# nv-tlabs/ChronoEdit

Hardware: AMD Instinct MI355X
Metric: denoising-steps/sec (higher is better)
Workload: dtype bf16

## Files before the change

### chronoedit_amd/csrc/ce_attn.hip

```cpp
#include <cstdlib>

#include "ce_common.h"

namespace {

constexpr int HD = 128;
constexpr int QW = 32;
constexpr int KVB = 64;
constexpr int K_TILE_BYTES = KVB * HD * 2;
constexpr int VT_TILE_BYTES = HD * KVB * 2;
constexpr int BUF_BYTES = K_TILE_BYTES + VT_TILE_BYTES;
constexpr int OST_ROW = HD * 2 + 16;
constexpr int smem_bytes(int nwave, bool two_seg) {
  const int stage = nwave * QW * OST_ROW;
  return two_seg ? 2 * BUF_BYTES + stage : (stage > 2 * BUF_BYTES ? stage : 2 * BUF_BYTES);
}
constexpr float NEG_BIG = -1.0e30f;

__device__ __forceinline__ int vt_swz(int dv) {
  return ((((dv >> 2) & 7) << 1) | (((dv >> 1) ^ (dv >> 5)) & 1)) ^ (((dv >> 6) & 1) << 1);
}

struct KVSeg {
  const bf16* k;
  const bf16* v;
  int len;
  int ldk;
  int ldv;
};
struct BlkRows {
  int rows;
  int stride;
  uint32_t magic;
  int vt_cols;
  unsigned char* q8;
  unsigned char* s8;
  int ld8;
};

template <bool TWO_SEG, int NWAVE>
__global__ __launch_bounds__(NWAVE * 64, NWAVE == 8 ? 2 : 2) void attn_fwd_kernel(const bf16* __restrict__ Q, bf16* __restrict__ O, KVSeg seg0,
                                                       KVSeg seg1, int Nq, int H, int ldq, int ldo, int nqb,
                                                       float scale_log2e) {
  extern __shared__ __attribute__((aligned(16))) unsigned char smem[];
  {
    const size_t bz = blockIdx.y;
    Q += bz * Nq * ldq;
    O += bz * Nq * ldo;
    seg0.k += bz * seg0.len * seg0.ldk;
    seg0.v += bz * seg0.len * seg0.ldv;
    if (TWO_SEG) {
      seg1.k += bz * seg1.len * seg1.ldk;
      seg1.v += bz * seg1.len * seg1.ldv;
    }
  }
  const int tid = threadIdx.x, lane = tid & 63, wave = tid >> 6;
  const int l31 = lane & 31, hh = lane >> 5;

  int head, qb;
  if ((H & 7) == 0) {
    const int xcd = blockIdx.x & 7, local = blockIdx.x >> 3;
    head = xcd + 8 * (local / nqb);
    qb = local % nqb;
  } else {
    head = blockIdx.x / nqb;
    qb = blockIdx.x % nqb;
  }
  constexpr int QB = QW * NWAVE;
  constexpr int NT = NWAVE * 64;
  const int q0 = qb * QB + wave * QW;
  const int hoff = head * HD;

  bf16x8 qf[8];
  {
    const bf16* qrow = Q + (size_t)min(q0 + l31, Nq - 1) * ldq + hoff + 8 * hh;
#pragma unroll
    for (int ks = 0; ks < 8; ++ks) qf[ks] = *reinterpret_cast<const bf16x8*>(qrow + 16 * ks);
  }

  constexpr int KREP = 1024 / NT, KROWS = NT / 16;
  const int k_ck = tid & 15, k_row0 = tid >> 4;
  constexpr int VREP = 512 / NT, VKQ = NT / 32;
  const int v_dvq = tid & 31, v_kvq = tid >> 5;

  unsigned char* ost = smem + (TWO_SEG ? 2 * BUF_BYTES : 0) + (size_t)(wave * QW + l31) * OST_ROW;

#pragma unroll
  for (int sidx = 0; sidx < (TWO_SEG ? 2 : 1); ++sidx) {
    const KVSeg sg = sidx == 0 ? seg0 : seg1;
    const int ntiles = (sg.len + KVB - 1) / KVB;

    f32x16 oacc[4];
#pragma unroll
    for (int m = 0; m < 4; ++m)
#pragma unroll
      for (int r = 0; r < 16; ++r) oacc[m][r] = 0.f;
    float m_run = NEG_BIG, l_run = 0.f;

    u32x4 kreg[KREP];
    u32x2 vreg[VREP][4];
    auto load_tile = [&](int t) {
      const int kv0 = t * KVB;
#pragma unroll
      for (int i = 0; i < KREP; ++i) {
        const int r = min(kv0 + k_row0 + KROWS * i, sg.len - 1);
        kreg[i] = *reinterpret_cast<const u32x4*>(sg.k + (size_t)r * sg.ldk + hoff + k_ck * 8);
      }
#pragma unroll
      for (int p = 0; p < VREP; ++p)
#pragma unroll
        for (int i = 0; i < 4; ++i) {
          const int r = min(kv0 + 4 * (v_kvq + VKQ * p) + i, sg.len - 1);
          vreg[p][i] = *reinterpret_cast<const u32x2*>(sg.v + (size_t)r * sg.ldv + hoff + v_dvq * 4);
        }
    };
    auto store_tile = [&](int buf) {
      unsigned char* sK = smem + buf * BUF_BYTES;
      unsigned char* sV = sK + K_TILE_BYTES;
#pragma unroll
      for (int i = 0; i < KREP; ++i) {
        const int r = k_row0 + KROWS * i;
        *reinterpret_cast<u32x4*>(sK + r * (HD * 2) + ((k_ck ^ (r & 15)) << 4)) = kreg[i];
      }
#pragma unroll
      for (int p = 0; p < VREP; ++p)
#pragma unroll
        for (int j = 0; j < 4; ++j) {
          const int w = j >> 1;
          uint32_t lo, hi;
          if ((j & 1) == 0) {
            lo = (vreg[p][0][w] & 0xffffu) | (vreg[p][1][w] << 16);
            hi = (vreg[p][2][w] & 0xffffu) | (vreg[p][3][w] << 16);
          } else {
            lo = (vreg[p][0][w] >> 16) | (vreg[p][1][w] & 0xffff0000u);
            hi = (vreg[p][2][w] >> 16) | (vreg[p][3][w] & 0xffff0000u);
          }
          const int dv = 4 * v_dvq + j;
          u32x2 val = {lo, hi};
          *reinterpret_cast<u32x2*>(sV + dv * (KVB * 2) + (((v_kvq + VKQ * p) ^ vt_swz(dv)) << 3)) = val;
        }
    };

    load_tile(0);
    __syncthreads();
    store_tile(0);
    __syncthreads();

    for (int t = 0; t < ntiles; ++t) {
      const int cur = t & 1;
      if (t + 1 < ntiles) load_tile(t + 1);
      const unsigned char* sK = smem + cur * BUF_BYTES;
      const unsigned char* sV = sK + K_TILE_BYTES;

      f32x16 st[2];
#pragma unroll
      for (int f = 0; f < 2; ++f) {
#pragma unroll
        for (int r = 0; r < 16; ++r) st[f][r] = 0.f;
        const int r = 32 * f + l31;
        const unsigned char* krow = sK + r * (HD * 2);
#pragma unroll
        for (int ks = 0; ks < 8; ++ks) {
          const bf16x8 kf = *reinterpret_cast<const bf16x8*>(krow + (((2 * ks + hh) ^ (r & 15)) << 4));
          st[f] = __builtin_amdgcn_mfma_f32_32x32x16_bf16(kf, qf[ks], st[f], 0, 0, 0);
        }
      }
      if ((t + 1) * KVB > sg.len) {
        const int base = t * KVB + 4 * hh;
#pragma unroll
        for (int f = 0; f < 2; ++f)
#pragma unroll
          for (int r = 0; r < 16; ++r) {
            const int kv = base + 32 * f + (r & 3) + 8 * (r >> 2);
            if (kv >= sg.len) st[f][r] = NEG_BIG;
          }
      }
      float mx = st[0][0];
#pragma unroll
      for (int f = 0; f < 2; ++f)
#pragma unroll
        for (int r = 0; r < 16; ++r) mx = fmaxf(mx, st[f][r]);
      mx = fmaxf(mx, __shfl_xor(mx, 32, 64));
      const float m_new = fmaxf(m_run, mx);
      const float alpha = __builtin_amdgcn_exp2f((m_run - m_new) * scale_log2e);
      const float mc = m_new * scale_log2e;
      m_run = m_new;
      float psum = 0.f;
#pragma unroll
      for (int f = 0; f < 2; ++f)
#pragma unroll
        for (int r = 0; r < 16; ++r) {
          const float p = __builtin_amdgcn_exp2f(fmaf(st[f][r], scale_log2e, -mc));
          st[f][r] = p;
          psum += p;
        }
      l_run = l_run * alpha + psum;
      if (__any(alpha != 1.0f)) {
#pragma unroll
        for (int m = 0; m < 4; ++m)
#pragma unroll
          for (int r = 0; r < 16; ++r) oacc[m][r] *= alpha;
      }

#pragma unroll
      for (int s = 0; s < 4; ++s) {
        const int f = s >> 1, rb = 8 * (s & 1);
        f32x2 t0 = {st[f][rb + 0], st[f][rb + 1]}, t1 = {st[f][rb + 2], st[f][rb + 3]};
        f32x2 t2 = {st[f][rb + 4], st[f][rb + 5]}, t3 = {st[f][rb + 6], st[f][rb + 7]};
        const bf16x2 p0 = __builtin_convertvector(t0, bf16x2), p1 = __builtin_convertvector(t1, bf16x2);
        const bf16x2 p2 = __builtin_convertvector(t2, bf16x2), p3 = __builtin_convertvector(t3, bf16x2);
        const bf16x8 pf = {p0[0], p0[1], p1[0], p1[1], p2[0], p2[1], p3[0], p3[1]};
        const int c0 = 4 * s + hh;
#pragma unroll
        for (int m = 0; m < 4; ++m) {
          const int dv = 32 * m + l31;
          const unsigned char* vrow = sV + dv * (KVB * 2);
          const int sw = vt_swz(dv);
          const bf16x4 va = *reinterpret_cast<const bf16x4*>(vrow + ((c0 ^ sw) << 3));
          const bf16x4 vb = *reinterpret_cast<const bf16x4*>(vrow + (((c0 + 2) ^ sw) << 3));
          const bf16x8 vf = {va[0], va[1], va[2], va[3], vb[0], vb[1], vb[2], vb[3]};
          oacc[m] = __builtin_amdgcn_mfma_f32_32x32x16_bf16(vf, pf, oacc[m], 0, 0, 0);
        }
      }
      if (t + 1 < ntiles) store_tile(cur ^ 1);
      __syncthreads();
    }

    const float l_tot = l_run + __shfl_xor(l_run, 32, 64);
    const float inv = 1.0f / l_tot;
#pragma unroll
    for (int m = 0; m < 4; ++m)
#pragma unroll
      for (int a = 0; a < 4; ++a) {
        uint32_t w0 = pack_bf16(oacc[m][4 * a + 0] * inv, oacc[m][4 * a + 1] * inv);
        uint32_t w1 = pack_bf16(oacc[m][4 * a + 2] * inv, oacc[m][4 * a + 3] * inv);
        u32x2* slot = reinterpret_cast<u32x2*>(ost + (32 * m + 8 * a + 4 * hh) * 2);
        if (TWO_SEG && sidx == 1) {
          const u32x2 pv = *slot;
          w0 = pack_bf16(bf16lo(pv[0]) + bf16lo(w0), bf16hi(pv[0]) + bf16hi(w0));
          w1 = pack_bf16(bf16lo(pv[1]) + bf16lo(w1), bf16hi(pv[1]) + bf16hi(w1));
        }
        u32x2 val = {w0, w1};
        *slot = val;
      }
  }

  __syncthreads();
#pragma unroll
  for (int i = 0; i < 8; ++i) {
    const int c = lane + 64 * i;
    const int rl = c >> 4, cc = c & 15;
    const int q = q0 + rl;
    if (q < Nq) {
      const u32x4 v = *reinterpret_cast<const u32x4*>(smem + (TWO_SEG ? 2 * BUF_BYTES : 0) + (size_t)(wave * QW + rl) * OST_ROW + cc * 16);
      *reinterpret_cast<u32x4*>(O + (size_t)q * ldo + hoff + cc * 8) = v;
    }
  }
}


#define CE_EPOCH_BARRIER()                          \
  asm volatile("s_waitcnt lgkmcnt(0)" ::: "memory"); \
  __builtin_amdgcn_s_barrier()
constexpr int PK_ROW = HD * 2 + 16;
constexpr int PV_ROW = KVB * 2 + 16;
constexpr int PK_TILE = KVB * PK_ROW;
constexpr int PV_TILE = HD * PV_ROW;
typedef __attribute__((ext_vector_type(4))) unsigned pp_u4;
typedef __attribute__((ext_vector_type(2))) unsigned pp_u2;

constexpr int K_GRP = 1088;
typedef __attribute__((address_space(3))) void lds_void;
#ifdef CE_DIAGNOSTICS
__device__ unsigned long long g_sp_exact_hits = 0ull;
#endif
constexpr float SP_SPEC_THR = 1024.0f;
constexpr int SP_V0 = 2 * PK_TILE;
constexpr int SP_TILE_BYTES = 2 * PK_TILE + 3 * PV_TILE;
constexpr int sp_smem_bytes(bool two_seg) { return two_seg ? SP_TILE_BYTES + 8 * QW * OST_ROW : SP_TILE_BYTES; }

template <bool TWO_SEG, bool VT = false, bool QOUT = false>
__global__ __launch_bounds__(512, 2) void attn_fwd_sp_kernel(const bf16* __restrict__ Q_, bf16* __restrict__ O_, KVSeg seg0_,
                                                              KVSeg seg1_, int Nq, int H, int ldq, int ldo, int nqb,
                                                              float scale_log2e, int batch, BlkRows blk) {
  extern __shared__ __attribute__((aligned(16))) unsigned char smem[];
  constexpr int NWAVE = 8, QB = QW * NWAVE;
  const int tid = threadIdx.x, lane = tid & 63;
  const int wave = __builtin_amdgcn_readfirstlane(tid >> 6);
  const int l31 = lane & 31, hh = lane >> 5;
  for (int item = blockIdx.x; item < nqb * H * batch; item += gridDim.x) {
  const bf16* Q = Q_;
  bf16* O = O_;
  KVSeg seg0 = seg0_, seg1 = seg1_;

  int head, qb, bz;
  {
    const int nqb_full = Nq / QB;
    if ((H & 7) == 0) {
      const int xcd = item & 7, local = item >> 3, hx_n = H >> 3;
      const int full = batch * hx_n * nqb_full;
      if (local < full) {
        bz = local / (hx_n * nqb_full);
        const int r = local % (hx_n * nqb_full);
        head = xcd + 8 * (r / nqb_full);
        qb = r % nqb_full;
      } else {
        const int l2 = local - full;
        bz = l2 / hx_n;
        head = xcd + 8 * (l2 % hx_n);
        qb = nqb_full;
      }
    } else {
      bz = item / (nqb * H);
      const int r = item % (nqb * H);
      head = r / nqb;
      qb = r % nqb;
    }
  }
  {
    if (VT && blk.rows > 0) {
      Q += (size_t)bz * blk.rows * ldq;
      O += (size_t)bz * blk.rows * ldo;
      seg0.k += (size_t)bz * blk.rows * seg0.ldk;
      seg0.v += (size_t)bz * blk.vt_cols;
    } else {
      Q += (size_t)bz * Nq * ldq;
      O += (size_t)bz * Nq * ldo;
      seg0.k += (size_t)bz * seg0.len * seg0.ldk;
      seg0.v += VT ? (size_t)bz * (TWO_SEG ? blk.vt_cols : seg0.len) : (size_t)bz * seg0.len * seg0.ldv;
    }
    if (TWO_SEG) {
      seg1.k += (size_t)bz * seg1.len * seg1.ldk;
      seg1.v += VT ? (size_t)bz * blk.stride : (size_t)bz * seg1.len * seg1.ldv;
    }
  }
  const int q0 = qb * QB + wave * QW;
  const int hoff = head * HD;
  const bool active = q0 < Nq;
  const int q0row = (VT && blk.rows > 0) ? (q0 / blk.rows) * blk.stride + q0 % blk.rows : q0;

  bf16x8 qf[8];
  {
    const bf16* qrow = Q + (size_t)(q0 + l31 < Nq ? q0row + l31 : 0) * ldq + hoff + 8 * hh;
#pragma unroll
    for (int ks = 0; ks < 8; ++ks) qf[ks] = *reinterpret_cast<const bf16x8*>(qrow + 16 * ks);
  }
  auto scale_q = [&]() __attribute__((always_inline)) {
#pragma unroll
  for (int ks = 0; ks < 8; ++ks) {
    const u32x4 w = __builtin_bit_cast(u32x4, qf[ks]);
    u32x4 o;
#pragma unroll
    for (int i = 0; i < 4; ++i) o[i] = pack_bf16(bf16lo(w[i]) * scale_log2e, bf16hi(w[i]) * scale_log2e);
    qf[ks] = __builtin_bit_cast(bf16x8, o);
  }
#pragma unroll
  for (int ks = 0; ks < 8; ++ks) asm volatile("" : "+v"(qf[ks]));

  };
  const int v_dvq = (tid & 1) | (((tid >> 4) & 15) << 1), v_kvq = ((tid >> 1) & 7) | (((tid >> 8) & 1) << 3);
  const int v_chunk = (v_kvq & ~3) | ((v_kvq & 1) << 1) | ((v_kvq >> 1) & 1);
  unsigned char* ost = smem + (TWO_SEG ? SP_TILE_BYTES : 0) + (size_t)(wave * QW + l31) * OST_ROW;
  const int k_w = l31 & 3;
  const unsigned char* k_rd = smem + (l31 >> 2) * K_GRP + k_w * 256 + ((hh ^ (k_w & 1)) << 4);
  const int k_eo[2] = {(k_w >> 1) << 5, ((k_w >> 1) ^ 1) << 5};
  const unsigned char* v_rd = smem + SP_V0 + l31 * PV_ROW + hh * 16;
  int vt_off[4];
#pragma unroll
  for (int s4 = 0; s4 < 4; ++s4) {
    const int x = (l31 >> 1) & 7;
    vt_off[s4] = l31 * 128 + ((2 * (s4 ^ (x >> 1)) + (hh ^ (x & 1))) << 4);
  }
  unsigned char* v_wr = smem + SP_V0 + (4 * v_dvq) * PV_ROW + v_chunk * 8;

#pragma unroll
  for (int sidx = 0; sidx < (TWO_SEG ? 2 : 1); ++sidx) {
    const KVSeg sg = sidx == 0 ? seg0 : seg1;
    const int ntiles = (sg.len + KVB - 1) / KVB;
    const int k_rows_span = (VT && blk.rows > 0) ? ((sg.len - 1) / blk.rows) * blk.stride + blk.rows : sg.len;
    const auto k_rsrc = __builtin_amdgcn_make_buffer_rsrc((void*)(sg.k + hoff), 0, (k_rows_span - 1) * sg.ldk * 2 + HD * 2, 0x00020000);
    const auto v_rsrc = VT ? __builtin_amdgcn_make_buffer_rsrc((void*)(sg.v + (size_t)hoff * sg.ldv), 0, ((HD - 1) * sg.ldv + ntiles * KVB) * 2, 0x00020000)
                           : __builtin_amdgcn_make_buffer_rsrc((void*)(sg.v + hoff), 0, (sg.len - 1) * sg.ldv * 2 + HD * 2, 0x00020000);
    int v_voff[4];
#pragma unroll
    for (int i = 0; i < 4; ++i) v_voff[i] = (4 * v_kvq + i) * sg.ldv * 2 + v_dvq * 8;
    const int k_tile_bytes = KVB * sg.ldk * 2, v_tile_bytes = KVB * sg.ldv * 2;

    f32x16 oacc[4];
#pragma unroll
    for (int m = 0; m < 4; ++m)
#pragma unroll
      for (int r = 0; r < 16; ++r) oacc[m][r] = 0.f;
    float l_run = 0.f, alpha_prev = 1.0f, mc = 0.f;
    f32x16 cinit;
#pragma unroll
    for (int r = 0; r < 16; ++r) cinit[r] = 0.f;
    u32x4 ppk[4];
#pragma unroll
    for (int s4 = 0; s4 < 4; ++s4) ppk[s4] = u32x4{0u, 0u, 0u, 0u};

    pp_u2 vreg[4];
    const int kd_row = VT ? (lane >> 4) + 4 * ((wave >> 1) & 1) + 8 * (wave & 1) + 16 * (wave >> 2) : 4 * wave + (lane >> 4);
    const int kd_voff0 = kd_row * sg.ldk * 2 + (((lane & 15) ^ (lane >> 4)) << 4), kd_voff1 = kd_voff0 + 32 * sg.ldk * 2;
    const int vd_row = 8 * wave + (lane >> 3);
    const int vd_voff0 = vd_row * sg.ldv * 2 + (((lane & 7) ^ ((vd_row >> 1) & 7)) << 4), vd_voff1 = vd_voff0 + 64 * sg.ldv * 2;
    auto dma_v = [&](int t, int buf, int j) {
      __builtin_amdgcn_raw_ptr_buffer_load_lds(v_rsrc, (lds_void*)(smem + SP_V0 + buf * PV_TILE + (wave + 8 * j) * 1024), 16,
                                               j ? vd_voff1 : vd_voff0, t * (KVB * 2), 0, 0);
    };
    auto dma_k = [&](int t, int buf, int j) {
      int soff = t * k_tile_bytes;
      if (VT && blk.rows > 0) {
        const int b_ = blk.magic ? (int)__umulhi((uint32_t)t, blk.magic) : t;
        soff = (b_ * blk.stride + (t - b_ * (blk.rows >> 6)) * KVB) * sg.ldk * 2;
      }
      __builtin_amdgcn_raw_ptr_buffer_load_lds(k_rsrc, (lds_void*)(smem + buf * PK_TILE + (wave + 8 * j) * K_GRP), 16,
                                               j ? kd_voff1 : kd_voff0, soff, 0, 0);
    };
    auto load_v = [&](int t) {
      const int so = t * v_tile_bytes;
#pragma unroll
      for (int i = 0; i < 4; ++i) vreg[i] = __builtin_amdgcn_raw_buffer_load_b64(v_rsrc, v_voff[i], so, 0);
    };
    auto store_v_part = [&](int buf, int j) {
      const int w = j >> 1;
      uint32_t lo, hi;
      if ((j & 1) == 0) {
        lo = (vreg[0][w] & 0xffffu) | (vreg[1][w] << 16);
        hi = (vreg[2][w] & 0xffffu) | (vreg[3][w] << 16);
      } else {
        lo = (vreg[0][w] >> 16) | (vreg[1][w] & 0xffff0000u);
        hi = (vreg[2][w] >> 16) | (vreg[3][w] & 0xffff0000u);
      }
      pp_u2 val = {lo, hi};
      *reinterpret_cast<pp_u2*>(v_wr + buf * PV_TILE + j * PV_ROW) = val;
    };
    auto store_v = [&](int buf) {
#pragma unroll
      for (int j = 0; j < 4; ++j) {
        const int w = j >> 1;
        uint32_t lo, hi;
        if ((j & 1) == 0) {
          lo = (vreg[0][w] & 0xffffu) | (vreg[1][w] << 16);
          hi = (vreg[2][w] & 0xffffu) | (vreg[3][w] << 16);
        } else {
          lo = (vreg[0][w] >> 16) | (vreg[1][w] & 0xffff0000u);
          hi = (vreg[2][w] >> 16) | (vreg[3][w] & 0xffff0000u);
        }
        pp_u2 val = {lo, hi};
        *reinterpret_cast<pp_u2*>(v_wr + buf * PV_TILE + j * PV_ROW) = val;
      }
    };

    if (TWO_SEG && sidx == 1) { CE_EPOCH_BARRIER(); }
    dma_k(0, 0, 0);
    dma_k(0, 0, 1);
    __builtin_amdgcn_sched_barrier(0);
    if (VT) {
      dma_v(0, 0, 0);
      dma_v(0, 0, 1);
    } else {
      load_v(0);
    }
    {
      const pp_u4 z = {0u, 0u, 0u, 0u};
      for (int i = tid; i < PV_TILE / 16; i += NWAVE * 64) *reinterpret_cast<pp_u4*>(smem + SP_V0 + 2 * PV_TILE + i * 16) = z;
    }
    if (!VT) {
      store_v(0);
      asm volatile("s_waitcnt vmcnt(0)" ::: "memory");
      load_v(1);
    }
    if (sidx == 0) scale_q();

#define CE_SP_KWAIT()                                          \
  do {                                                         \
    if (VT) asm volatile("s_waitcnt vmcnt(2)" ::: "memory");   \
    else asm volatile("s_waitcnt vmcnt(4)" ::: "memory");      \
  } while (0)
    int vb_prev = 2, vb_cur = 0;

    for (int t = 0; !active && t < ntiles; ++t) {
      CE_SP_KWAIT();
      CE_EPOCH_BARRIER();
      const int vb_next = 3 - vb_prev - vb_cur;
      dma_k(t + 1, (t + 1) & 1, 0);
      dma_k(t + 1, (t + 1) & 1, 1);
      __builtin_amdgcn_sched_barrier(0);
      if (VT) {
        dma_v(t + 1, vb_next, 0);
        dma_v(t + 1, vb_next, 1);
      } else {
        store_v(vb_next);
        load_v(t + 2);
      }
      vb_prev = vb_cur;
      vb_cur = vb_next;
    }
    for (int t = 0; active && t < ntiles; ++t) {
      CE_SP_KWAIT();
// ... 622 lines not shown
#pragma unroll
          for (int m = 0; m < 4; ++m)
#pragma unroll
            for (int r = 0; r < 16; ++r) oacc[sb][m][r] *= alpha_prev[sb];
          W4A_SETTLE_O(sb);
        }
#pragma unroll
      for (int u = 0; u < 16; ++u) {
        const bf16x8 vfd = CE_LDV(vtb, u);
#pragma unroll
        for (int sb = 0; sb < NSB; ++sb) W4A_PV(oacc[sb][u & 3], vfd, ppk[sb][u >> 2]);
      }
    }
#undef CE_LDK
#undef CE_LDV
#pragma unroll
    for (int sb = 0; sb < NSB; ++sb) W4A_SETTLE_O(sb);
    CE_EPOCH_BARRIER();
#pragma unroll
    for (int sb = 0; sb < NSB; ++sb) {
      unsigned char* ost = smem + (size_t)(wave * QWW + 32 * sb + l31) * OST_ROW;
      const float l_tot = l_run[sb] + __shfl_xor(l_run[sb], 32, 64);
      const float inv = 1.0f / l_tot;
#pragma unroll
      for (int m = 0; m < 4; ++m)
#pragma unroll
        for (int a = 0; a < 4; ++a) {
          const uint32_t w0 = pack_bf16(oacc[sb][m][4 * a + 0] * inv, oacc[sb][m][4 * a + 1] * inv);
          const uint32_t w1 = pack_bf16(oacc[sb][m][4 * a + 2] * inv, oacc[sb][m][4 * a + 3] * inv);
          *reinterpret_cast<u32x2*>(ost + (32 * m + 8 * a + 4 * hh) * 2) = u32x2{w0, w1};
        }
    }
  };
  if (active) {
    if (two_sub) run(w4_int<2>{});
    else run(w4_int<1>{});
  }
  __syncthreads();
#pragma unroll
  for (int i = 0; i < 16; ++i) {
    const int c = lane + 64 * i;
    const int rl = c >> 4, cc = c & 15;
    if (q0 + rl < Nq) {
      const u32x4 v = *reinterpret_cast<const u32x4*>(smem + (size_t)(wave * QWW + rl) * OST_ROW + cc * 16);
      *reinterpret_cast<u32x4*>(O + (size_t)(q0row + rl) * ldo + hoff + cc * 8) = v;
    }
  }
  __syncthreads();
  }
}
#undef W4A_S_FIRST
#undef W4A_S
#undef W4A_PV
#undef W4A_ADD
#undef W4A_CVT
#undef W4A_EXP
#undef W4A_SETTLE_S
#undef W4A_SETTLE_O

__global__ __launch_bounds__(256) void v_transpose_kernel(const bf16* __restrict__ V, int ldv, bf16* __restrict__ VT, int ldvt, int n_keys,
                                                          int blk_rows, int blk_stride, int vt_cols) {
  __shared__ __attribute__((aligned(16))) unsigned char tile[HD * (KVB * 2 + 16)];
  constexpr int TROW = KVB * 2 + 16;
  const int tid = threadIdx.x, head = blockIdx.y, key0 = blockIdx.x * KVB;
  if (blk_rows > 0) {
    V += ((size_t)(key0 / blk_rows) * blk_stride + (size_t)blockIdx.z * blk_rows + key0 % blk_rows - key0) * ldv;
    VT += (size_t)blockIdx.z * vt_cols;
  }
  const int col_end = blk_rows > 0 ? vt_cols : ldvt;
  const int kq = tid & 15, dq = tid >> 4;
#pragma unroll
  for (int pass = 0; pass < 2; ++pass) {
    const int d0 = 4 * (dq + 16 * pass);
    pp_u2 r[4];
#pragma unroll
    for (int i = 0; i < 4; ++i) {
      const int key = key0 + 4 * kq + i;
      r[i] = key < n_keys ? *reinterpret_cast<const pp_u2*>(V + (size_t)key * ldv + head * HD + d0) : pp_u2{0u, 0u};
    }
#pragma unroll
    for (int j = 0; j < 4; ++j) {
      const int w = j >> 1;
      uint32_t lo, hi;
      if ((j & 1) == 0) {
        lo = (r[0][w] & 0xffffu) | (r[1][w] << 16);
        hi = (r[2][w] & 0xffffu) | (r[3][w] << 16);
      } else {
        lo = (r[0][w] >> 16) | (r[1][w] & 0xffff0000u);
        hi = (r[2][w] >> 16) | (r[3][w] & 0xffff0000u);
      }
      *reinterpret_cast<pp_u2*>(tile + (d0 + j) * TROW + kq * 8) = pp_u2{lo, hi};
    }
  }
  __syncthreads();
#pragma unroll
  for (int i = 0; i < 4; ++i) {
    const int c = tid + 256 * i;
    const int d = c >> 3, ch = c & 7;
    const pp_u4 v = *reinterpret_cast<const pp_u4*>(tile + d * TROW + ch * 16);
    const int col = key0 + 8 * ch;
    if (col < col_end) *reinterpret_cast<pp_u4*>(VT + (size_t)(head * HD + d) * ldvt + col) = v;
  }
}

}

#ifdef CE_DIAGNOSTICS
extern "C" int ce_diag_mx_exact_hits(unsigned long long* out, int reset);
CE_API int ce_diag_attention_exact_route_hits(unsigned long long* hits, int reset) {
  if (!hits) return CE_ERR_ARG;
  unsigned long long v = 0ull, z = 0ull;
  if (hipDeviceSynchronize() != hipSuccess) return CE_ERR_ARG;
  if (hipMemcpyFromSymbol(&v, HIP_SYMBOL(g_sp_exact_hits), sizeof(v)) != hipSuccess) return CE_ERR_ARG;
  if (reset && hipMemcpyToSymbol(HIP_SYMBOL(g_sp_exact_hits), &z, sizeof(z)) != hipSuccess) return CE_ERR_ARG;
  hits[0] = v;
  return ce_diag_mx_exact_hits(hits + 1, reset);
}
#endif
CE_KNOB g_attn_nwave = 0;
#ifdef CE_DIAGNOSTICS
CE_API int ce_set_attention_waves(int nwave) {
  const int old = g_attn_nwave;
  if (nwave == 0 || nwave == 4 || nwave == 8 || nwave == 16 || nwave == 64 || nwave == 128 || nwave == 129) g_attn_nwave = nwave;
  return old;
}
#endif

CE_API int ce_attention_batched_bf16(const void* Q, const void* K1, const void* V1, int len1, int ldk1, int ldv1,
                                         const void* K2, const void* V2, int len2, int ldk2, int ldv2, void* O, int Nq, int H,
                                         int head_dim, int ldq, int ldo, float softmax_scale, int batch, hipStream_t stream) {
  if (!Q || !K1 || !V1 || !O) return CE_ERR_ARG;
  if (head_dim != HD || Nq <= 0 || H <= 0 || len1 <= 0 || batch <= 0 || batch > 65535) return CE_ERR_SHAPE;
  if ((ldq & 7) || (ldo & 7) || (ldk1 & 7) || (ldv1 & 3)) return CE_ERR_ALIGN;
  const bool two = (K2 != nullptr && V2 != nullptr && len2 > 0);
  if (two && ((ldk2 & 7) || (ldv2 & 3))) return CE_ERR_ALIGN;
  KVSeg s0{(const bf16*)K1, (const bf16*)V1, len1, ldk1, ldv1};
  KVSeg s1{(const bf16*)K2, (const bf16*)V2, two ? len2 : 0, ldk2, ldv2};
  const float sl2 = softmax_scale * 1.4426950408889634f;
  const bool sp = g_attn_nwave == 64 || g_attn_nwave == 0 || g_attn_nwave >= 128;
  const int nwave = sp ? 8 : g_attn_nwave;
  const int nqb = (Nq + nwave * QW - 1) / (nwave * QW);
  dim3 grid(nqb * H, batch), block(nwave * 64);
  if (sp) {
#define CE_ATTN_SP(TWO)                                                                                              \
  do {                                                                                                               \
    static bool done_[CE_MAX_DEVICES] = {};                                                                          \
    bool& done = done_[ce_device_slot()];                                                                            \
    if (!done) {                                                                                                     \
      (void)hipFuncSetAttribute((const void*)attn_fwd_sp_kernel<TWO>, hipFuncAttributeMaxDynamicSharedMemorySize,    \
                                sp_smem_bytes(TWO));                                                                 \
      done = true;                                                                                                   \
    }                                                                                                                \
    hipLaunchKernelGGL((attn_fwd_sp_kernel<TWO>), dim3(nqb * H * batch), block, sp_smem_bytes(TWO), stream, (const bf16*)Q, \
                       (bf16*)O, s0, s1, Nq, H, ldq, ldo, nqb, sl2, batch, BlkRows{0, 0, 0u, 0});                    \
  } while (0)
    if (two) CE_ATTN_SP(true); else CE_ATTN_SP(false);
#undef CE_ATTN_SP
    return (int)hipGetLastError();
  }
#define CE_ATTN_LAUNCH(TWO, NW)                                                                                     \
  do {                                                                                                              \
    static bool done_[CE_MAX_DEVICES] = {};                                                                         \
    bool& done = done_[ce_device_slot()];                                                                           \
    if (!done) {                                                                                                    \
      (void)hipFuncSetAttribute((const void*)attn_fwd_kernel<TWO, NW>, hipFuncAttributeMaxDynamicSharedMemorySize,  \
                                smem_bytes(NW, TWO));                                                               \
      done = true;                                                                                                  \
    }                                                                                                               \
    hipLaunchKernelGGL((attn_fwd_kernel<TWO, NW>), grid, block, smem_bytes(NW, TWO), stream, (const bf16*)Q, (bf16*)O, \
                       s0, s1, Nq, H, ldq, ldo, nqb, sl2);                                                          \
  } while (0)
  if (two) {
    if (nwave == 8) CE_ATTN_LAUNCH(true, 8); else CE_ATTN_LAUNCH(true, 4);
  } else {
    if (nwave == 8) CE_ATTN_LAUNCH(false, 8); else CE_ATTN_LAUNCH(false, 4);
  }
#undef CE_ATTN_LAUNCH
  return (int)hipGetLastError();
}

CE_API int ce_attention_bf16(const void* Q, const void* K1, const void* V1, int len1, int ldk1, int ldv1, const void* K2,
                                 const void* V2, int len2, int ldk2, int ldv2, void* O, int Nq, int H, int head_dim, int ldq,
                                 int ldo, float softmax_scale, hipStream_t stream) {
  return ce_attention_batched_bf16(Q, K1, V1, len1, ldk1, ldv1, K2, V2, len2, ldk2, ldv2, O, Nq, H, head_dim, ldq, ldo,
                                   softmax_scale, 1, stream);
}

CE_API int ce_v_transpose_bf16(const void* v, int ldv, void* vt, int ldvt, int n_keys, int H, hipStream_t stream) {
  if (!v || !vt) return CE_ERR_ARG;
  if (n_keys <= 0 || H <= 0 || ldvt < n_keys) return CE_ERR_SHAPE;
  if ((ldv & 3) || (ldvt & 7)) return CE_ERR_ALIGN;
  hipLaunchKernelGGL(v_transpose_kernel, dim3((ldvt + KVB - 1) / KVB, H), dim3(256), 0, stream, (const bf16*)v, ldv, (bf16*)vt, ldvt, n_keys, 0, 0, 0);
  return (int)hipGetLastError();
}

CE_API int ce_v_transpose_blocked_bf16(const void* v, int ldv, void* vt, int ldvt, int n_keys, int H, int batch, int blk_rows, int blk_stride,
                                           int vt_sample_cols, hipStream_t stream) {
  if (!v || !vt) return CE_ERR_ARG;
  if (n_keys <= 0 || H <= 0 || batch <= 0 || blk_rows <= 0 || (blk_rows & 63) || blk_stride < batch * blk_rows || (vt_sample_cols & 63) ||
      vt_sample_cols < (n_keys + KVB - 1) / KVB * KVB || ldvt < batch * vt_sample_cols)
    return CE_ERR_SHAPE;
  if ((ldv & 3) || (ldvt & 7)) return CE_ERR_ALIGN;
  hipLaunchKernelGGL(v_transpose_kernel, dim3(vt_sample_cols / KVB, H, batch), dim3(256), 0, stream, (const bf16*)v, ldv, (bf16*)vt, ldvt, n_keys,
                     blk_rows, blk_stride, vt_sample_cols);
  return (int)hipGetLastError();
}

#ifdef CE_DIAGNOSTICS
extern "C" int ce_attn16_launch(const void* Q, const void* K, const void* Vt, int len, int ldk, int ldvt, void* O, int Nq, int H, int ldq, int ldo,
                                float sl2, int batch, int cus, hipStream_t stream);
#endif

static int attention_vt_launch(const void* Q, const void* K, const void* Vt, int len, int ldk, int ldvt, void* O, int Nq, int H, int head_dim,
                               int ldq, int ldo, float softmax_scale, int batch, int blk_rows, int blk_stride, int vt_sample_cols,
                               hipStream_t stream) {
  if (!Q || !K || !Vt || !O) return CE_ERR_ARG;
  if (head_dim != HD || Nq <= 0 || H <= 0 || len <= 0 || batch <= 0 || batch > 65535) return CE_ERR_SHAPE;
  const int ntiles_cols = (len + KVB - 1) / KVB * KVB;
  if (blk_rows == 0) {
    vt_sample_cols = len;
    if (ldvt < (batch - 1) * len + ntiles_cols) return CE_ERR_SHAPE;
  } else {
    if ((blk_rows & 63) || blk_stride < batch * blk_rows || (Nq % blk_rows) || vt_sample_cols < ntiles_cols ||
        ldvt < (batch - 1) * vt_sample_cols + ntiles_cols)
      return CE_ERR_SHAPE;
  }
  if ((ldq & 7) || (ldo & 7) || (ldk & 7) || (ldvt & 7) || (batch > 1 && (vt_sample_cols & 1))) return CE_ERR_ALIGN;
  KVSeg s0{(const bf16*)K, (const bf16*)Vt, len, ldk, ldvt};
  KVSeg s1{nullptr, nullptr, 0, 0, 0};
  BlkRows blk{blk_rows, blk_stride, 0u, vt_sample_cols};
  if (blk_rows > 0) {
    const uint32_t tps = (uint32_t)(blk_rows >> 6);
    blk.magic = tps == 1 ? 0u : (uint32_t)(((1ull << 32) + tps - 1) / tps);
  }
  const float sl2 = softmax_scale * 1.4426950408889634f;
  const int nqb = (Nq + 8 * QW - 1) / (8 * QW);
  static bool done_[CE_MAX_DEVICES] = {};
  bool& done = done_[ce_device_slot()];
  if (!done) {
    (void)hipFuncSetAttribute((const void*)attn_fwd_sp_kernel<false, true>, hipFuncAttributeMaxDynamicSharedMemorySize, sp_smem_bytes(false));
    done = true;
  }
  const int cus = ce_device_cus();
  const int items = nqb * H * batch;
#ifdef CE_DIAGNOSTICS
  if (g_attn_nwave == 16 && blk_rows == 0) {
    const int rc = ce_attn16_launch(Q, K, Vt, len, ldk, ldvt, O, Nq, H, ldq, ldo, sl2, batch, cus, stream);
    if (rc != CE_ERR_ALIGN) return rc;
  }
#endif
  if (g_attn_nwave == 128 || g_attn_nwave == 129) {
    static bool done4_[CE_MAX_DEVICES] = {};
    bool& done4 = done4_[ce_device_slot()];
    if (!done4) {
      (void)hipFuncSetAttribute((const void*)attn_fwd_w4_kernel, hipFuncAttributeMaxDynamicSharedMemorySize, W4_SMEM);
      done4 = true;
    }
    const int grid4 = (g_attn_nwave == 129 && items > cus) ? (cus & ~7) : items;
    hipLaunchKernelGGL(attn_fwd_w4_kernel, dim3(grid4), dim3(256), W4_SMEM, stream, (const bf16*)Q, (bf16*)O, s0, Nq, H, ldq, ldo, nqb,
                       sl2, batch, blk);
    return (int)hipGetLastError();
  }
  const int grid_vt = items <= 2 * cus ? items : ((2 * cus) & ~7);
  hipLaunchKernelGGL((attn_fwd_sp_kernel<false, true>), dim3(grid_vt), dim3(512), sp_smem_bytes(false), stream, (const bf16*)Q, (bf16*)O,
                     s0, s1, Nq, H, ldq, ldo, nqb, sl2, batch, blk);
  return (int)hipGetLastError();
}

CE_API int ce_attention_vt_bf16(const void* Q, const void* K, const void* Vt, int len, int ldk, int ldvt, void* O, int Nq, int H,
                                    int head_dim, int ldq, int ldo, float softmax_scale, int batch, hipStream_t stream) {
  return attention_vt_launch(Q, K, Vt, len, ldk, ldvt, O, Nq, H, head_dim, ldq, ldo, softmax_scale, batch, 0, 0, 0, stream);
}

CE_API int ce_attention_vt_blocked_bf16(const void* Q, const void* K, const void* Vt, int len, int ldk, int ldvt, void* O, int Nq, int H,
                                            int head_dim, int ldq, int ldo, float softmax_scale, int batch, int blk_rows, int blk_stride,
                                            int vt_sample_cols, hipStream_t stream) {
  if (blk_rows <= 0) return CE_ERR_SHAPE;
  return attention_vt_launch(Q, K, Vt, len, ldk, ldvt, O, Nq, H, head_dim, ldq, ldo, softmax_scale, batch, blk_rows, blk_stride, vt_sample_cols,
                             stream);
}


static int attention_2seg_vt_launch(const void* Q, const void* K1, const void* V1t, int len1, int ldk1, int ldv1t, int vt_cols1,
                                    const void* K2, const void* V2t, int len2, int ldk2, int ldv2t, int vt_cols2, void* O, int Nq,
                                    int H, int head_dim, int ldq, int ldo, float softmax_scale, int batch, void* O8, void* S8, int ldo8,
                                    hipStream_t stream) {
  if (!Q || !K1 || !V1t || !K2 || !V2t || (!O && !O8)) return CE_ERR_ARG;
  if (head_dim != HD || Nq <= 0 || H <= 0 || len1 <= 0 || len2 <= 0 || batch <= 0 || batch > 65535) return CE_ERR_SHAPE;
  const int c1 = (len1 + KVB - 1) / KVB * KVB, c2 = (len2 + KVB - 1) / KVB * KVB;
  if (vt_cols1 < len1 || vt_cols2 < len2 || ldv1t < (batch - 1) * vt_cols1 + c1 || ldv2t < (batch - 1) * vt_cols2 + c2) return CE_ERR_SHAPE;
  if ((ldq & 7) || (ldo & 7) || (ldk1 & 7) || (ldk2 & 7) || (ldv1t & 7) || (ldv2t & 7) || (vt_cols1 & 1) || (vt_cols2 & 1)) return CE_ERR_ALIGN;
  KVSeg s0{(const bf16*)K1, (const bf16*)V1t, len1, ldk1, ldv1t};
  KVSeg s1{(const bf16*)K2, (const bf16*)V2t, len2, ldk2, ldv2t};
  const float sl2 = softmax_scale * 1.4426950408889634f;
  const int nqb = (Nq + 8 * QW - 1) / (8 * QW);
  static bool done_[CE_MAX_DEVICES] = {};
  bool& done = done_[ce_device_slot()];
  if (!done) {
    (void)hipFuncSetAttribute((const void*)attn_fwd_sp_kernel<true, true>, hipFuncAttributeMaxDynamicSharedMemorySize, sp_smem_bytes(true));
    (void)hipFuncSetAttribute((const void*)attn_fwd_sp_kernel<true, true, true>, hipFuncAttributeMaxDynamicSharedMemorySize, sp_smem_bytes(true));
    done = true;
  }
  const BlkRows blk{0, vt_cols2, 0u, vt_cols1, (unsigned char*)O8, (unsigned char*)S8, ldo8};
  const int cus = ce_device_cus();
  const int items = nqb * H * batch;
  const int grid = items <= 2 * cus ? items : ((2 * cus) & ~7);
  if (O8)
    hipLaunchKernelGGL((attn_fwd_sp_kernel<true, true, true>), dim3(grid), dim3(512), sp_smem_bytes(true), stream, (const bf16*)Q,
                       (bf16*)O, s0, s1, Nq, H, ldq, ldo, nqb, sl2, batch, blk);
  else
    hipLaunchKernelGGL((attn_fwd_sp_kernel<true, true>), dim3(grid), dim3(512), sp_smem_bytes(true), stream, (const bf16*)Q, (bf16*)O,
                       s0, s1, Nq, H, ldq, ldo, nqb, sl2, batch, blk);
  return (int)hipGetLastError();
}

CE_API int ce_attention_2seg_vt_bf16(const void* Q, const void* K1, const void* V1t, int len1, int ldk1, int ldv1t, int vt_cols1,
                                         const void* K2, const void* V2t, int len2, int ldk2, int ldv2t, int vt_cols2, void* O, int Nq,
                                         int H, int head_dim, int ldq, int ldo, float softmax_scale, int batch, hipStream_t stream) {
  if (!O) return CE_ERR_ARG;
  return attention_2seg_vt_launch(Q, K1, V1t, len1, ldk1, ldv1t, vt_cols1, K2, V2t, len2, ldk2, ldv2t, vt_cols2, O, Nq, H, head_dim, ldq, ldo,
                                  softmax_scale, batch, nullptr, nullptr, 0, stream);
}

CE_API int ce_attention_2seg_vt_quant_bf16(const void* Q, const void* K1, const void* V1t, int len1, int ldk1, int ldv1t, int vt_cols1,
                                               const void* K2, const void* V2t, int len2, int ldk2, int ldv2t, int vt_cols2, void* o8,
                                               void* scale8, int Nq, int H, int head_dim, int ldq, int ldo8, float softmax_scale, int batch,
                                               hipStream_t stream) {
  if (!o8 || !scale8 || (ldo8 & 15) || ((H * head_dim) & 127)) return CE_ERR_ARG;
  return attention_2seg_vt_launch(Q, K1, V1t, len1, ldk1, ldv1t, vt_cols1, K2, V2t, len2, ldk2, ldv2t, vt_cols2, nullptr, Nq, H, head_dim, ldq,
                                  8, softmax_scale, batch, o8, scale8, ldo8, stream);
}
```

### chronoedit_amd/csrc/ce_rowops.hip

```cpp
#include "ce_common.h"

#define ROW_MAXC 10
#ifndef CE_LN_ROWS
#define CE_LN_ROWS 2
#endif

template <int FP8, bool FULL, int R>
__global__ __launch_bounds__(256) void ln_affine_kernel(const bf16* __restrict__ x, bf16* __restrict__ y,
                                                        const float* __restrict__ a, const float* __restrict__ b,
                                                        int M, int D, int ldx, int ldy, float eps, int ab_rows, int ab_stride,
                                                        unsigned char* __restrict__ q8, float* __restrict__ qscale, int ldq) {
  const int lane = threadIdx.x & 63;
  const int row0 = (blockIdx.x * 4 + (threadIdx.x >> 6)) * R;
  if (row0 >= M) return;
  if (ab_rows > 0) {
    a += (size_t)(row0 / ab_rows) * ab_stride;
    b += (size_t)(row0 / ab_rows) * ab_stride;
  }
  const int nch = D >> 3;
  u32x4 raw[R][ROW_MAXC];
  float mean[R], rstd[R];
#pragma unroll
  for (int k = 0; k < R; ++k) {
    const bf16* xr = x + (size_t)min(row0 + k, M - 1) * ldx;
#pragma unroll
    for (int i = 0; i < ROW_MAXC; ++i) {
      const int c = lane + 64 * i;
      if (FULL || c < nch) raw[k][i] = *reinterpret_cast<const u32x4*>(xr + c * 8);
    }
  }
#pragma unroll
  for (int k = 0; k < R; ++k) {
    float s = 0.f;
#pragma unroll
    for (int i = 0; i < ROW_MAXC; ++i) {
      const int c = lane + 64 * i;
      if (FULL || c < nch) {
#pragma unroll
        for (int j = 0; j < 4; ++j) s += bf16lo(raw[k][i][j]) + bf16hi(raw[k][i][j]);
      }
    }
    mean[k] = wave_sum(s) / (float)D;
    float v = 0.f;
#pragma unroll
    for (int i = 0; i < ROW_MAXC; ++i) {
      const int c = lane + 64 * i;
      if (FULL || c < nch) {
#pragma unroll
        for (int j = 0; j < 4; ++j) {
          const float d0 = bf16lo(raw[k][i][j]) - mean[k], d1 = bf16hi(raw[k][i][j]) - mean[k];
          v += d0 * d0 + d1 * d1;
        }
      }
    }
    rstd[k] = 1.0f / sqrtf(wave_sum(v) / (float)D + eps);
  }
  float amax[R];
#pragma unroll
  for (int k = 0; k < R; ++k) amax[k] = 0.f;
#pragma unroll
  for (int i = 0; i < ROW_MAXC; ++i) {
    const int c = lane + 64 * i;
    if (FULL || c < nch) {
      const f32x4 a0 = *reinterpret_cast<const f32x4*>(a + c * 8), a1 = *reinterpret_cast<const f32x4*>(a + c * 8 + 4);
      const f32x4 b0 = *reinterpret_cast<const f32x4*>(b + c * 8), b1 = *reinterpret_cast<const f32x4*>(b + c * 8 + 4);
#pragma unroll
      for (int k = 0; k < R; ++k) {
        u32x4 o;
#pragma unroll
        for (int j = 0; j < 4; ++j) {
          const float aa0 = j < 2 ? a0[2 * j] : a1[2 * j - 4], aa1 = j < 2 ? a0[2 * j + 1] : a1[2 * j - 3];
          const float bb0 = j < 2 ? b0[2 * j] : b1[2 * j - 4], bb1 = j < 2 ? b0[2 * j + 1] : b1[2 * j - 3];
          const float n0 = (bf16lo(raw[k][i][j]) - mean[k]) * rstd[k], n1 = (bf16hi(raw[k][i][j]) - mean[k]) * rstd[k];
          o[j] = pack_bf16(n0 * aa0 + bb0, n1 * aa1 + bb1);
          if (FP8 == 1) amax[k] = fmaxf(amax[k], fmaxf(fabsf(bf16lo(o[j])), fabsf(bf16hi(o[j]))));
        }
        if (FP8 == 1) raw[k][i] = o;
        else if (FP8 == 0 && row0 + k < M) *reinterpret_cast<u32x4*>(y + (size_t)(row0 + k) * ldy + c * 8) = o;
        if (FP8 == 2) raw[k][i] = o;
      }
    }
    if (FP8 == 2) {
#pragma unroll
      for (int k = 0; k < R; ++k) {
        const bool on = (FULL || c < nch) && row0 + k < M;
        const u32x4 v = raw[k][i];
        float am = 0.f;
        if (FULL || c < nch) {
#pragma unroll
          for (int j = 0; j < 4; ++j) am = fmaxf(am, fmaxf(fabsf(bf16lo(v[j])), fabsf(bf16hi(v[j]))));
        }
        am = fmaxf(am, __shfl_xor(am, 1, 64));
        am = fmaxf(am, __shfl_xor(am, 2, 64));
        if (on) {
          const int byte = mx_scale_byte_nosat(am);
          const float inv = mx_inv_scale(byte);
          int w0 = 0, w1 = 0;
          w0 = __builtin_amdgcn_cvt_pk_fp8_f32(clamp448(bf16lo(v[0]) * inv), clamp448(bf16hi(v[0]) * inv), w0, false);
          w0 = __builtin_amdgcn_cvt_pk_fp8_f32(clamp448(bf16lo(v[1]) * inv), clamp448(bf16hi(v[1]) * inv), w0, true);
          w1 = __builtin_amdgcn_cvt_pk_fp8_f32(clamp448(bf16lo(v[2]) * inv), clamp448(bf16hi(v[2]) * inv), w1, false);
          w1 = __builtin_amdgcn_cvt_pk_fp8_f32(clamp448(bf16lo(v[3]) * inv), clamp448(bf16hi(v[3]) * inv), w1, true);
          const u32x2 ov = {(uint32_t)w0, (uint32_t)w1};
          *reinterpret_cast<u32x2*>(q8 + (size_t)(row0 + k) * ldq + c * 8) = ov;
          if ((lane & 3) == 0) reinterpret_cast<unsigned char*>(qscale)[mx_gemm_scale_offset(row0 + k, c >> 2, D >> 7)] = (unsigned char)byte;
        }
      }
    }
  }
  if (FP8 == 1) {
#pragma unroll
    for (int k = 0; k < R; ++k) {
      const float am = wave_max(amax[k]);
      const float sc = am > 0.f ? am * (1.0f / 448.0f) : 1.0f;
      const float inv = 1.0f / sc;
      if (row0 + k >= M) continue;
      if (lane == 0) qscale[row0 + k] = sc;
      unsigned char* qr = q8 + (size_t)(row0 + k) * ldq;
#pragma unroll
      for (int i = 0; i < ROW_MAXC; ++i) {
        const int c = lane + 64 * i;
        if (FULL || c < nch) {
          const u32x4 v = raw[k][i];
          int w0 = 0, w1 = 0;
          w0 = __builtin_amdgcn_cvt_pk_fp8_f32(bf16lo(v[0]) * inv, bf16hi(v[0]) * inv, w0, false);
          w0 = __builtin_amdgcn_cvt_pk_fp8_f32(bf16lo(v[1]) * inv, bf16hi(v[1]) * inv, w0, true);
          w1 = __builtin_amdgcn_cvt_pk_fp8_f32(bf16lo(v[2]) * inv, bf16hi(v[2]) * inv, w1, false);
          w1 = __builtin_amdgcn_cvt_pk_fp8_f32(bf16lo(v[3]) * inv, bf16hi(v[3]) * inv, w1, true);
          u32x2 o = {(uint32_t)w0, (uint32_t)w1};
          *reinterpret_cast<u32x2*>(qr + c * 8) = o;
        }
      }
    }
  }
}

template <bool FULL>
__global__ __launch_bounds__(256) void rmsnorm_rope_kernel(bf16* __restrict__ x0, const float* __restrict__ w0,
                                                           bf16* __restrict__ x1, const float* __restrict__ w1,
                                                           const float* __restrict__ cs, int M, int D, int ld,
                                                           int head_dim, float eps, int rope_rows) {
  const int lane = threadIdx.x & 63;
  const int row = blockIdx.x * 4 + (threadIdx.x >> 6);
  if (row >= M) return;
  bf16* __restrict__ x = blockIdx.y ? x1 : x0;
  const float* __restrict__ w = blockIdx.y ? w1 : w0;
  const int cs_row = rope_rows > 0 ? row % rope_rows : row;
  const int nch = D >> 3;
  bf16* xr = x + (size_t)row * ld;
  u32x4 raw[ROW_MAXC];
  float s = 0.f;
#pragma unroll
  for (int i = 0; i < ROW_MAXC; ++i) {
    const int c = lane + 64 * i;
    if (FULL || c < nch) {
      raw[i] = *reinterpret_cast<const u32x4*>(xr + c * 8);
#pragma unroll
      for (int j = 0; j < 4; ++j) {
        const float v0 = bf16lo(raw[i][j]), v1 = bf16hi(raw[i][j]);
        s += v0 * v0 + v1 * v1;
      }
    }
  }
  const float rstd = 1.0f / sqrtf(wave_sum(s) / (float)D + eps);
  const int half = head_dim >> 1;
  const bool cs_once = cs != nullptr && (512 % head_dim) == 0;
  f32x4 csa = {0.f, 0.f, 0.f, 0.f}, csb = {0.f, 0.f, 0.f, 0.f};
  if (cs_once) {
    const float* p = cs + ((size_t)cs_row * half + (((lane * 8) % head_dim) >> 1)) * 2;
    csa = *reinterpret_cast<const f32x4*>(p);
    csb = *reinterpret_cast<const f32x4*>(p + 4);
  }
#pragma unroll
  for (int i = 0; i < ROW_MAXC; ++i) {
    const int c = lane + 64 * i;
    if (FULL || c < nch) {
      const f32x4 w0 = *reinterpret_cast<const f32x4*>(w + c * 8), w1 = *reinterpret_cast<const f32x4*>(w + c * 8 + 4);
      u32x4 o;
      f32x4 cs0 = csa, cs1 = csb;
      if (cs != nullptr && !cs_once) {
        const int pair0 = ((c * 8) % head_dim) >> 1;
        const float* p = cs + ((size_t)cs_row * half + pair0) * 2;
        cs0 = *reinterpret_cast<const f32x4*>(p);
        cs1 = *reinterpret_cast<const f32x4*>(p + 4);
      }
#pragma unroll
      for (int j = 0; j < 4; ++j) {
        const float ww0 = j < 2 ? w0[2 * j] : w1[2 * j - 4], ww1 = j < 2 ? w0[2 * j + 1] : w1[2 * j - 3];
        float v0 = round_bf16(round_bf16(bf16lo(raw[i][j]) * rstd) * ww0);
        float v1 = round_bf16(round_bf16(bf16hi(raw[i][j]) * rstd) * ww1);
        if (cs != nullptr) {
          const float co = j < 2 ? cs0[2 * j] : cs1[2 * j - 4], si = j < 2 ? cs0[2 * j + 1] : cs1[2 * j - 3];
          const float r0 = v0 * co - v1 * si, r1 = v0 * si + v1 * co;
          v0 = r0;
          v1 = r1;
        }
        o[j] = pack_bf16(v0, v1);
      }
      *reinterpret_cast<u32x4*>(xr + c * 8) = o;
    }
  }
}

template <bool FULL>
__global__ __launch_bounds__(256) void rope_scatter_kernel(const bf16* __restrict__ x, int ldx, bf16* __restrict__ send,
                                                           int M, int D, int W, int nt, int col0, const float* __restrict__ w0,
                                                           int col1, const float* __restrict__ w1, int col2,
                                                           const float* __restrict__ w2, const float* __restrict__ cs,
                                                           int head_dim, float eps, int rope_rows) {
  const int lane = threadIdx.x & 63;
  const int row = blockIdx.x * 4 + (threadIdx.x >> 6);
  if (row >= M) return;
  const int ti = blockIdx.y;
  const int col = ti == 0 ? col0 : ti == 1 ? col1 : col2;
  const float* __restrict__ w = ti == 0 ? w0 : ti == 1 ? w1 : w2;
  const int cs_row = rope_rows > 0 ? row % rope_rows : row;
  const int nch = D >> 3;
  const int Dl = D / W;
  const bf16* xr = x + (size_t)row * ldx + col;
  u32x4 raw[ROW_MAXC];
  float s = 0.f;
#pragma unroll
  for (int i = 0; i < ROW_MAXC; ++i) {
    const int c = lane + 64 * i;
    if (FULL || c < nch) {
      raw[i] = *reinterpret_cast<const u32x4*>(xr + c * 8);
#pragma unroll
      for (int j = 0; j < 4; ++j) {
        const float v0 = bf16lo(raw[i][j]), v1 = bf16hi(raw[i][j]);
        s += v0 * v0 + v1 * v1;
      }
    }
  }
  const float rstd = 1.0f / sqrtf(wave_sum(s) / (float)D + eps);
  const int half = head_dim >> 1;
#pragma unroll
  for (int i = 0; i < ROW_MAXC; ++i) {
    const int c = lane + 64 * i;
    if (FULL || c < nch) {
      u32x4 o = raw[i];
      if (w != nullptr) {
        const f32x4 wa = *reinterpret_cast<const f32x4*>(w + c * 8), wb = *reinterpret_cast<const f32x4*>(w + c * 8 + 4);
        f32x4 cs0, cs1;
        if (cs != nullptr) {
          const int pair0 = ((c * 8) % head_dim) >> 1;
          const float* p = cs + ((size_t)cs_row * half + pair0) * 2;
          cs0 = *reinterpret_cast<const f32x4*>(p);
          cs1 = *reinterpret_cast<const f32x4*>(p + 4);
        }
#pragma unroll
        for (int j = 0; j < 4; ++j) {
          const float ww0 = j < 2 ? wa[2 * j] : wb[2 * j - 4], ww1 = j < 2 ? wa[2 * j + 1] : wb[2 * j - 3];
          float v0 = round_bf16(round_bf16(bf16lo(raw[i][j]) * rstd) * ww0);
          float v1 = round_bf16(round_bf16(bf16hi(raw[i][j]) * rstd) * ww1);
          if (cs != nullptr) {
            const float co = j < 2 ? cs0[2 * j] : cs1[2 * j - 4], si = j < 2 ? cs0[2 * j + 1] : cs1[2 * j - 3];
            const float r0 = v0 * co - v1 * si, r1 = v0 * si + v1 * co;
            v0 = r0;
            v1 = r1;
          }
          o[j] = pack_bf16(v0, v1);
        }
      }
      const int n = c * 8, r = n / Dl, cc = n - r * Dl;
      *reinterpret_cast<u32x4*>(send + (((size_t)r * M + row) * nt + ti) * Dl + cc) = o;
    }
  }
}

template <typename TT>
__global__ void timestep_sinusoid_kernel(const TT* __restrict__ t, float* __restrict__ out, int dim) {
  const int i = blockIdx.x * blockDim.x + threadIdx.x;
  const int half = dim >> 1;
  if (i >= dim) return;
  const int k = i < half ? i : i - half;
  const float freq = expf(-9.210340371976184f * (float)k / (float)half);
  const float arg = (float)t[0] * freq;
  out[i] = i < half ? cosf(arg) : sinf(arg);
}

constexpr int GEMV_ROWS = 16;
template <typename WT>
__global__ __launch_bounds__(256) void gemv_kernel(const WT* __restrict__ W, const float* __restrict__ x,
                                                   const float* __restrict__ bias, float* __restrict__ y, int N, int K,
                                                   int flags) {
  extern __shared__ __attribute__((aligned(16))) float xs[];
  for (int k = threadIdx.x; k < K; k += 256) {
    float xv = x[k];
    if (flags & 1) xv = round_bf16(silu(xv));
    xs[k] = xv;
  }
  __syncthreads();
  const int lane = threadIdx.x & 63, wave = threadIdx.x >> 6;
  constexpr int VEC = 16 / sizeof(WT);
  const bool vec = (K % (64 * VEC)) == 0 && ((size_t)W & 15) == 0;
  for (int r = 0; r < GEMV_ROWS / 4; ++r) {
    const int n = blockIdx.x * GEMV_ROWS + r * 4 + wave;
    if (n >= N) break;
    const WT* wr = W + (size_t)n * K;
    float acc = 0.f;
    if (vec) {
      for (int k = lane * VEC; k < K; k += 64 * VEC) {
        const u32x4 wv = *reinterpret_cast<const u32x4*>(wr + k);
        const f32x4 x0 = *reinterpret_cast<const f32x4*>(xs + k);
        if (sizeof(WT) == 2) {
          const f32x4 x1 = *reinterpret_cast<const f32x4*>(xs + k + 4);
#pragma unroll
          for (int j = 0; j < 4; ++j) {
            acc += bf16lo(wv[j]) * (j < 2 ? x0[2 * j] : x1[2 * j - 4]);
            acc += bf16hi(wv[j]) * (j < 2 ? x0[2 * j + 1] : x1[2 * j - 3]);
          }
        } else {
#pragma unroll
          for (int j = 0; j < 4; ++j) acc += __uint_as_float(wv[j]) * x0[j];
        }
      }
    } else {
      for (int k = lane; k < K; k += 64) acc += (float)wr[k] * xs[k];
    }
    acc = wave_sum(acc);
    if (lane == 0) {
      float rr = acc + (bias ? bias[n] : 0.f);
      if (flags & 4) rr = round_bf16(rr);
      if (flags & 2) rr = silu(rr);
      y[n] = rr;
    }
  }
}

__global__ void modulation_kernel(const float* __restrict__ table, const float* __restrict__ v, float* __restrict__ mod,
                                  int L, int J, int D, int v_rows, int one_mask) {
  const size_t idx = (size_t)blockIdx.x * blockDim.x + threadIdx.x;
  const size_t total = (size_t)L * J * D;
  if (idx >= total) return;
  const int d = idx % D;
  const int j = (idx / D) % J;
  const float add = v[(size_t)(v_rows == 1 ? 0 : j) * D + d];
  float r = table[idx] + add;
  if ((one_mask >> j) & 1) r = 1.0f + r;
  mod[idx] = r;
}

__global__ void patchify_kernel(const bf16* __restrict__ x, bf16* __restrict__ cols, int C, int T, int H, int W, int Kpad,
                                int row0, int nrows) {
  const size_t idx = (size_t)blockIdx.x * blockDim.x + threadIdx.x;
  const int h2 = H >> 1, w2 = W >> 1;
  const size_t ntok = (size_t)T * h2 * w2;
  const size_t total = (size_t)nrows * Kpad;
  if (idx >= total) return;
  const int k = idx % Kpad;
  const size_t tok = idx / Kpad + row0;
  bf16 v = (bf16)0.f;
  if (k < C * 4 && tok < ntok) {
    const int c = k >> 2, dh = (k >> 1) & 1, dw = k & 1;
    const int wq = tok % w2, hq = (tok / w2) % h2, t = tok / ((size_t)w2 * h2);
    v = x[(((size_t)c * T + t) * H + (hq * 2 + dh)) * W + wq * 2 + dw];
  }
  cols[idx] = v;
}

__global__ void unpatchify_kernel(const bf16* __restrict__ y, bf16* __restrict__ out, int Cout, int T, int H, int W, int ldy) {
  const size_t idx = (size_t)blockIdx.x * blockDim.x + threadIdx.x;
  const size_t total = (size_t)Cout * T * H * W;
  if (idx >= total) return;
  const int w = idx % W, h = (idx / W) % H, t = (idx / ((size_t)W * H)) % T, c = idx / ((size_t)W * H * T);
  const int h2 = H >> 1, w2 = W >> 1;
  const size_t tok = ((size_t)t * h2 + (h >> 1)) * w2 + (w >> 1);
  out[idx] = y[tok * ldy + ((h & 1) * 2 + (w & 1)) * Cout + c];
}

CE_API int ce_ln_affine_bf16(const void* x, void* y, const float* a, const float* b, int M, int D, int ldx, int ldy,
                                 float eps, int ab_rows, int ab_stride, hipStream_t stream) {
  if (!x || !y || !a || !b) return CE_ERR_ARG;
  if (M <= 0 || D <= 0 || (D & 7) || D > 64 * 8 * ROW_MAXC || (ldx & 7) || (ldy & 7) || (ab_rows > 0 && (ab_stride & 3))) return CE_ERR_SHAPE;
  const bool multi = D == 64 * 8 * ROW_MAXC && (ab_rows <= 0 || ab_rows % CE_LN_ROWS == 0);
  if (multi)
    hipLaunchKernelGGL((ln_affine_kernel<0, true, CE_LN_ROWS>), dim3((M + 4 * CE_LN_ROWS - 1) / (4 * CE_LN_ROWS)), dim3(256), 0, stream,
                       (const bf16*)x, (bf16*)y, a, b, M, D, ldx, ldy, eps, ab_rows, ab_stride, nullptr, nullptr, 0);
  else if (D == 64 * 8 * ROW_MAXC)
    hipLaunchKernelGGL((ln_affine_kernel<0, true, 1>), dim3((M + 3) / 4), dim3(256), 0, stream, (const bf16*)x, (bf16*)y, a, b, M,
                       D, ldx, ldy, eps, ab_rows, ab_stride, nullptr, nullptr, 0);
  else
    hipLaunchKernelGGL((ln_affine_kernel<0, false, 1>), dim3((M + 3) / 4), dim3(256), 0, stream, (const bf16*)x, (bf16*)y, a, b, M,
                       D, ldx, ldy, eps, ab_rows, ab_stride, nullptr, nullptr, 0);
  return (int)hipGetLastError();
}

CE_API int ce_ln_affine_fp8(const void* x, void* q, float* scale, const float* a, const float* b, int M, int D, int ldx, int ldq,
                                float eps, int ab_rows, int ab_stride, hipStream_t stream) {
  if (!x || !q || !scale || !a || !b) return CE_ERR_ARG;
  if (M <= 0 || D <= 0 || (D & 7) || D > 64 * 8 * ROW_MAXC || (ldx & 7) || (ldq & 7) || (ab_rows > 0 && (ab_stride & 3))) return CE_ERR_SHAPE;
  if (D == 64 * 8 * ROW_MAXC)
    hipLaunchKernelGGL((ln_affine_kernel<1, true, 1>), dim3((M + 3) / 4), dim3(256), 0, stream, (const bf16*)x, nullptr, a, b, M, D,
                       ldx, 0, eps, ab_rows, ab_stride, (unsigned char*)q, scale, ldq);
  else
    hipLaunchKernelGGL((ln_affine_kernel<1, false, 1>), dim3((M + 3) / 4), dim3(256), 0, stream, (const bf16*)x, nullptr, a, b, M, D,
                       ldx, 0, eps, ab_rows, ab_stride, (unsigned char*)q, scale, ldq);
  return (int)hipGetLastError();
}

CE_API int ce_ln_affine_mxfp8(const void* x, void* q, void* scale8, const float* a, const float* b, int M, int D, int ldx, int ldq, float eps,
                                  int ab_rows, int ab_stride, hipStream_t stream) {
  if (!x || !q || !scale8 || !a || !b) return CE_ERR_ARG;
  if (M <= 0 || D <= 0 || (D & 127) || D > 64 * 8 * ROW_MAXC || (ldx & 7) || (ldq & 7) || (ab_rows > 0 && (ab_stride & 3))) return CE_ERR_SHAPE;
  if (D == 64 * 8 * ROW_MAXC)
    hipLaunchKernelGGL((ln_affine_kernel<2, true, 1>), dim3((M + 3) / 4), dim3(256), 0, stream, (const bf16*)x, nullptr, a, b, M, D, ldx, 0, eps,
                       ab_rows, ab_stride, (unsigned char*)q, (float*)scale8, ldq);
  else
    hipLaunchKernelGGL((ln_affine_kernel<2, false, 1>), dim3((M + 3) / 4), dim3(256), 0, stream, (const bf16*)x, nullptr, a, b, M, D, ldx, 0, eps,
                       ab_rows, ab_stride, (unsigned char*)q, (float*)scale8, ldq);
  return (int)hipGetLastError();
}

CE_API int ce_rmsnorm_rope_bf16(void* x, const float* w, void* x2, const float* w2, const float* cos_sin, int M, int D, int ld,
                                    int head_dim, float eps, int rope_rows, hipStream_t stream) {
  if (!x || !w || (x2 && !w2)) return CE_ERR_ARG;
  if (M <= 0 || D <= 0 || (D & 7) || D > 64 * 8 * ROW_MAXC || (ld & 7) || (head_dim & 7) || D % head_dim) return CE_ERR_SHAPE;
  if (D == 64 * 8 * ROW_MAXC)
    hipLaunchKernelGGL(rmsnorm_rope_kernel<true>, dim3((M + 3) / 4, x2 ? 2 : 1), dim3(256), 0, stream, (bf16*)x, w, (bf16*)x2, w2,
                       cos_sin, M, D, ld, head_dim, eps, rope_rows);
  else
    hipLaunchKernelGGL(rmsnorm_rope_kernel<false>, dim3((M + 3) / 4, x2 ? 2 : 1), dim3(256), 0, stream, (bf16*)x, w, (bf16*)x2, w2,
                       cos_sin, M, D, ld, head_dim, eps, rope_rows);
  return (int)hipGetLastError();
}

CE_API int ce_timestep_sinusoid(const int64_t* t, float* out, int dim, hipStream_t stream) {
  if (!t || !out || dim <= 0 || (dim & 1)) return CE_ERR_ARG;
  hipLaunchKernelGGL(timestep_sinusoid_kernel<int64_t>, dim3((dim + 255) / 256), dim3(256), 0, stream, t, out, dim);
  return (int)hipGetLastError();
}

CE_API int ce_timestep_sinusoid_f32(const float* t, float* out, int dim, hipStream_t stream) {
  if (!t || !out || dim <= 0 || (dim & 1)) return CE_ERR_ARG;
  hipLaunchKernelGGL(timestep_sinusoid_kernel<float>, dim3((dim + 255) / 256), dim3(256), 0, stream, t, out, dim);
  return (int)hipGetLastError();
}

CE_API int ce_gemv(const void* W, int w_is_bf16, const float* x, const float* bias, float* y, int N, int K, int flags,
                       hipStream_t stream) {
  if (!W || !x || !y || N <= 0 || K <= 0) return CE_ERR_ARG;
  if (K > 16384) return CE_ERR_SHAPE;
  if (w_is_bf16)
    hipLaunchKernelGGL(gemv_kernel<bf16>, dim3((N + GEMV_ROWS - 1) / GEMV_ROWS), dim3(256), (size_t)K * 4, stream, (const bf16*)W, x, bias, y,
                       N, K, flags);
  else
    hipLaunchKernelGGL(gemv_kernel<float>, dim3((N + GEMV_ROWS - 1) / GEMV_ROWS), dim3(256), (size_t)K * 4, stream, (const float*)W, x, bias,
                       y, N, K, flags);
  return (int)hipGetLastError();
}

CE_API int ce_modulation(const float* table, const float* v, float* mod, int L, int J, int D, int v_rows, int one_mask,
                             hipStream_t stream) {
  if (!table || !v || !mod || L <= 0 || J <= 0 || D <= 0 || (v_rows != 1 && v_rows != J)) return CE_ERR_ARG;
  const size_t total = (size_t)L * J * D;
  hipLaunchKernelGGL(modulation_kernel, dim3((unsigned)((total + 255) / 256)), dim3(256), 0, stream, table, v, mod, L, J, D,
                     v_rows, one_mask);
  return (int)hipGetLastError();
}

CE_API int ce_patchify_rows_bf16(const void* x, void* cols, int C, int T, int H, int W, int Kpad, int row0, int nrows,
                                     hipStream_t stream) {
  if (!x || !cols || (H & 1) || (W & 1) || Kpad < C * 4 || row0 < 0 || nrows <= 0) return CE_ERR_ARG;
  const size_t total = (size_t)nrows * Kpad;
  hipLaunchKernelGGL(patchify_kernel, dim3((unsigned)((total + 255) / 256)), dim3(256), 0, stream, (const bf16*)x, (bf16*)cols,
                     C, T, H, W, Kpad, row0, nrows);
  return (int)hipGetLastError();
}

CE_API int ce_patchify_bf16(const void* x, void* cols, int C, int T, int H, int W, int Kpad, hipStream_t stream) {
  if ((H & 1) || (W & 1)) return CE_ERR_ARG;
  return ce_patchify_rows_bf16(x, cols, C, T, H, W, Kpad, 0, T * (H / 2) * (W / 2), stream);
}

CE_API int ce_rope_scatter_bf16(const void* x, int ldx, void* send, int M, int D, int W, int nt, int col0, const float* w0,
                                    int col1, const float* w1, int col2, const float* w2, const float* cos_sin, int head_dim,
                                    float eps, int rope_rows, hipStream_t stream) {
  if (!x || !send || nt < 1 || nt > 3 || W < 1) return CE_ERR_ARG;
  if (M <= 0 || D <= 0 || (D & 7) || D > 64 * 8 * ROW_MAXC || (ldx & 7) || (head_dim & 7) || D % head_dim || D % W ||
      ((D / W) & 7) || (col0 & 7) || (col1 & 7) || (col2 & 7))
    return CE_ERR_SHAPE;
  if (D == 64 * 8 * ROW_MAXC)
    hipLaunchKernelGGL(rope_scatter_kernel<true>, dim3((M + 3) / 4, nt), dim3(256), 0, stream, (const bf16*)x, ldx, (bf16*)send, M,
                       D, W, nt, col0, w0, col1, w1, col2, w2, cos_sin, head_dim, eps, rope_rows);
  else
    hipLaunchKernelGGL(rope_scatter_kernel<false>, dim3((M + 3) / 4, nt), dim3(256), 0, stream, (const bf16*)x, ldx, (bf16*)send, M,
                       D, W, nt, col0, w0, col1, w1, col2, w2, cos_sin, head_dim, eps, rope_rows);
  return (int)hipGetLastError();
}

CE_API int ce_unpatchify_bf16(const void* y, void* out, int Cout, int T, int H, int W, int ldy, hipStream_t stream) {
  if (!y || !out || (H & 1) || (W & 1) || ldy < 4 * Cout) return CE_ERR_ARG;
  const size_t total = (size_t)Cout * T * H * W;
  hipLaunchKernelGGL(unpatchify_kernel, dim3((unsigned)((total + 255) / 256)), dim3(256), 0, stream, (const bf16*)y, (bf16*)out,
                     Cout, T, H, W, ldy);
  return (int)hipGetLastError();
}
```

### chronoedit_amd/hiplib.py

```python
from __future__ import annotations

import ctypes
import os
import re
import subprocess
from typing import Dict, List

PKG_DIR = os.path.dirname(os.path.abspath(__file__))
ROOT = os.path.dirname(PKG_DIR)
CSRC = os.path.join(PKG_DIR, "csrc")
LIB_DIR = os.path.join(PKG_DIR, "lib")
LIB_PATH = os.path.join(LIB_DIR, "libchronoedit_hip.so")
DIAG_LIB_PATH = os.path.join(LIB_DIR, "libchronoedit_hip_diag.so")
OBJ_DIR = os.path.join(LIB_DIR, "obj")
HEADER = os.path.join(ROOT, "include", "chronoedit_hip.h")
DIAG_HEADER = os.path.join(ROOT, "include", "chronoedit_hip_diag.h")

DIAG_SOURCES = ["ce_gemm.hip", "ce_gemm256.hip", "ce_attn.hip", "ce_attn_fp8.hip", "ce_gemm_fp8.hip", "ce_gemm_fp8w4.hip"]
DIAG_ONLY_SOURCES = ["ce_attn16.hip"]
SOURCES = ["ce_rowops.hip", "ce_gemm.hip", "ce_gemm256.hip", "ce_gemm256w4.hip", "ce_gemm384.hip", "ce_attn.hip", "ce_attn16.hip", "ce_attn_fp8.hip", "ce_sched.hip", "ce_conv.hip", "ce_enc.hip", "ce_gemm_fp8.hip", "ce_gemm_fp8w4.hip", "ce_comm.hip", "ce_lora.hip"]

_c = ctypes
_P, _I, _F = _c.c_void_p, _c.c_int, _c.c_float

SIGNATURES: Dict[str, List] = {
    "ce_ln_affine_bf16": [_P, _P, _P, _P, _I, _I, _I, _I, _F, _I, _I, _P],
    "ce_rmsnorm_rope_bf16": [_P, _P, _P, _P, _P, _I, _I, _I, _I, _F, _I, _P],
    "ce_gemm_bf16": [_P, _P, _P, _P, _I, _P, _P, _I, _I, _I, _I, _I, _I, _I, _I, _I, _c.c_longlong, _I, _c.c_longlong, _P, _c.c_size_t, _P],
    "ce_rmsnorm_rope_mxfp8": [_P, _P, _P, _P, _P, _I, _I, _I, _I, _I, _F, _I, _F, _P],
    "ce_v_mxfp8_transpose": [_P, _I, _P, _P, _I, _I, _I, _I, _P],
    "ce_attention_mxfp8": [_P, _P, _P, _P, _P, _P, _P, _I, _I, _I, _I, _I, _I, _I, _I, _I, _P],
    "ce_attention_mxfp8_quant": [_P, _P, _P, _P, _P, _P, _P, _P, _I, _I, _I, _I, _I, _I, _I, _I, _I, _P],
    "ce_attention_mxfp8_add": [_P, _P, _P, _P, _P, _P, _P, _I, _P, _I, _P, _P, _I, _I, _I, _I, _I, _I, _I, _I, _I, _P],
    "ce_rope_scatter_bf16": [_P, _I, _P, _I, _I, _I, _I, _I, _P, _I, _P, _I, _P, _P, _I, _F, _I, _P],
    "ce_patchify_rows_bf16": [_P, _P, _I, _I, _I, _I, _I, _I, _I, _P],
    "ce_comm_load": [ctypes.c_char_p],
    "ce_comm_unique_id": [_P],
    "ce_comm_init": [ctypes.POINTER(ctypes.c_void_p), _P, _I, _I],
    "ce_comm_destroy": [_P],
    "ce_comm_all_to_all": [_P, _P, _P, ctypes.c_size_t, _P],
    "ce_comm_all_gather": [_P, _P, _P, ctypes.c_size_t, _P],
    "ce_ln_affine_fp8": [_P, _P, _P, _P, _P, _I, _I, _I, _I, _F, _I, _I, _P],
    "ce_quant_rows_fp8": [_P, _P, _P, _I, _I, _I, _I, _P],
    "ce_gemm_fp8": [_P, _P, _P, _P, _P, _P, _I, _P, _P, _I, _I, _I, _I, _I, _I, _I, _I, _P, _c.c_size_t, _P],
    "ce_quant_rows_mxfp8": [_P, _P, _P, _I, _I, _I, _I, _P],
    "ce_quant_rows_mxfp8_w": [_P, _P, _P, _I, _I, _I, _I, _P],
    "ce_ln_affine_mxfp8": [_P, _P, _P, _P, _P, _I, _I, _I, _I, _F, _I, _I, _P],
    "ce_gemm_mxfp8": [_P, _P, _P, _P, _P, _P, _I, _P, _P, _I, _I, _I, _I, _I, _I, _I, _I, _P, _c.c_size_t, _P],
    "ce_gemm_mxfp8_gelu_quant": [_P, _P, _P, _P, _P, _P, _P, _I, _I, _I, _I, _I, _I, _P, _c.c_size_t, _P],
    "ce_gemm_batched_bf16": [_P, _P, _P, _P, _I, _I, _I, _I, _I, _I, _I, _I, _I] + [ctypes.c_longlong] * 6 + [_P],
    "ce_im2col_patch2d_bf16": [_P, _P, _I, _I, _I, _I, _I, _I, _P],
    "ce_gather_rows_bf16": [_P, _P, _P, _I, _I, _I, _I, _I, _P],
    "ce_rmsnorm_bf16": [_P, _P, _P, _I, _I, _I, _I, _F, _P],
    "ce_softmax_t5_bf16": [_P, _P, _I, _I, _I, _I, _I, _I, _P, _P, _P, _P],
    "ce_attention_bf16": [_P, _P, _P, _I, _I, _I, _P, _P, _I, _I, _I, _P, _I, _I, _I, _I, _I, _F, _P],
    "ce_attention_batched_bf16": [_P, _P, _P, _I, _I, _I, _P, _P, _I, _I, _I, _P, _I, _I, _I, _I, _I, _F, _I, _P],
    "ce_attention_vt_bf16": [_P, _P, _P, _I, _I, _I, _P, _I, _I, _I, _I, _I, _F, _I, _P],
    "ce_attention_2seg_vt_bf16": [_P, _P, _P, _I, _I, _I, _I, _P, _P, _I, _I, _I, _I, _P, _I, _I, _I, _I, _I, _F, _I, _P],
    "ce_attention_2seg_vt_quant_bf16": [_P, _P, _P, _I, _I, _I, _I, _P, _P, _I, _I, _I, _I, _P, _P, _I, _I, _I, _I, _I, _F, _I, _P],
    "ce_v_transpose_bf16": [_P, _I, _P, _I, _I, _I, _P],
    "ce_attention_vt_blocked_bf16": [_P, _P, _P, _I, _I, _I, _P, _I, _I, _I, _I, _I, _F, _I, _I, _I, _I, _P],
    "ce_v_transpose_blocked_bf16": [_P, _I, _P, _I, _I, _I, _I, _I, _I, _I, _P],
    "ce_timestep_sinusoid": [_P, _P, _I, _P],
    "ce_timestep_sinusoid_f32": [_P, _P, _I, _P],
    "ce_gemv": [_P, _I, _P, _P, _P, _I, _I, _I, _P],
    "ce_modulation": [_P, _P, _P, _I, _I, _I, _I, _I, _P],
    "ce_patchify_bf16": [_P, _P, _I, _I, _I, _I, _I, _P],
    "ce_unpatchify_bf16": [_P, _P, _I, _I, _I, _I, _I, _P],
    "ce_conv_igemm_bf16": [_P, _I, _P, _P, _P, _I, _P] + [_I] * 16 + [_P],
    "ce_conv3d_head_bf16": [_P, _I, _P, _P, _P, _I] + [_I] * 10 + [_P],
    "ce_gemm_bf16_tile_rows": [_I, _I, _I, _I, _c.c_longlong],
    "ce_zero_border_bf16": [_P, _I, _I, _I, _I, _I, _P],
    "ce_conv3d_gemm_bf16": [_P, _P, _I, _P, _P, _P, _I, _I, _I, _I, _I, _I, _I, _I, _P],
    "ce_conv3d_gemm_rms_silu_bf16": [_P, _P, _I, _P, _P, _P, _P, _I, _I, _I, _I, _I, _I, _I, _P, _I, _P],
    "ce_rms_silu_bf16": [_P, _P, _P, _c.c_longlong, _I, _I, _I, _I, _I, _I, _P],
    "ce_upsample2x_bf16": [_P, _P, _I, _I, _I, _I, _P],
    "ce_softmax_rows_f32_bf16": [_P, _P, _I, _I, _I, _I, _I, _F, _P],
    "ce_attention_1head_bf16": [_P, _P, _P, _P, _I, _I, _I, _I, _I, _I, _I, _F, _P, _c.c_longlong, _P],
    "ce_cfg_unipc_step": [_P, _P, _P, _P, _P, _P, _P, _P, _P, _c.c_longlong, _I, _P],
    "ce_lora_merge_bf16": [_P, _I, _P, _I, _I, _I, _I, _P, _P, _P, _P, _P],
    "ce_build_info": [],
}
DIAG_SIGNATURES: Dict[str, List] = {
    "ce_set_gemm_variant": [_I],
    "ce_set_attention_waves": [_I],
    "ce_set_gemm_fp8_variant": [_I],
    "ce_set_attention_mxfp8_variant": [_I],
    "ce_set_attention_mxfp8_persistent": [_I],
    "ce_diag_attention_exact_route_hits": [_P, _I],
}


def header_symbols(diag: bool = False) -> List[str]:
    txt = open(DIAG_HEADER if diag else HEADER).read()
    return re.findall(r"^int (ce_\w+)\(", txt, flags=re.M)


def exported_symbols(path: str) -> List[str]:
    nm = "/opt/rocm/lib/llvm/bin/llvm-nm" if os.path.exists("/opt/rocm/lib/llvm/bin/llvm-nm") else "nm"
    out = subprocess.run([nm, "-D", "--defined-only", path], check=True, capture_output=True, text=True).stdout
    return sorted(l.split()[-1] for l in out.splitlines() if l.split() and l.split()[-2] in ("T", "t", "W", "D", "B"))


HIPCC_FLAGS = ["--offload-arch=gfx950", "-O3", "-std=c++17", "-fPIC", "-fvisibility=hidden"]


def build(force: bool = False, verbose: bool = False, jobs: int = 0) -> str:
    import glob
    from concurrent.futures import ThreadPoolExecutor
    srcs = [s for s in SOURCES if os.path.exists(os.path.join(CSRC, s))]
    hdrs = sorted(glob.glob(os.path.join(CSRC, "*.h"))) + [HEADER, DIAG_HEADER]
    hdr_m = max(os.path.getmtime(d) for d in hdrs)
    os.makedirs(OBJ_DIR, exist_ok=True)
    hipcc = os.environ.get("HIPCC", "/opt/rocm/bin/hipcc")
    todo, objs, diag_objs = [], [], []
    for s_ in srcs:
        src, stem = os.path.join(CSRC, s_), s_[:-4]
        variants = [("", [])] + ([(".diag", ["-DCE_DIAGNOSTICS"])] if s_ in DIAG_SOURCES else [])
        for tag, defs in variants:
            obj = os.path.join(OBJ_DIR, stem + tag + ".o")
            if force or not os.path.exists(obj) or os.path.getmtime(obj) < max(os.path.getmtime(src), hdr_m):
                todo.append([hipcc, *HIPCC_FLAGS, *defs, "-I", CSRC, "-c", src, "-o", obj])
            if tag or s_ in DIAG_ONLY_SOURCES:
                diag_objs.append(obj)
            else:
                objs.append(obj)
        if s_ not in DIAG_SOURCES and s_ not in DIAG_ONLY_SOURCES:
            diag_objs.append(os.path.join(OBJ_DIR, stem + ".o"))

    def run(cmd):
        if verbose:
            print(" ".join(cmd), flush=True)
        subprocess.run(cmd, check=True)

    if todo:
        with ThreadPoolExecutor(max_workers=jobs or min(8, os.cpu_count() or 4)) as ex:
            list(ex.map(run, todo))
    for path, group, diag in ((LIB_PATH, objs, False), (DIAG_LIB_PATH, diag_objs, True)):
        if force or todo or not os.path.exists(path) or os.path.getmtime(path) < max([hdr_m] + [os.path.getmtime(o) for o in group]):
            vs = os.path.join(OBJ_DIR, "exports_diag.map" if diag else "exports.map")
            names = header_symbols() + (header_symbols(diag=True) if diag else [])
            with open(vs, "w") as f:
                f.write("{\n  global:\n" + "".join(f"    {n};\n" for n in names) + "  local: *;\n};\n")
            run([hipcc, "--offload-arch=gfx950", "-shared", "-fPIC", *group, "-ldl", f"-Wl,--version-script={vs}", "-o", path])
    return LIB_PATH


_LIB = None
_DIAG = None


def _open(path: str, diag: bool) -> ctypes.CDLL:
    if not os.path.exists(path):
        raise RuntimeError(
            f"{path} is missing: the HIP extension is the only compute path of chronoedit_amd "
            "(no CPU/eager fallback). Build it with `python -c 'import __graft_entry__ as g; g.build()'`."
        )
    import torch
    declared, selectors = set(header_symbols()), set(header_symbols(diag=True))
    if diag:
        declared |= selectors
    exported = {s for s in exported_symbols(path) if s.startswith("ce_")}
    missing, unknown = declared - exported, exported - declared - selectors
    if missing or unknown:
        raise RuntimeError(f"{path} does not match include/chronoedit_hip{'_diag' if diag else ''}.h: missing {sorted(missing)}, "
                           f"not declared {sorted(unknown)}")
    lib = ctypes.CDLL(path)
    for name, argtypes in dict(SIGNATURES, **(DIAG_SIGNATURES if diag else {})).items():
        fn = getattr(lib, name)
        fn.argtypes = argtypes
        fn.restype = _c.c_int
    return lib


def load() -> ctypes.CDLL:
    global _LIB
    if _LIB is not None:
        return _LIB
    path = LIB_PATH
    override = os.environ.get("CE_HIPLIB_PATH")
    if override:
        import warnings
        warnings.warn(f"CE_HIPLIB_PATH is set: loading {override} instead of the in-tree build {LIB_PATH}", RuntimeWarning, stacklevel=2)
        path = override
    lib = _open(path, diag=False)
    info = lib.ce_build_info()
    if (info & 1 or (info >> 8) & 255) and os.environ.get("CE_HIPLIB_ALLOW_DIAGNOSTIC_BUILD") != "1":
        raise RuntimeError(f"{path}: ce_build_info() = {info:#x} - " + ("a timing-only F8_ABLATE build whose results are garbage" if (info >> 8) & 255
                           else "the diagnostic build") + "; refusing to use it as the product library (CE_HIPLIB_ALLOW_DIAGNOSTIC_BUILD=1 overrides)")
    _LIB = lib
    return lib


def load_diagnostics() -> ctypes.CDLL:
    global _DIAG
    if _DIAG is None:
        _DIAG = _open(DIAG_LIB_PATH, diag=True)
        if not _DIAG.ce_build_info() & 1:
            raise RuntimeError(f"{DIAG_LIB_PATH} was not compiled with -DCE_DIAGNOSTICS")
    return _DIAG
```

### chronoedit_amd/ops.py

```python
from __future__ import annotations

import ctypes
from typing import Optional

import torch

from . import hiplib

EPI_BIAS, EPI_BIAS_GELU, EPI_GATE_RES, EPI_BIAS_GELU_ERF = 0, 1, 2, 3
EPI_F32, EPI_MUL, EPI_BIAS_ROW, EPI_BIAS_T = 4, 5, 6, 7

_lib = None
_product = None

_KNOB_DEFAULTS = {"ce_set_gemm_variant": -1, "ce_set_attention_waves": 0, "ce_set_gemm_fp8_variant": 1,
                  "ce_set_attention_mxfp8_variant": 1, "ce_set_attention_mxfp8_persistent": 512}
_knobs = dict(_KNOB_DEFAULTS)


def lib():
    global _lib, _product
    if _lib is None:
        _lib = _product = hiplib.load()
        import os
        v8 = os.environ.get("CE_GEMM_FP8_VARIANT")
        if v8 is not None:
            _set_knob("ce_set_gemm_fp8_variant", int(v8))
        v = os.environ.get("CE_GEMM_VARIANT")
        if v is not None:
            _set_knob("ce_set_gemm_variant", int(v))
    return _lib


_force_diag = False


def force_diagnostics(on: bool = True) -> None:
    global _lib, _force_diag
    lib()
    _force_diag = bool(on)
    want = hiplib.load_diagnostics() if (_force_diag or any(_knobs[k] != _KNOB_DEFAULTS[k] for k in _knobs)) else _product
    if want is not _lib:
        _lib = want


def attention_exact_route_hits(reset: bool = True):
    buf = (ctypes.c_ulonglong * 2)()
    _check(hiplib.load_diagnostics().ce_diag_attention_exact_route_hits(buf, 1 if reset else 0), "ce_diag_attention_exact_route_hits")
    return int(buf[0]), int(buf[1])


def _set_knob(symbol: str, v: int) -> int:
    global _lib
    lib()
    diag = hiplib.load_diagnostics()
    prev = getattr(diag, symbol)(int(v))
    _knobs[symbol] = getattr(diag, symbol)(int(v))
    want = diag if (_force_diag or any(_knobs[k] != _KNOB_DEFAULTS[k] for k in _knobs)) else _product
    if want is not _lib:
        _lib = want
    return prev


class HipKernelError(RuntimeError):
    pass


_PROF = None


class profile:

    def __enter__(self):
        global _PROF
        _PROF = []
        return self

    def __exit__(self, *exc):
        global _PROF
        self.records, _PROF = _PROF, None
        return False

    def summary(self):
        torch.cuda.synchronize()
        out = {}
        for key, work, st, en in self.records:
            d = out.setdefault(key, {"n": 0, "total_ms": 0.0, "work": work})
            d["n"] += 1
            d["total_ms"] += st.elapsed_time(en)
        for d in out.values():
            d["avg_ms"] = d["total_ms"] / d["n"]
        return out


def _prof_begin():
    if _PROF is None:
        return None
    st = torch.cuda.Event(enable_timing=True)
    st.record()
    return st


def _prof_end(st, key, work):
    if st is not None:
        en = torch.cuda.Event(enable_timing=True)
        en.record()
        _PROF.append((key, work, st, en))


def _check(rc: int, name: str):
    if rc != 0:
        kind = {-1: "bad argument", -2: "unsupported shape", -3: "misaligned stride"}.get(rc, f"hipError {rc}")
        raise HipKernelError(f"{name} failed: {kind}")


def _stream() -> ctypes.c_void_p:
    return ctypes.c_void_p(torch.cuda.current_stream().cuda_stream)


def _ptr(t: Optional[torch.Tensor]) -> ctypes.c_void_p:
    return ctypes.c_void_p(0 if t is None else t.data_ptr())


def _dev(t: torch.Tensor, dtype, name: str):
    if not t.is_cuda:
        raise HipKernelError(f"{name}: tensor must live on the GPU (the HIP path has no CPU fallback)")
    if t.dtype != dtype:
        raise TypeError(f"{name}: expected {dtype}, got {t.dtype}")


def _rows(t: torch.Tensor, name: str):
    if t.dim() != 2 or t.stride(1) != 1:
        raise ValueError(f"{name}: need a 2-D tensor with contiguous rows, got shape {tuple(t.shape)} stride {t.stride()}")
    return t.shape[0], t.shape[1], t.stride(0)


def ln_affine(x: torch.Tensor, a: torch.Tensor, b: torch.Tensor, eps: float, out: Optional[torch.Tensor] = None,
              ab_rows: int = 0, ab_stride: int = 0):
    _dev(x, torch.bfloat16, "x"), _dev(a, torch.float32, "a"), _dev(b, torch.float32, "b")
    M, D, ldx = _rows(x, "x")
    if out is None:
        out = torch.empty((M, D), dtype=torch.bfloat16, device=x.device)
    _, _, ldy = _rows(out, "out")
    st = _prof_begin()
    _check(lib().ce_ln_affine_bf16(_ptr(x), _ptr(out), _ptr(a), _ptr(b), M, D, ldx, ldy, float(eps), int(ab_rows), int(ab_stride),
                                   _stream()), "ce_ln_affine_bf16")
    _prof_end(st, f"ln_affine_{M}x{D}", 4.0 * M * D)
    return out


def rmsnorm_rope_(x: torch.Tensor, w: torch.Tensor, cos_sin: Optional[torch.Tensor], head_dim: int, eps: float,
                  x2: Optional[torch.Tensor] = None, w2: Optional[torch.Tensor] = None):
    _dev(x, torch.bfloat16, "x"), _dev(w, torch.float32, "w")
    M, D, ld = _rows(x, "x")
    rope_rows = 0
    if cos_sin is not None:
        _dev(cos_sin, torch.float32, "cos_sin")
        assert cos_sin.is_contiguous() and cos_sin.shape[1:] == (head_dim // 2, 2) and M % cos_sin.shape[0] == 0, (cos_sin.shape, M)
        rope_rows = cos_sin.shape[0]
    if x2 is not None:
        _dev(x2, torch.bfloat16, "x2"), _dev(w2, torch.float32, "w2")
        assert _rows(x2, "x2") == (M, D, ld)
    st = _prof_begin()
    _check(lib().ce_rmsnorm_rope_bf16(_ptr(x), _ptr(w), _ptr(x2), _ptr(w2), _ptr(cos_sin), M, D, ld, head_dim, float(eps), rope_rows,
                                      _stream()), "ce_rmsnorm_rope_bf16")
    _prof_end(st, f"rmsnorm_rope_{M}x{D}" + ("x2" if x2 is not None else ""), (8.0 if x2 is not None else 4.0) * M * D)
    return x


def gemm(a: torch.Tensor, w: torch.Tensor, bias: Optional[torch.Tensor], out: Optional[torch.Tensor] = None,
         epilogue: int = EPI_BIAS, gate: Optional[torch.Tensor] = None, res: Optional[torch.Tensor] = None, gate_rows: int = 0):
    _dev(a, torch.bfloat16, "a"), _dev(w, torch.bfloat16, "w")
    a_seg_k, a_seg_stride = 0, 0
    if a.dim() == 3:
        S, M, Ks = a.shape
        if a.stride(2) != 1 or a.stride(1) < Ks:
            raise ValueError(f"gemm: segmented a needs unit inner stride, got {a.stride()}")
        K, lda, a_seg_k, a_seg_stride = S * Ks, a.stride(1), Ks, a.stride(0)
    else:
        M, K, lda = _rows(a, "a")
    N, K2, ldw = _rows(w, "w")
    if K != K2:
        raise ValueError(f"gemm: K mismatch {K} vs {K2}")
    if bias is not None:
        _dev(bias, torch.float32, "bias")
        assert bias.numel() == (M if epilogue == EPI_BIAS_ROW else N) and bias.is_contiguous()
    oshape = (N, M) if epilogue == EPI_BIAS_T else (M, N)
    if out is None:
        out = torch.empty(oshape, dtype=torch.bfloat16, device=a.device)
    _dev(out, torch.bfloat16, "out")
    Mo, No, ldc = _rows(out, "out")
    assert (Mo, No) == oshape, ((Mo, No), oshape)
    ldres = 0
    if epilogue in (EPI_GATE_RES, EPI_MUL):
        if res is None:
            raise ValueError("EPI_GATE_RES / EPI_MUL need res")
        _dev(res, torch.bfloat16, "res")
        _, _, ldres = _rows(res, "res")
        if gate is not None:
            _dev(gate, torch.float32, "gate")
            assert gate.is_contiguous() and gate.numel() == (N if gate_rows <= 0 else (M + gate_rows - 1) // gate_rows * N)
    ws, ws_bytes = _gemm_scratch(a.device)
    st = _prof_begin()
    _check(lib().ce_gemm_bf16(_ptr(a), _ptr(w), _ptr(out), _ptr(bias), epilogue, _ptr(gate), _ptr(res), M, N, K, lda, ldw, ldc, ldres,
                              int(gate_rows), int(a_seg_k), int(a_seg_stride), 0, 0, ws, ws_bytes, _stream()), "ce_gemm_bf16")
    _prof_end(st, f"gemm_{M}x{N}x{K}_epi{epilogue}", 2.0 * M * N * K)
    return out


def rope_scatter(x: torch.Tensor, cols, weights, D: int, world: int, cos_sin: Optional[torch.Tensor], head_dim: int, eps: float,
                 out: Optional[torch.Tensor] = None):
    _dev(x, torch.bfloat16, "x")
    M, _, ldx = _rows(x, "x")
    nt = len(cols)
    assert 1 <= nt <= 3 and len(weights) == nt
    for w in weights:
        if w is not None:
            _dev(w, torch.float32, "w")
            assert w.is_contiguous() and w.numel() == D
    rope_rows = 0
    if cos_sin is not None:
        _dev(cos_sin, torch.float32, "cos_sin")
        assert cos_sin.is_contiguous() and cos_sin.shape[1:] == (head_dim // 2, 2) and M % cos_sin.shape[0] == 0
        rope_rows = cos_sin.shape[0]
    if out is None:
        out = torch.empty((world, M, nt, D // world), dtype=torch.bfloat16, device=x.device)
    _dev(out, torch.bfloat16, "out")
    assert out.is_contiguous() and out.numel() == M * nt * D
    c = list(cols) + [0] * (3 - nt)
    w = list(weights) + [None] * (3 - nt)
    st = _prof_begin()
    _check(lib().ce_rope_scatter_bf16(_ptr(x), ldx, _ptr(out), M, D, world, nt, c[0], _ptr(w[0]), c[1], _ptr(w[1]), c[2], _ptr(w[2]),
                                      _ptr(cos_sin), head_dim, float(eps), rope_rows, _stream()), "ce_rope_scatter_bf16")
    _prof_end(st, f"rope_scatter_{M}x{D}x{nt}", 4.0 * M * D * nt)
    return out


_gemm_split = True
GEMM_WS_BYTES = 256 * 384 * 256 * 4


GEMM_WS_STREAMS = 8
_gemm_default = {}
_gemm_own = {}


def _gemm_scratch(device: torch.device):
    if not _gemm_split:
        return None, 0
    dev = device.index if device.index is not None else torch.cuda.current_device()
    stream = torch.cuda.current_stream(dev).cuda_stream
    first = _gemm_default.get(dev)
    if first is not None and first[0] == stream:
        buf = first[1]
    elif (dev, stream) in _gemm_own:
        buf = _gemm_own[(dev, stream)] = _gemm_own.pop((dev, stream))
    else:
        with torch.cuda.device(dev):
            capturing = torch.cuda.is_current_stream_capturing()
        if capturing:
            if first is None:
                return None, 0
            buf = first[1]
        elif first is None:
            buf = torch.empty(GEMM_WS_BYTES, dtype=torch.uint8, device=dev)
            _gemm_default[dev] = (stream, buf)
        else:
            mine = [k for k in _gemm_own if k[0] == dev]
            if len(mine) >= GEMM_WS_STREAMS:
                del _gemm_own[mine[0]]
            buf = _gemm_own[(dev, stream)] = torch.empty(GEMM_WS_BYTES, dtype=torch.uint8, device=dev)
    return buf.data_ptr(), buf.numel()


def set_gemm_split(on: bool) -> bool:
    global _gemm_split
    prev, _gemm_split = _gemm_split, bool(on)
    return prev


def set_gemm_variant(v: int) -> int:
    return _set_knob("ce_set_gemm_variant", v)


def set_attention_waves(n: int) -> int:
    return _set_knob("ce_set_attention_waves", n)


def attention(q: torch.Tensor, k: torch.Tensor, v: torch.Tensor, heads: int, out: Optional[torch.Tensor] = None,
              k2: Optional[torch.Tensor] = None, v2: Optional[torch.Tensor] = None, scale: Optional[float] = None,
              batch: int = 1):
    for n, t in (("q", q), ("k", k), ("v", v)):
        _dev(t, torch.bfloat16, n)
    Nq, Dq, ldq = _rows(q, "q")
    head_dim = Dq // heads
    L1, _, ldk = _rows(k, "k")
    L1v, _, ldv = _rows(v, "v")
    assert L1 == L1v
    if batch < 1 or Nq % batch or L1 % batch or (k2 is not None and k2.shape[0] % batch):
        raise ValueError(f"attention: row counts must be multiples of batch={batch}")
    if out is None:
        out = torch.empty((Nq, Dq), dtype=torch.bfloat16, device=q.device)
    _, _, ldo = _rows(out, "out")
    L2 = ldk2 = ldv2 = 0
    if k2 is not None:
        _dev(k2, torch.bfloat16, "k2"), _dev(v2, torch.bfloat16, "v2")
        L2, _, ldk2 = _rows(k2, "k2")
        _, _, ldv2 = _rows(v2, "v2")
    if scale is None:
        scale = head_dim ** -0.5
    st = _prof_begin()
    nq, l1, l2 = Nq // batch, L1 // batch, L2 // batch
    _check(lib().ce_attention_batched_bf16(_ptr(q), _ptr(k), _ptr(v), l1, ldk, ldv, _ptr(k2), _ptr(v2), l2, ldk2, ldv2, _ptr(out),
                                           nq, heads, head_dim, ldq, ldo, float(scale), batch, _stream()), "ce_attention_bf16")
    _prof_end(st, f"attention_{nq}x{l1}+{l2}_h{heads}" + (f"_b{batch}" if batch > 1 else ""),
              4.0 * nq * (l1 + l2) * head_dim * heads * batch)
    return out


def vt_columns(n_keys_total: int) -> int:
    return (n_keys_total + 63) // 64 * 64 + 64


def v_transpose(v: torch.Tensor, heads: int, out: Optional[torch.Tensor] = None):
    _dev(v, torch.bfloat16, "v")
    n, D, ldv = _rows(v, "v")
    assert D == heads * 128
    if out is None:
        out = torch.empty((D, vt_columns(n)), dtype=torch.bfloat16, device=v.device)
    _dev(out, torch.bfloat16, "vt")
    assert out.shape[0] == D and out.is_contiguous() and out.shape[1] >= n
    st = _prof_begin()
    _check(lib().ce_v_transpose_bf16(_ptr(v), ldv, _ptr(out), out.shape[1], n, heads, _stream()), "ce_v_transpose_bf16")
    _prof_end(st, f"v_transpose_{n}x{D}", 4.0 * n * D)
    return out


def attention_vt(q: torch.Tensor, k: torch.Tensor, vt: torch.Tensor, heads: int, out: Optional[torch.Tensor] = None,
                 scale: Optional[float] = None, batch: int = 1):
    for n, t in (("q", q), ("k", k), ("vt", vt)):
        _dev(t, torch.bfloat16, n)
    Nq, Dq, ldq = _rows(q, "q")
    L1, _, ldk = _rows(k, "k")
    assert Dq == heads * 128 and vt.shape[0] == Dq and vt.stride(1) == 1
    if batch < 1 or Nq % batch or L1 % batch:
        raise ValueError(f"attention_vt: row counts must be multiples of batch={batch}")
    if out is None:
        out = torch.empty((Nq, Dq), dtype=torch.bfloat16, device=q.device)
    _, _, ldo = _rows(out, "out")
    if scale is None:
        scale = 128 ** -0.5
    st = _prof_begin()
    nq, l1 = Nq // batch, L1 // batch
    _check(lib().ce_attention_vt_bf16(_ptr(q), _ptr(k), _ptr(vt), l1, ldk, vt.stride(0), _ptr(out), nq, heads, 128, ldq, ldo, float(scale),
                                      batch, _stream()), "ce_attention_vt_bf16")
    _prof_end(st, f"attention_{nq}x{l1}+0_h{heads}" + (f"_b{batch}" if batch > 1 else ""), 4.0 * nq * l1 * 128 * heads * batch)
    return out


def attention_2seg_vt(q: torch.Tensor, k1: torch.Tensor, v1t: torch.Tensor, len1: int, k2: torch.Tensor, v2t: torch.Tensor, len2: int,
                      heads: int, out: Optional[torch.Tensor] = None, scale: Optional[float] = None, batch: int = 1,
                      cols1: Optional[int] = None, cols2: Optional[int] = None, out8: Optional[torch.Tensor] = None,
                      scale8: Optional[torch.Tensor] = None):
    for n, t in (("q", q), ("k1", k1), ("v1t", v1t), ("k2", k2), ("v2t", v2t)):
        _dev(t, torch.bfloat16, n)
    Nq, Dq, ldq = _rows(q, "q")
    _, _, ldk1 = _rows(k1, "k1")
    _, _, ldk2 = _rows(k2, "k2")
    assert Dq == heads * 128 and v1t.shape[0] == Dq and v2t.shape[0] == Dq and v1t.stride(1) == 1 and v2t.stride(1) == 1
    assert Nq % batch == 0 and k1.shape[0] == batch * len1 and k2.shape[0] == batch * len2
    if cols1 is None:
        assert v1t.shape[1] % batch == 0
        cols1 = v1t.shape[1] // batch
    if cols2 is None:
        assert v2t.shape[1] % batch == 0
        cols2 = v2t.shape[1] // batch
    if scale is None:
        scale = 128 ** -0.5
    nq = Nq // batch
    if out8 is not None:
        _dev(out8, torch.uint8, "out8"), _dev(scale8, torch.uint8, "scale8")
        _, D8, ld8 = _rows(out8, "out8")
        assert out8.shape[0] == Nq and D8 == Dq and scale8.is_contiguous() and scale8.numel() >= mx_scale_bytes(Nq, Dq)
        st = _prof_begin()
        _check(lib().ce_attention_2seg_vt_quant_bf16(_ptr(q), _ptr(k1), _ptr(v1t), len1, ldk1, v1t.stride(0), int(cols1), _ptr(k2), _ptr(v2t),
                                                     len2, ldk2, v2t.stride(0), int(cols2), _ptr(out8), _ptr(scale8), nq, heads, 128, ldq, ld8,
                                                     float(scale), batch, _stream()), "ce_attention_2seg_vt_quant_bf16")
        _prof_end(st, f"attention_{nq}x{len1}+{len2}_h{heads}" + (f"_b{batch}" if batch > 1 else "") + "_mxq",
                  4.0 * nq * (len1 + len2) * 128 * heads * batch)
        return out8
    if out is None:
        out = torch.empty((Nq, Dq), dtype=torch.bfloat16, device=q.device)
    _, _, ldo = _rows(out, "out")
    st = _prof_begin()
    _check(lib().ce_attention_2seg_vt_bf16(_ptr(q), _ptr(k1), _ptr(v1t), len1, ldk1, v1t.stride(0), int(cols1), _ptr(k2), _ptr(v2t),
                                           len2, ldk2, v2t.stride(0), int(cols2), _ptr(out), nq, heads, 128, ldq, ldo,
                                           float(scale), batch, _stream()), "ce_attention_2seg_vt_bf16")
    _prof_end(st, f"attention_{nq}x{len1}+{len2}_h{heads}" + (f"_b{batch}" if batch > 1 else ""), 4.0 * nq * (len1 + len2) * 128 * heads * batch)
    return out


def v_transpose_blocked(v: torch.Tensor, heads: int, batch: int, blk_rows: int, n_keys: int, out: Optional[torch.Tensor] = None):
    _dev(v, torch.bfloat16, "v")
    rows, D, ldv = _rows(v, "v")
    assert D == heads * 128 and blk_rows % 64 == 0 and rows % (batch * blk_rows) == 0
    cols = (n_keys + 63) // 64 * 64 + 64
    if out is None:
        out = torch.empty((D, batch * cols), dtype=torch.bfloat16, device=v.device)
    assert out.shape == (D, batch * cols) and out.is_contiguous()
    st = _prof_begin()
    _check(lib().ce_v_transpose_blocked_bf16(_ptr(v), ldv, _ptr(out), out.shape[1], n_keys, heads, batch, blk_rows, batch * blk_rows, cols,
                                             _stream()), "ce_v_transpose_blocked_bf16")
    _prof_end(st, f"v_transpose_{batch * n_keys}x{D}", 4.0 * batch * n_keys * D)
    return out


def attention_vt_blocked(q: torch.Tensor, k: torch.Tensor, vt: torch.Tensor, heads: int, batch: int, blk_rows: int, n_keys: int,
                         out: Optional[torch.Tensor] = None, scale: Optional[float] = None):
    for n, t in (("q", q), ("k", k), ("vt", vt)):
        _dev(t, torch.bfloat16, n)
    rows, Dq, ldq = _rows(q, "q")
    rk, _, ldk = _rows(k, "k")
    assert Dq == heads * 128 and vt.shape[0] == Dq and vt.stride(1) == 1 and rows == rk and rows % (batch * blk_rows) == 0
    nq = rows // batch
    cols = vt.shape[1] // batch
    if out is None:
        out = torch.empty((rows, Dq), dtype=torch.bfloat16, device=q.device)
    _, _, ldo = _rows(out, "out")
    if scale is None:
        scale = 128 ** -0.5
    st = _prof_begin()
    _check(lib().ce_attention_vt_blocked_bf16(_ptr(q), _ptr(k), _ptr(vt), n_keys, ldk, vt.stride(0), _ptr(out), nq, heads, 128, ldq, ldo,
                                              float(scale), batch, blk_rows, batch * blk_rows, cols, _stream()), "ce_attention_vt_blocked_bf16")
    _prof_end(st, f"attention_{nq}x{n_keys}+0_h{heads}" + (f"_b{batch}" if batch > 1 else ""), 4.0 * nq * n_keys * 128 * heads * batch)
    return out


def timestep_sinusoid(t: torch.Tensor, dim: int, out: Optional[torch.Tensor] = None):
    if t.dtype == torch.float32:
        _dev(t, torch.float32, "timestep")
    else:
        _dev(t, torch.int64, "timestep")
    if out is None:
        out = torch.empty((dim,), dtype=torch.float32, device=t.device)
    if t.dtype == torch.float32:
        _check(lib().ce_timestep_sinusoid_f32(_ptr(t), _ptr(out), dim, _stream()), "ce_timestep_sinusoid_f32")
    else:
        _check(lib().ce_timestep_sinusoid(_ptr(t), _ptr(out), dim, _stream()), "ce_timestep_sinusoid")
    return out


def gemv(w: torch.Tensor, x: torch.Tensor, bias: Optional[torch.Tensor], flags: int = 0, out: Optional[torch.Tensor] = None):
    _dev(x, torch.float32, "x")
    assert w.is_cuda and w.dtype in (torch.float32, torch.bfloat16) and w.is_contiguous()
    N, K = w.shape
    assert x.numel() == K
    if bias is not None:
        _dev(bias, torch.float32, "bias")
    if out is None:
        out = torch.empty((N,), dtype=torch.float32, device=x.device)
    _check(lib().ce_gemv(_ptr(w), int(w.dtype == torch.bfloat16), _ptr(x), _ptr(bias), _ptr(out), N, K, flags, _stream()), "ce_gemv")
    return out


def modulation(table: torch.Tensor, v: torch.Tensor, one_mask: int, out: Optional[torch.Tensor] = None):
    _dev(table, torch.float32, "table"), _dev(v, torch.float32, "v")
    L, J, D = table.shape
    v_rows = v.numel() // D
    assert table.is_contiguous() and v.is_contiguous() and v_rows in (1, J)
    if out is None:
        out = torch.empty_like(table)
    _check(lib().ce_modulation(_ptr(table), _ptr(v), _ptr(out), L, J, D, v_rows, one_mask, _stream()), "ce_modulation")
    return out


def patchify(x: torch.Tensor, kpad: int, out: Optional[torch.Tensor] = None, row0: int = 0, nrows: Optional[int] = None):
    _dev(x, torch.bfloat16, "x")
    assert x.is_contiguous() and x.dim() == 4
    C, T, H, W = x.shape
    n = T * (H // 2) * (W // 2) if nrows is None else int(nrows)
    if out is None:
        out = torch.empty((n, kpad), dtype=torch.bfloat16, device=x.device)
    assert out.is_contiguous() and out.shape == (n, kpad)
    _check(lib().ce_patchify_rows_bf16(_ptr(x), _ptr(out), C, T, H, W, kpad, int(row0), n, _stream()), "ce_patchify_rows_bf16")
    return out


def unpatchify(y: torch.Tensor, cout: int, T: int, H: int, W: int, out: Optional[torch.Tensor] = None):
    _dev(y, torch.bfloat16, "y")
    _, _, ldy = _rows(y, "y")
    if out is None:
        out = torch.empty((cout, T, H, W), dtype=torch.bfloat16, device=y.device)
    _check(lib().ce_unpatchify_bf16(_ptr(y), _ptr(out), cout, T, H, W, ldy, _stream()), "ce_unpatchify_bf16")
    return out


def cfg_unipc_step(v_cond: torch.Tensor, v_uncond: Optional[torch.Tensor], x: torch.Tensor, x_last: torch.Tensor, m0: torch.Tensor,
                   m1: torch.Tensor, coef: torch.Tensor, x0_out: Optional[torch.Tensor] = None, round_sigma_v: bool = True,
                   bf16_state: bool = False):
    _dev(v_cond, torch.bfloat16, "v_cond")
    for n, t in (("x", x), ("x_last", x_last), ("m0", m0), ("m1", m1), ("coef", coef)):
        _dev(t, torch.float32, n)
        assert t.is_contiguous()
    if v_uncond is not None:
        _dev(v_uncond, torch.bfloat16, "v_uncond")
        assert v_uncond.is_contiguous()
    assert v_cond.is_contiguous() and coef.numel() >= 10
    n = x.numel()
    assert v_cond.numel() == n == x_last.numel() == m0.numel() == m1.numel()
    _check(lib().ce_cfg_unipc_step(_ptr(v_cond), _ptr(v_uncond), _ptr(x), _ptr(x_last), _ptr(m0), _ptr(m1), _ptr(x0_out), _ptr(coef),
                                   _ptr(None), n, int(round_sigma_v) | (2 if bf16_state else 0), _stream()), "ce_cfg_unipc_step")
    return x


def conv3d_gemm(in_stack: torch.Tensor, weight: torch.Tensor, bias: Optional[torch.Tensor], out_stack: torch.Tensor,
                res_stack: Optional[torch.Tensor], *, T_out: int, H: int, W: int, Cin: int, Cout: int, KT: int, n_tile: int = 0):
    _dev(in_stack, torch.bfloat16, "in_stack")
    _dev(out_stack, torch.bfloat16, "out_stack")
    _dev(weight, torch.bfloat16, "weight")
    assert in_stack.is_contiguous() and out_stack.is_contiguous() and weight.is_contiguous() and weight.dim() == 2
    assert in_stack.shape[0] >= T_out + KT and tuple(in_stack.shape[1:]) == (H + 2, W + 2, Cin), in_stack.shape
    assert out_stack.shape[0] >= T_out and tuple(out_stack.shape[1:3]) == (H + 2, W + 2), out_stack.shape
    if res_stack is not None:
        _dev(res_stack, torch.bfloat16, "res_stack")
        assert res_stack.is_contiguous() and res_stack.shape[1:] == out_stack.shape[1:] and res_stack.shape[0] >= T_out
    st_ev = _prof_begin()
    _check(lib().ce_conv3d_gemm_bf16(_ptr(in_stack), _ptr(weight), weight.shape[1], _ptr(bias), _ptr(out_stack), _ptr(res_stack), T_out, H, W,
                                     Cin, Cout, KT, out_stack.shape[3], n_tile, _stream()), "ce_conv3d_gemm_bf16")
    _prof_end(st_ev, f"conv_{KT}x3x3_{Cin}->{Cout}_{T_out}x{H}x{W}", 2.0 * T_out * H * W * Cout * Cin * KT * 9)


def conv3d_gemm_rms_silu(in_stack: torch.Tensor, weight: torch.Tensor, bias: Optional[torch.Tensor], normed_stack: torch.Tensor, gamma: torch.Tensor, *,
                         T_out: int, H: int, W: int, Cin: int, Cout: int, KT: int, silu: bool = True, out_stack: Optional[torch.Tensor] = None,
                         res_stack: Optional[torch.Tensor] = None):
    _dev(in_stack, torch.bfloat16, "in_stack")
    _dev(normed_stack, torch.bfloat16, "normed_stack")
    _dev(weight, torch.bfloat16, "weight")
    _dev(gamma, torch.float32, "gamma")
    assert in_stack.is_contiguous() and normed_stack.is_contiguous() and weight.is_contiguous() and weight.dim() == 2 and gamma.numel() == Cout
    assert in_stack.shape[0] >= T_out + KT and tuple(in_stack.shape[1:]) == (H + 2, W + 2, Cin), in_stack.shape
    assert normed_stack.shape[0] >= T_out and tuple(normed_stack.shape[1:3]) == (H + 2, W + 2), normed_stack.shape
    for t, nm in ((out_stack, "out_stack"), (res_stack, "res_stack")):
        if t is not None:
            _dev(t, torch.bfloat16, nm)
            assert t.is_contiguous() and t.shape[1:] == normed_stack.shape[1:] and t.shape[0] >= T_out, (nm, t.shape)
    assert res_stack is None or out_stack is not None
# ... 498 lines not shown
```

### chronoedit_amd/transformer.py

```python
from __future__ import annotations

import inspect
import math
import re
from dataclasses import dataclass
from types import SimpleNamespace
from typing import Any, Dict, Optional, Tuple, Union

import torch
import torch.nn as nn

from . import ops, weights
from .weights import LoraMixin


_VT_GEMM_SWAPPED = __import__("os").environ.get("CE_VT_GEMM") == "row"


@dataclass
class Transformer2DModelOutput:
    sample: torch.Tensor


class _Config(SimpleNamespace):
    def __getitem__(self, k):
        return getattr(self, k)

    def get(self, k, d=None):
        return getattr(self, k, d)


class RMSNormParams(nn.Module):

    def __init__(self, dim: int, eps: float, device=None, dtype=None):
        super().__init__()
        self.eps = eps
        self.weight = nn.Parameter(torch.ones(dim, device=device, dtype=dtype))


class AttentionParams(nn.Module):

    def __init__(self, dim: int, heads: int, eps: float, added_kv_proj_dim: Optional[int], device=None, dtype=None):
        super().__init__()
        kw = dict(device=device, dtype=dtype)
        self.heads = heads
        self.to_q = nn.Linear(dim, dim, **kw)
        self.to_k = nn.Linear(dim, dim, **kw)
        self.to_v = nn.Linear(dim, dim, **kw)
        self.to_out = nn.ModuleList([nn.Linear(dim, dim, **kw), nn.Dropout(0.0)])
        self.norm_q = RMSNormParams(dim, eps, **kw)
        self.norm_k = RMSNormParams(dim, eps, **kw)
        self.add_k_proj = self.add_v_proj = self.norm_added_k = None
        if added_kv_proj_dim is not None:
            self.add_k_proj = nn.Linear(added_kv_proj_dim, dim, **kw)
            self.add_v_proj = nn.Linear(added_kv_proj_dim, dim, **kw)
            self.norm_added_k = RMSNormParams(dim, eps, **kw)


class _GELUProj(nn.Module):
    def __init__(self, din, dout, device=None, dtype=None):
        super().__init__()
        self.proj = nn.Linear(din, dout, device=device, dtype=dtype)


class FeedForwardParams(nn.Module):

    def __init__(self, dim, inner, dim_out=None, device=None, dtype=None):
        super().__init__()
        self.net = nn.ModuleList([
            _GELUProj(dim, inner, device=device, dtype=dtype),
            nn.Dropout(0.0),
            nn.Linear(inner, dim_out if dim_out is not None else dim, device=device, dtype=dtype),
        ])


class BlockParams(nn.Module):

    def __init__(self, dim, ffn_dim, heads, cross_attn_norm, eps, added_kv_proj_dim, device=None, dtype=None):
        super().__init__()
        self.attn1 = AttentionParams(dim, heads, eps, None, device=device, dtype=dtype)
        self.attn2 = AttentionParams(dim, heads, eps, added_kv_proj_dim, device=device, dtype=dtype)
        self.norm2 = nn.LayerNorm(dim, eps, elementwise_affine=True, device=device, dtype=torch.float32) if cross_attn_norm else nn.Identity()
        self.ffn = FeedForwardParams(dim, ffn_dim, device=device, dtype=dtype)
        self.scale_shift_table = nn.Parameter(torch.randn(1, 6, dim, device=device, dtype=torch.float32) / dim**0.5)


class _TimestepEmbedding(nn.Module):
    def __init__(self, din, dim, device=None):
        super().__init__()
        self.linear_1 = nn.Linear(din, dim, device=device, dtype=torch.float32)
        self.linear_2 = nn.Linear(dim, dim, device=device, dtype=torch.float32)


class _TextProjection(nn.Module):
    def __init__(self, din, dim, device=None, dtype=None):
        super().__init__()
        self.linear_1 = nn.Linear(din, dim, device=device, dtype=dtype)
        self.linear_2 = nn.Linear(dim, dim, device=device, dtype=dtype)


class _ImageEmbedding(nn.Module):
    def __init__(self, din, dout, device=None, dtype=None):
        super().__init__()
        self.norm1 = nn.LayerNorm(din, device=device, dtype=torch.float32)
        self.ff = FeedForwardParams(din, din, dout, device=device, dtype=dtype)
        self.norm2 = nn.LayerNorm(dout, device=device, dtype=torch.float32)


class ConditionEmbedderParams(nn.Module):

    def __init__(self, dim, time_freq_dim, time_proj_dim, text_embed_dim, image_embed_dim, device=None, dtype=None):
        super().__init__()
        self.time_embedder = _TimestepEmbedding(time_freq_dim, dim, device=device)
        self.time_proj = nn.Linear(dim, time_proj_dim, device=device, dtype=dtype)
        self.text_embedder = _TextProjection(text_embed_dim, dim, device=device, dtype=dtype)
        self.image_embedder = None
        if image_embed_dim is not None:
            self.image_embedder = _ImageEmbedding(image_embed_dim, dim, device=device, dtype=dtype)


import itertools

_GENERATION = itertools.count(1)


class ChronoEditTransformer3DModel(LoraMixin, nn.Module):

    _supports_gradient_checkpointing = False
    _no_split_modules = ["BlockParams"]
    _keep_in_fp32_modules = ["time_embedder", "scale_shift_table", "norm1", "norm2", "norm3"]
    _keys_to_ignore_on_load_unexpected = ["norm_added_q"]

    def __init__(
        self,
        patch_size: Tuple[int, int, int] = (1, 2, 2),
        num_attention_heads: int = 40,
        attention_head_dim: int = 128,
        in_channels: int = 16,
        out_channels: int = 16,
        text_dim: int = 4096,
        freq_dim: int = 256,
        ffn_dim: int = 13824,
        num_layers: int = 40,
        cross_attn_norm: bool = True,
        qk_norm: Optional[str] = "rms_norm_across_heads",
        eps: float = 1e-6,
        image_dim: Optional[int] = None,
        added_kv_proj_dim: Optional[int] = None,
        rope_max_seq_len: int = 1024,
        rope_temporal_skip_len: int = 8,
        device=None,
        dtype: torch.dtype = torch.bfloat16,
    ) -> None:
        super().__init__()
        if qk_norm != "rms_norm_across_heads":
            raise NotImplementedError("only qk_norm='rms_norm_across_heads' (the ChronoEdit/Wan setting) is supported")
        if tuple(patch_size) != (1, 2, 2):
            raise NotImplementedError("patch_size must be (1, 2, 2)")
        if attention_head_dim != 128:
            raise NotImplementedError("the gfx950 attention kernel is specialised for head_dim 128")
        self.config = _Config(
            patch_size=tuple(patch_size), num_attention_heads=num_attention_heads, attention_head_dim=attention_head_dim,
            in_channels=in_channels, out_channels=out_channels or in_channels, text_dim=text_dim, freq_dim=freq_dim,
            ffn_dim=ffn_dim, num_layers=num_layers, cross_attn_norm=cross_attn_norm, qk_norm=qk_norm, eps=eps,
            image_dim=image_dim, added_kv_proj_dim=added_kv_proj_dim, rope_max_seq_len=rope_max_seq_len,
            rope_temporal_skip_len=rope_temporal_skip_len,
        )
        inner = num_attention_heads * attention_head_dim
        kw = dict(device=device, dtype=dtype)
        self.patch_embedding = nn.Conv3d(in_channels, inner, kernel_size=patch_size, stride=patch_size, **kw)
        self.condition_embedder = ConditionEmbedderParams(inner, freq_dim, inner * 6, text_dim, image_dim, **kw)
        self.blocks = nn.ModuleList(
            [BlockParams(inner, ffn_dim, num_attention_heads, cross_attn_norm, eps, added_kv_proj_dim, **kw) for _ in range(num_layers)]
        )
        self.proj_out = nn.Linear(inner, self.config.out_channels * math.prod(patch_size), **kw)
        self.scale_shift_table = nn.Parameter(torch.randn(1, 2, inner, device=device, dtype=torch.float32) / inner**0.5)
        self._engine: Optional["DiTEngine"] = None
        self._gen = next(_GENERATION)
        self.cache_context = False
        self.gemm_dtype = "bf16"
        self.fp8_linears = self.FP8_LINEARS
        self.attn_dtype = "bf16"
        self.v_transposed = True
        self.sp_batch_cfg = True
        self.fp8_fuse_quant = True
        self.fp8_fuse_attn_quant = True
        self.cross_vt = True
        self._sp = None
        self._cfgp = None

    @property
    def dtype(self) -> torch.dtype:
        return self.proj_out.weight.dtype

    @property
    def device(self) -> torch.device:
        return self.proj_out.weight.device

    @classmethod
    def from_pretrained(cls, path: str, subfolder: Optional[str] = None, torch_dtype: torch.dtype = torch.bfloat16,
                        device=None, **unused) -> "ChronoEditTransformer3DModel":
        cfg = weights.read_config(path, subfolder)
        known = set(inspect.signature(cls.__init__).parameters) - {"self", "device", "dtype"}
        model = cls(**{k: v for k, v in cfg.items() if k in known}, device=device, dtype=torch_dtype)
        sd = weights.load_state_dict_files(weights.shard_files(path, subfolder))
        weights.assign_state_dict(model, sd, ignore_unexpected=cls._keys_to_ignore_on_load_unexpected)
        model.invalidate()
        return model

    def load_wan_native_state_dict(self, sd: Dict[str, torch.Tensor]):
        renamed = weights.wan_native_to_diffusers(sd, [k for k, _ in self.named_parameters()])
        weights.assign_state_dict(self, renamed, ignore_unexpected=self._keys_to_ignore_on_load_unexpected)
        self.invalidate()
        return self

    def wan_native_state_dict(self) -> Dict[str, torch.Tensor]:
        return {weights.diffusers_to_wan_native_key(k): p.detach() for k, p in self.named_parameters()}

    def save_pretrained(self, path: str, max_shard_bytes: int = 5 << 30):
        return weights.save_pretrained(self, path, dict(vars(self.config)), max_shard_bytes, "ChronoEditTransformer3DModel")

    def load_synthetic_(self, params: Dict[str, torch.Tensor]):
        own = dict(self.named_parameters())
        missing = set(own) - set(params)
        extra = set(params) - set(own)
        if missing or extra:
            raise KeyError(f"state mismatch: missing {sorted(missing)[:4]} unexpected {sorted(extra)[:4]}")
        with torch.no_grad():
            for k, p in own.items():
                p.copy_(params[k].to(p.dtype))
        self.invalidate()
        return self

    def enable_sequence_parallel(self, group=None, force: bool = False, owned_comm: bool = False):
        from .parallel import Ulysses
        self._sp = Ulysses(group, force=force, owned_comm=owned_comm)
        if self.config.num_attention_heads % self._sp.world:
            raise ValueError(f"{self.config.num_attention_heads} heads do not divide over {self._sp.world} ranks")
        if self._engine is not None:
            self._engine._ws = {}
            self._engine.ws_generation += 1
        return self

    def enable_cfg_parallel(self):
        from .parallel import CFGParallel, Ulysses
        self._cfgp = CFGParallel()
        self._sp = Ulysses(self._cfgp.sp_group)
        if self.config.num_attention_heads % self._sp.world:
            raise ValueError(f"{self.config.num_attention_heads} heads do not divide over {self._sp.world} ranks")
        if self._engine is not None:
            self._engine._ws = {}
            self._engine.ws_generation += 1
        return self

    def clear_context_cache(self):
        if self._engine is not None:
            self._engine.clear_context_cache()

    @torch.no_grad()
    def prime_context(self, encoder_hidden_states: torch.Tensor, encoder_hidden_states_image: Optional[torch.Tensor]):
        if self.cache_context:
            self.engine()._context(encoder_hidden_states, encoder_hidden_states_image)

    def invalidate(self):
        self._engine = None

    FP8_LINEARS = ("qkv", "o1", "q2", "o2", "f1", "f2")
    FP8_POLICIES = {"fast": ("qkv", "o1", "q2", "o2", "f1", "f2"), "accurate": ("qkv", "o1", "q2", "f1", "f2")}

    def enable_fp8_gemms(self, on: bool = True, mx: bool = True, linears=None, policy: Optional[str] = None):
        if policy is not None:
            if linears is not None:
                raise ValueError("enable_fp8_gemms: give `linears` or `policy`, not both")
            if policy not in self.FP8_POLICIES:
                raise ValueError(f"enable_fp8_gemms: unknown policy {policy!r} (one of {sorted(self.FP8_POLICIES)})")
            linears = self.FP8_POLICIES[policy]
        linears = tuple(self.FP8_LINEARS if linears is None else linears)
        bad = [n for n in linears if n not in self.FP8_LINEARS]
        if bad:
            raise ValueError(f"enable_fp8_gemms: unknown Linear name(s) {bad} (of {self.FP8_LINEARS})")
        self.fp8_linears = tuple(n for n in self.FP8_LINEARS if n in linears)
        self.gemm_dtype = ("mxfp8" if mx else "fp8") if (on and self.fp8_linears) else "bf16"
        self._engine = None
        return self

    def enable_transposed_v(self, on: bool = True):
        self.v_transposed = bool(on)
        if self._engine is not None:
            self._engine.v_transposed = self.v_transposed
            self._engine._ws = {}
            self._engine.ws_generation += 1
        return self

    def enable_cross_vt(self, on: bool = True):
        self.cross_vt = bool(on)
        self._engine = None
        return self

    def enable_fp8_attention(self, on: bool = True, cross: bool = False):
        self.attn_dtype = "mxfp8" if on else "bf16"
        self.fp8_cross = bool(on and cross)
        self._engine = None
        return self

    def attention_path(self) -> str:
        sharded = self._sp is not None and self._sp.sharded
        return "mxfp8" if (self.attn_dtype == "mxfp8" and not sharded) else "bf16"

    def _apply(self, fn, *a, **kw):
        self._engine = None
        out = super()._apply(fn, *a, **kw)
        self._lora_moved(fn)
        return out

    def load_state_dict(self, *a, **kw):
        self._engine = None
        return super().load_state_dict(*a, **kw)

    _LORA_SLOTS = {"attn1.to_q": "qkv", "attn1.to_k": "qkv", "attn1.to_v": "qkv", "attn1.to_out.0": "o1", "attn2.to_q": "q2", "attn2.to_out.0": "o2",
                   "ffn.net.0.proj": "f1", "ffn.net.2": "f2", "attn2.to_k": "k_t", "attn2.to_v": "v_t", "attn2.add_k_proj": "k_i", "attn2.add_v_proj": "v_i"}
    _LORA_CONTEXT_SLOTS = ("k_t", "v_t", "k_i", "v_i")

    def _lora_weights_changed(self, modules):
        eng = self._engine
        if eng is None:
            return
        own = dict(self.named_modules())
        requant, context = set(), False
        for m in modules:
            mt = re.match(r"^blocks\.(\d+)\.(.+)$", m)
            slot = self._LORA_SLOTS.get(mt.group(2)) if mt else None
            if slot is None:
                return self.invalidate()
            li = int(mt.group(1))
            op = getattr(eng, f"w_{slot}_all", None) if slot in self._LORA_CONTEXT_SLOTS else getattr(eng.blk[li], "w_" + slot, None)
            if op is None or op.untyped_storage().data_ptr() != own[m].weight.untyped_storage().data_ptr():
                return self.invalidate()
            context |= slot in self._LORA_CONTEXT_SLOTS
            if slot in eng.fp8_set:
                requant.add((li, slot))
        for li, slot in sorted(requant):
            p = eng.blk[li]
            q, s = getattr(p, "q_" + slot)
            (ops.quant_rows_mxfp8(getattr(p, "w_" + slot), out=q, scale=s, w_order=True) if eng.mx else
             ops.quant_rows_fp8(getattr(p, "w_" + slot), out=q, scale=s))
        if context:
            eng.clear_context_cache()

    def engine(self) -> "DiTEngine":
        rt = getattr(self, "_lora_rt", None)
        if rt is not None and rt.dirty:
            self._lora_apply()
        if self._engine is None:
            self._engine = DiTEngine(self)
            self._gen = next(_GENERATION)
        return self._engine

    def engine_generation(self):
        eng = self._engine
        sp = self._sp
        return (self._gen, None if eng is None else eng.ws_generation, self.gemm_dtype, self.fp8_linears, self.attn_dtype, self.v_transposed, self.cross_vt,
                self.sp_batch_cfg, bool(getattr(self, "rope_plain_temporal", False)), self.cache_context,
                None if sp is None else (sp.world, sp.rank), self._cfgp is not None)

    @torch.no_grad()
    def forward(
        self,
        hidden_states: torch.Tensor,
        timestep: torch.LongTensor,
        encoder_hidden_states: torch.Tensor,
        encoder_hidden_states_image: Optional[torch.Tensor] = None,
        return_dict: bool = True,
        attention_kwargs: Optional[Dict[str, Any]] = None,
    ) -> Union[Transformer2DModelOutput, Tuple[torch.Tensor]]:
        if not hidden_states.is_cuda:
            raise ops.HipKernelError("ChronoEditTransformer3DModel (chronoedit_amd) runs only on an MI355X device: "
                                     "there is no CPU fallback (use oracle/ for CPU reference numbers)")
        B = hidden_states.shape[0]
        ts = timestep.reshape(-1)
        if ts.numel() == 1 and B > 1:
            ts = ts.expand(B)
        output = self.engine().forward(hidden_states, ts, encoder_hidden_states, encoder_hidden_states_image).to(hidden_states.dtype)
        if not return_dict:
            return (output,)
        return Transformer2DModelOutput(sample=output)


def rope_cos_sin(head_dim: int, max_len: int, skip_len: int, T: int, Hp: int, Wp: int, theta: float = 10000.0,
                 plain_temporal: bool = False) -> torch.Tensor:
    assert plain_temporal or T == 2 or T == skip_len, f"num_frames must be 2 or {skip_len}, but got {T}"
    h_dim = w_dim = 2 * (head_dim // 6)
    t_dim = head_dim - h_dim - w_dim

    def ang(dim, idx):
        f = 1.0 / (theta ** (torch.arange(0, dim, 2, dtype=torch.float64)[: dim // 2] / dim))
        return torch.outer(idx.to(torch.float64), f)

    t_idx = torch.tensor([0, skip_len - 1]) if (T == 2 and not plain_temporal) else torch.arange(T)
    assert max(T, Hp, Wp, skip_len) <= max_len
    a_t = ang(t_dim, t_idx).view(T, 1, 1, -1).expand(T, Hp, Wp, -1)
    a_h = ang(h_dim, torch.arange(Hp)).view(1, Hp, 1, -1).expand(T, Hp, Wp, -1)
    a_w = ang(w_dim, torch.arange(Wp)).view(1, 1, Wp, -1).expand(T, Hp, Wp, -1)
    a = torch.cat([a_t, a_h, a_w], dim=-1).reshape(T * Hp * Wp, head_dim // 2)
    return torch.stack([torch.cos(a), torch.sin(a)], dim=-1).to(torch.float32).contiguous()


def _pad_k(w: torch.Tensor, mult: int = 64) -> torch.Tensor:
    K = w.shape[1]
    Kp = (K + mult - 1) // mult * mult
    if Kp == K:
        return w.contiguous()
    out = torch.zeros((w.shape[0], Kp), dtype=w.dtype, device=w.device)
    out[:, :K] = w
    return out


def _pad_n(w: torch.Tensor, b: Optional[torch.Tensor], mult: int = 8):
    N = w.shape[0]
    Np = (N + mult - 1) // mult * mult
    if Np == N:
        return w, b
    w2 = torch.zeros((Np, w.shape[1]), dtype=w.dtype, device=w.device)
    w2[:N] = w
    b2 = None
    if b is not None:
        b2 = torch.zeros((Np,), dtype=b.dtype, device=b.device)
        b2[:N] = b
    return w2, b2


class DiTEngine:

    def __init__(self, model: ChronoEditTransformer3DModel):
        cfg = model.config
        self.cfg = cfg
        self.model = model
        dev = model.device
        if dev.type != "cuda":
            raise ops.HipKernelError("DiTEngine needs the model on the GPU")
        if model.dtype != torch.bfloat16:
            raise TypeError("the HIP path computes in bf16 (run_inference_diffusers.py hard-codes bf16, :344-362); "
                            f"got model dtype {model.dtype}")
        self.dev = dev
        self.D = cfg.num_attention_heads * cfg.attention_head_dim
        self.H = cfg.num_attention_heads
        self.F = cfg.ffn_dim
        self.L = cfg.num_layers
        f32 = lambda t: t.detach().to(torch.float32).contiguous()
        ce = model.condition_embedder

        self.kpatch = (cfg.in_channels * 4 + 63) // 64 * 64
        self.w_patch = _pad_k(model.patch_embedding.weight.detach().reshape(self.D, -1))
        self.b_patch = f32(model.patch_embedding.bias)

        self.te_w1, self.te_b1 = ce.time_embedder.linear_1.weight.detach().contiguous(), f32(ce.time_embedder.linear_1.bias)
        self.te_w2, self.te_b2 = ce.time_embedder.linear_2.weight.detach().contiguous(), f32(ce.time_embedder.linear_2.bias)
        self.tp_w, self.tp_b = ce.time_proj.weight.detach().contiguous(), f32(ce.time_proj.bias)

        self.tx_w1, self.tx_b1 = _pad_k(ce.text_embedder.linear_1.weight.detach()), f32(ce.text_embedder.linear_1.bias)
        self.tx_w2, self.tx_b2 = ce.text_embedder.linear_2.weight.detach().contiguous(), f32(ce.text_embedder.linear_2.bias)
        self.has_image = ce.image_embedder is not None
        if self.has_image:
            ie = ce.image_embedder
            self.im_n1 = (f32(ie.norm1.weight), f32(ie.norm1.bias), ie.norm1.eps)
            self.im_w1, self.im_b1 = _pad_k(ie.ff.net[0].proj.weight.detach()), f32(ie.ff.net[0].proj.bias)
            self.im_w2, self.im_b2 = _pad_k(ie.ff.net[2].weight.detach()), f32(ie.ff.net[2].bias)
            self.im_n2 = (f32(ie.norm2.weight), f32(ie.norm2.bias), ie.norm2.eps)

        self.blk = []
        tables = []
        for blk in model.blocks:
            p = SimpleNamespace()
            a1, a2 = blk.attn1, blk.attn2
            p.w_qkv = self._fuse([a1.to_q, a1.to_k, a1.to_v])
            p.b_qkv = torch.cat([f32(a1.to_q.bias), f32(a1.to_k.bias), f32(a1.to_v.bias)])
            p.nq1, p.nk1 = f32(a1.norm_q.weight), f32(a1.norm_k.weight)
            p.w_o1, p.b_o1 = a1.to_out[0].weight.detach().contiguous(), f32(a1.to_out[0].bias)
            p.w_q2, p.b_q2 = a2.to_q.weight.detach().contiguous(), f32(a2.to_q.bias)
            p.nq2, p.nk2 = f32(a2.norm_q.weight), f32(a2.norm_k.weight)
            p.has_img = a2.add_k_proj is not None
            if p.has_img:
                p.nk_i = f32(a2.norm_added_k.weight)
            p.w_o2, p.b_o2 = a2.to_out[0].weight.detach().contiguous(), f32(a2.to_out[0].bias)
            if cfg.cross_attn_norm:
                p.n2w, p.n2b = f32(blk.norm2.weight), f32(blk.norm2.bias)
            else:
                p.n2w = p.n2b = None
            p.w_f1, p.b_f1 = blk.ffn.net[0].proj.weight.detach().contiguous(), f32(blk.ffn.net[0].proj.bias)
            p.w_f2, p.b_f2 = blk.ffn.net[2].weight.detach().contiguous(), f32(blk.ffn.net[2].bias)
            tables.append(f32(blk.scale_shift_table).reshape(6, self.D))
            self.blk.append(p)
        self.fp8_attn = model.attn_dtype == "mxfp8"
        self.fp8_cross = self.fp8_attn and bool(getattr(model, "fp8_cross", False))
        self.fp8 = model.gemm_dtype in ("fp8", "mxfp8")
        self.mx = model.gemm_dtype == "mxfp8"
        self.fp8_set = frozenset(getattr(model, "fp8_linears", model.FP8_LINEARS)) if self.fp8 else frozenset()
        self.fuse_quant = bool(getattr(model, "fp8_fuse_quant", True)) and self.F % 128 == 0
        self.fuse_attn_quant = self.fuse_quant and bool(getattr(model, "fp8_fuse_attn_quant", True))
        self.v_transposed = bool(getattr(model, "v_transposed", True))
        if self.fp8:
            if self.D % 256 or self.F % 256:
                raise NotImplementedError("fp8 GEMMs need inner and ffn dims that are multiples of 256")
            for p in self.blk:
                for name in sorted(self.fp8_set):
                    w = getattr(p, "w_" + name)
                    setattr(p, "q_" + name, ops.quant_rows_mxfp8(w, w_order=True) if self.mx else ops.quant_rows_fp8(w))
        self.w_k_t_all = self._fuse([blk.attn2.to_k for blk in model.blocks])
        self.b_k_t_all = torch.cat([f32(blk.attn2.to_k.bias) for blk in model.blocks])
        self.w_v_t_all = self._fuse([blk.attn2.to_v for blk in model.blocks])
        self.b_v_t_all = torch.cat([f32(blk.attn2.to_v.bias) for blk in model.blocks])
        self.all_img = all(p.has_img for p in self.blk)
        if self.all_img:
            self.w_k_i_all = self._fuse([blk.attn2.add_k_proj for blk in model.blocks])
            self.b_k_i_all = torch.cat([f32(blk.attn2.add_k_proj.bias) for blk in model.blocks])
            self.w_v_i_all = self._fuse([blk.attn2.add_v_proj for blk in model.blocks])
            self.b_v_i_all = torch.cat([f32(blk.attn2.add_v_proj.bias) for blk in model.blocks])
        self.cross_vt = bool(getattr(model, "cross_vt", True))
        self._ctx_bufs = {}
        self.tables = torch.stack(tables, 0).contiguous()
        self.table_out = f32(model.scale_shift_table).reshape(1, 2, self.D)
        self.w_out, self.b_out = _pad_n(model.proj_out.weight.detach().contiguous(), f32(model.proj_out.bias))
        self.ones = torch.ones(self.D, dtype=torch.float32, device=dev)
        self.zeros = torch.zeros(self.D, dtype=torch.float32, device=dev)
        self._rope = {}
        self._ws = {}
        self.ws_generation = 0
        self._ctx_key = None
        self._ctx = None
        self._ctx_refs = None

    def _fuse(self, linears) -> torch.Tensor:
        w = torch.cat([l.weight.detach() for l in linears], dim=0).contiguous()
        o = 0
        for l in linears:
            n = l.weight.shape[0]
            l.weight.data = w[o : o + n]
            o += n
        return w

    def _ln_linear(self, ws, x: torch.Tensor, a_row, b_row, p, name: str, out: torch.Tensor, ab_rows: int = 0, ab_stride: int = 0, **kw):
        eps = self.cfg.eps
        if name not in self.fp8_set:
            ops.ln_affine(x, a_row, b_row, eps, out=ws.h, ab_rows=ab_rows, ab_stride=ab_stride)
            return ops.gemm(ws.h, getattr(p, "w_" + name), getattr(p, "b_" + name), out=out, **kw)
        aq = ws.a8[:, : x.shape[1]]
        wq, sw = getattr(p, "q_" + name)
        if self.mx:
            ops.ln_affine_mxfp8(x, a_row, b_row, eps, out=aq, scale=ws.s8, ab_rows=ab_rows, ab_stride=ab_stride)
            return ops.gemm_mxfp8(aq, ws.s8, wq, sw, getattr(p, "b_" + name), out=out, **kw)
        ops.ln_affine_fp8(x, a_row, b_row, eps, out=aq, scale=ws.s8, ab_rows=ab_rows, ab_stride=ab_stride)
        return ops.gemm_fp8(aq, ws.s8, wq, sw, getattr(p, "b_" + name), out=out, **kw)

    def _linear(self, ws, a: torch.Tensor, p, name: str, out: torch.Tensor, quantised: bool = False, **kw):
        w, b = getattr(p, "w_" + name), getattr(p, "b_" + name)
        if name not in self.fp8_set:
            assert not quantised, name
            return ops.gemm(a, w, b, out=out, **kw)
        K = a.shape[1]
        aq = ws.a8[:, :K]
        wq, sw = getattr(p, "q_" + name)
        if self.mx:
            if not quantised:
                ops.quant_rows_mxfp8(a, out=aq, scale=ws.s8)
            return ops.gemm_mxfp8(aq, ws.s8, wq, sw, b, out=out, **kw)
        ops.quant_rows_fp8(a, out=aq, scale=ws.s8)
        return ops.gemm_fp8(aq, ws.s8, wq, sw, b, out=out, **kw)

    def _self_attention_ulysses(self, ws, sp, x, a_row, b_row, p, cs, N: int, Nl: int, B: int = 1):
        D, H, hd, eps, W = self.D, self.H, self.cfg.attention_head_dim, self.cfg.eps, sp.world
        Dl = D // W
        if "qkv" not in self.fp8_set:
            ops.ln_affine(x, a_row, b_row, eps, out=ws.h, ab_rows=Nl, ab_stride=6 * D)
            lin = lambda lo, hi, out: ops.gemm(ws.h, p.w_qkv[lo:hi], p.b_qkv[lo:hi], out=out)
        else:
            aq = ws.a8[:, :D]
            wq, sw = p.q_qkv
            if self.mx:
                ops.ln_affine_mxfp8(x, a_row, b_row, eps, out=aq, scale=ws.s8, ab_rows=Nl, ab_stride=6 * D)
                sblk = (D // 128) * 512
                lin = lambda lo, hi, out: ops.gemm_mxfp8(aq, ws.s8, wq[lo:hi], sw[lo // 128 * sblk: hi // 128 * sblk], p.b_qkv[lo:hi], out=out)
            else:
                ops.ln_affine_fp8(x, a_row, b_row, eps, out=aq, scale=ws.s8, ab_rows=Nl, ab_stride=6 * D)
                lin = lambda lo, hi, out: ops.gemm_fp8(aq, ws.s8, wq[lo:hi], sw[lo:hi], p.b_qkv[lo:hi], out=out)
        lin(D, 3 * D, ws.qkv[:, D:])
        ops.rope_scatter(ws.qkv, (D, 2 * D), (p.nk1, None), D, W, cs, hd, eps, out=ws.send_kv)
        _, wait_kv = sp.all_to_all(ws.send_kv, ws.recv_kv, async_op=True)
        lin(0, D, ws.qkv[:, :D])
        ops.rope_scatter(ws.qkv, (0,), (p.nq1,), D, W, cs, hd, eps, out=ws.send_q)
        _, wait_q = sp.all_to_all(ws.send_q, ws.recv_q, async_op=True)
        wait_kv.wait()
        wait_q.wait()
        kv = sp.gathered_view(ws.recv_kv)
        if B > 1:
            vt_shape = (Dl, B * ops.vt_columns(N))
            ws.vt_sp = ops.v_transpose_blocked(kv[:, Dl:], H // W, B, Nl, N, out=ws.vt_sp if getattr(ws, "vt_sp", torch.empty(0)).shape == vt_shape else None)
            ops.attention_vt_blocked(sp.gathered_view(ws.recv_q), kv[:, :Dl], ws.vt_sp, H // W, B, Nl, N, out=ws.att_g)
        elif self.v_transposed:
            if getattr(ws, "vt_sp", None) is None or ws.vt_sp.shape != (Dl, ops.vt_columns(N)):
                ws.vt_sp = torch.zeros((Dl, ops.vt_columns(N)), dtype=torch.bfloat16, device=self.dev)
            ops.v_transpose(kv[:N, Dl:], H // W, out=ws.vt_sp)
            ops.attention_vt(sp.gathered_view(ws.recv_q), kv[:N, :Dl], ws.vt_sp, H // W, out=ws.att_g)
        else:
            ops.attention(sp.gathered_view(ws.recv_q), kv[:N, :Dl], kv[:N, Dl:], H // W, out=ws.att_g)
        y, _ = sp.all_to_all(ws.att_g.view(W, B * Nl, Dl), ws.att_seg)
        if "o1" in self.fp8_set:
            ws.att.copy_(sp.merge_heads_reference(y))
            return ws.att
        return y

    def _workspace(self, N: int):
        ws = self._ws.get(N)
        if ws is None:
            D, F, dev = self.D, self.F, self.dev
            e = lambda *s: torch.empty(s, dtype=torch.bfloat16, device=dev)
            ws = SimpleNamespace(x=e(N, D), h=e(N, D), qkv=e(N, 3 * D), att=e(N, D), q2=e(N, D), ffn=e(N, F),
                                 cols=e(N, self.kpatch), head=e(N, self.w_out.shape[0]))
            if self.fp8:
                ws.a8 = torch.empty((N, max(D, F)), dtype=torch.uint8, device=dev)
                ws.s8 = (torch.empty((ops.mx_scale_bytes(N, max(D, F)),), dtype=torch.uint8, device=dev) if self.mx else
                         torch.empty((N,), dtype=torch.float32, device=dev))
                if self.mx and self.fuse_quant and F % 128 == 0:
                    ws.a8b = torch.empty((N, F), dtype=torch.uint8, device=dev)
                    ws.s8b = torch.empty((ops.mx_scale_bytes(N, F),), dtype=torch.uint8, device=dev)
            if self.fp8_attn:
                u8 = lambda *s: torch.empty(s, dtype=torch.uint8, device=dev)
                ws.q8, ws.k8, ws.sq, ws.sk = u8(N, D), u8(N, D), u8(N, D // 32), u8(N, D // 32)
                ws.v8t = ws.sv = None
            sp = self.model._sp
            if sp is not None and sp.sharded:
                W, Dl = sp.world, D // sp.world
                ws.send_kv, ws.recv_kv = e(W, N, 2, Dl), e(W, N, 2, Dl)
                ws.send_q, ws.recv_q = e(W, N, 1, Dl), e(W, N, 1, Dl)
                ws.att_g, ws.att_seg = e(W * N, Dl), e(W, N, Dl)
            if len(self._ws) > 1:
                self.ws_generation += 1
            keep = list(self._ws.items())[-1:]
            self._ws = dict(keep + [(N, ws)])
        return ws

    def _rope_table(self, T, Hp, Wp):
        plain = bool(getattr(self.model, "rope_plain_temporal", False))
        key = (T, Hp, Wp, plain)
        if key not in self._rope:
            c = self.cfg
            if len(self._rope) >= 4:
                self._rope.pop(next(iter(self._rope)))
            self._rope[key] = rope_cos_sin(c.attention_head_dim, c.rope_max_seq_len, c.rope_temporal_skip_len, T, Hp, Wp,
                                           plain_temporal=plain).to(self.dev)
        return self._rope[key]

    def is_warm(self, B: int, T: int, Hh: int, Ww: int) -> bool:
        plain = bool(getattr(self.model, "rope_plain_temporal", False))
        N = T * (Hh // 2) * (Ww // 2)
        return (B * N) in self._ws and (T, Hh // 2, Ww // 2, plain) in self._rope

    def _context(self, text: torch.Tensor, image: Optional[torch.Tensor]):
        key = None
        if self.model.cache_context:
            key = (text.data_ptr(), text._version, tuple(text.shape), text.dtype,
                   None if image is None else (image.data_ptr(), image._version, tuple(image.shape), image.dtype))
            if key == self._ctx_key:
                return self._ctx
        keyed = (text, image)
        D = self.D
        B, Tt = text.shape[0], text.shape[1]
        text = text.to(torch.bfloat16).reshape(B * Tt, -1)
        if text.shape[1] != self.tx_w1.shape[1]:
            tp = torch.zeros((text.shape[0], self.tx_w1.shape[1]), dtype=torch.bfloat16, device=self.dev)
            tp[:, : text.shape[1]] = text
            text = tp
        t1 = ops.gemm(text.contiguous(), self.tx_w1, self.tx_b1, epilogue=ops.EPI_BIAS_GELU)
        enc_t = ops.gemm(t1, self.tx_w2, self.tx_b2)
        enc_i = None
        Ti = 0
        if image is not None:
            if not self.has_image:
                raise ValueError("encoder_hidden_states_image given but the model has no image_embedder (image_dim=None)")
            Ti = image.shape[1]
            image = image.to(torch.bfloat16).reshape(B * Ti, -1).contiguous()
            w, b, eps = self.im_n1
            h = ops.ln_affine(image, w, b, eps)
            if h.shape[1] != self.im_w1.shape[1]:
                hp = torch.zeros((h.shape[0], self.im_w1.shape[1]), dtype=torch.bfloat16, device=self.dev)
                hp[:, : h.shape[1]] = h
                h = hp
            h = ops.gemm(h, self.im_w1, self.im_b1, epilogue=ops.EPI_BIAS_GELU_ERF)
            if h.shape[1] != self.im_w2.shape[1]:
                hp = torch.zeros((h.shape[0], self.im_w2.shape[1]), dtype=torch.bfloat16, device=self.dev)
                hp[:, : h.shape[1]] = h
                h = hp
            h_img = ops.gemm(h, self.im_w2, self.im_b2)
            w, b, eps = self.im_n2
            enc_i = ops.ln_affine(h_img, w, b, eps)
        eps = self.cfg.eps
        hd = self.cfg.attention_head_dim
        L = self.L
        f8 = self.fp8_cross and (self.model._sp is None or not self.model._sp.sharded) and getattr(self.model, "_cfgp", None) is None
        use_vt = self.cross_vt and enc_i is not None and self.all_img and Tt % 8 == 0 and not f8
        k_t_all = ops.gemm(enc_t, self.w_k_t_all, self.b_k_t_all)
        k_i_all = v_t_all = v_i_all = v1t = v2t = None
        c1 = c2 = 0
        if enc_i is not None and self.all_img:
            k_i_all = ops.gemm(enc_i, self.w_k_i_all, self.b_k_i_all)
        if use_vt:
            c1, c2 = Tt, (Ti + 7) // 8 * 8
            ld1 = ((B - 1) * c1 + (Tt + 63) // 64 * 64 + 7) // 8 * 8
            ld2 = ((B - 1) * c2 + (Ti + 63) // 64 * 64 + 7) // 8 * 8
            bufs = self._ctx_bufs.get((B, Tt, Ti))
            if bufs is None:
                z = lambda *sh: torch.zeros(sh, dtype=torch.bfloat16, device=self.dev)
                bufs = SimpleNamespace(enc_i_pad=z(B * c2, D), v1t=z(L * D, ld1), v2t=z(L * D, ld2))
                self._ctx_bufs = dict(list(self._ctx_bufs.items())[-1:] + [((B, Tt, Ti), bufs)])
            v1t, v2t = bufs.v1t, bufs.v2t
            self._ctx_key = self._ctx = self._ctx_refs = None
            w, b, eps_i = self.im_n2
            for bi in range(B):
                ops.ln_affine(h_img[bi * Ti:(bi + 1) * Ti], w, b, eps_i, out=bufs.enc_i_pad[bi * c2: bi * c2 + Ti])
            ops.gemm(self.w_v_t_all, enc_t, self.b_v_t_all, out=v1t[:, : B * Tt], epilogue=ops.EPI_BIAS_ROW)
            ops.gemm(self.w_v_i_all, bufs.enc_i_pad, self.b_v_i_all, out=v2t[:, : B * c2], epilogue=ops.EPI_BIAS_ROW)
        else:
            v_t_all = ops.gemm(enc_t, self.w_v_t_all, self.b_v_t_all)
            if k_i_all is not None:
                v_i_all = ops.gemm(enc_i, self.w_v_i_all, self.b_v_i_all)
        kv = []
        for li, p in enumerate(self.blk if not f8 else ()):
            cols = slice(li * D, (li + 1) * D)
            k_t = k_t_all[:, cols]
            ops.rmsnorm_rope_(k_t, p.nk2, None, hd, eps)
            k_i = None
            if k_i_all is not None:
                k_i = k_i_all[:, cols]
                ops.rmsnorm_rope_(k_i, p.nk_i, None, hd, eps)
            if use_vt:
                kv.append((k_t, v1t[cols], k_i, v2t[cols]))
            else:
                kv.append((k_t, v_t_all[:, cols], k_i, None if v_i_all is None else v_i_all[:, cols]))
        if f8:
            for li, p in enumerate(self.blk):
                cols = slice(li * D, (li + 1) * D)
                seg_t = ops.rmsnorm_rope_mxfp8(k_t_all[:, cols], p.nk2, None, hd, eps) + ops.v_mxfp8_transpose(v_t_all[:, cols], Tt, B, self.H)
                seg_i = None
                if k_i_all is not None:
                    seg_i = ops.rmsnorm_rope_mxfp8(k_i_all[:, cols], p.nk_i, None, hd, eps) + ops.v_mxfp8_transpose(v_i_all[:, cols], Ti, B, self.H)
                kv.append((seg_t, seg_i))
        ctx = SimpleNamespace(kv=kv, Tt=Tt, Ti=Ti, vt=use_vt, c1=c1, c2=c2, f8=f8)
        if key is not None:
            self._ctx_key, self._ctx, self._ctx_refs = key, ctx, keyed
        return ctx

    def clear_context_cache(self):
        self._ctx_key = self._ctx = self._ctx_refs = None

    def forward(self, hidden: torch.Tensor, timestep: torch.Tensor, text: torch.Tensor, image: Optional[torch.Tensor]):
        cfg, D, H = self.cfg, self.D, self.H
        B, C, T, Hh, Ww = hidden.shape
        if C != cfg.in_channels:
            raise ValueError(f"expected {cfg.in_channels} input channels, got {C}")
        Hp, Wp = Hh // 2, Ww // 2
        N = T * Hp * Wp
        hd = cfg.attention_head_dim
        eps = cfg.eps
        cs = self._rope_table(T, Hp, Wp)
        sp = self.model._sp
        if sp is not None and sp.sharded:
            if B != 1 and not self.v_transposed:
                raise ValueError("several samples per sequence-parallel forward need the V^T attention path (enable_transposed_v)")
            if self.fp8_attn and not getattr(self, "_warned_fp8_attn_sp", False):
                import warnings
                warnings.warn("enable_fp8_attention() has no effect while the tokens are sharded (Ulysses / CFG parallel): the exchange "
                              "carries bf16 q / k / v and the self-attention runs the bf16 V^T kernel; see attention_path()")
                self._warned_fp8_attn_sp = True
            align = 64 if B > 1 else 1
            Nl = sp.shard(N, align)[0]
            key = ("sp", T, Hp, Wp, sp.rank, sp.world, Nl)
            if key not in self._rope:
                self._rope[key] = sp.take_rows(cs, N, align).contiguous()
            cs = self._rope[key]
        else:
            sp = None
            Nl = N
        ws = self._workspace(B * Nl)
        hidden = hidden.to(torch.bfloat16).contiguous()
        timestep = timestep.to(device=self.dev, dtype=torch.float32 if timestep.is_floating_point() else torch.int64).contiguous()
        rows = [slice(b * Nl, (b + 1) * Nl) for b in range(B)]

        if sp is None:
            for b in range(B):
                ops.patchify(hidden[b], self.kpatch, out=ws.cols[rows[b]])
        else:
            for b in range(B):
                ops.patchify(hidden[b], self.kpatch, out=ws.cols[rows[b]], row0=sp.rank * Nl, nrows=Nl)
        ops.gemm(ws.cols, self.w_patch, self.b_patch, out=ws.x)

        mods, gates1, gates2, mods_out = [], [], [], []
        for b in range(B):
            sin = ops.timestep_sinusoid(timestep[b : b + 1], cfg.freq_dim)
            h1 = ops.gemv(self.te_w1, sin, self.te_b1, flags=2)
            temb = ops.gemv(self.te_w2, h1, self.te_b2, flags=4)
            tproj = ops.gemv(self.tp_w, temb, self.tp_b, flags=1 | 4)
            mods.append(ops.modulation(self.tables, tproj.view(6, D), one_mask=0b010010))
            mods_out.append(ops.modulation(self.table_out, temb.view(1, D), one_mask=0b10))
        mod = torch.stack(mods, dim=1).contiguous()
        mod_out = torch.stack(mods_out, dim=0).contiguous()
        if B > 1:
            gate_msa = mod[:, :, 2].contiguous()
            gate_ffn = mod[:, :, 5].contiguous()

        if text.shape[0] != B or (image is not None and image.shape[0] != B):
            raise ValueError("encoder_hidden_states / encoder_hidden_states_image batch size must match hidden_states")
        ctx = self._context(text, image)
        Tt, Ti = ctx.Tt, ctx.Ti
        grow = Nl if B > 1 else 0

        x = ws.x
        fuse_o = self.mx and self.fuse_attn_quant and D % 128 == 0
        fuse_o1, fuse_o2 = fuse_o and "o1" in self.fp8_set, fuse_o and "o2" in self.fp8_set
        for li, p in enumerate(self.blk):
            q_o1 = False
            if sp is None and self.fp8_attn:
                self._ln_linear(ws, x, mod[li, 0, 1], mod[li, 0, 0], p, "qkv", ws.qkv, ab_rows=Nl, ab_stride=6 * D)
                ops.rmsnorm_rope_mxfp8(ws.qkv[:, :D], p.nq1, cs, hd, eps, out=ws.q8, scale=ws.sq, post_scale=ops.MXFP8_Q_SCALE)
                ops.rmsnorm_rope_mxfp8(ws.qkv[:, D : 2 * D], p.nk1, cs, hd, eps, out=ws.k8, scale=ws.sk)
                if ws.v8t is None or ws.v8t.shape[0] != B:
                    ws.v8t = ws.sv = None
                ws.v8t, ws.sv = ops.v_mxfp8_transpose(ws.qkv[:, 2 * D :], Nl, B, H, out=ws.v8t, scale=ws.sv)
                if fuse_o1:
                    ops.attention_mxfp8(ws.q8, ws.sq, ws.k8, ws.sk, ws.v8t, ws.sv, H, batch=B, out8=ws.a8[:, :D], scale8=ws.s8)
                    q_o1 = True
                else:
                    ops.attention_mxfp8(ws.q8, ws.sq, ws.k8, ws.sk, ws.v8t, ws.sv, H, out=ws.att, batch=B)
                att = ws.att
            elif sp is None and self.v_transposed and "qkv" not in self.fp8_set and (B * Nl) % 8 == 0 and (B == 1 or Nl % 2 == 0):
                if getattr(ws, "vt", None) is None:
                    ws.vt = torch.zeros((D, ops.vt_columns(B * Nl)), dtype=torch.bfloat16, device=self.dev)
                ops.ln_affine(x, mod[li, 0, 1], mod[li, 0, 0], eps, out=ws.h, ab_rows=Nl, ab_stride=6 * D)
                ops.gemm(ws.h, p.w_qkv[: 2 * D], p.b_qkv[: 2 * D], out=ws.qkv[:, : 2 * D])
                if _VT_GEMM_SWAPPED:
                    ops.gemm(p.w_qkv[2 * D :], ws.h, p.b_qkv[2 * D :], out=ws.vt[:, : B * Nl], epilogue=ops.EPI_BIAS_ROW)
                else:
                    ops.gemm(ws.h, p.w_qkv[2 * D :], p.b_qkv[2 * D :], out=ws.vt[:, : B * Nl], epilogue=ops.EPI_BIAS_T)
                ops.rmsnorm_rope_(ws.qkv[:, :D], p.nq1, cs, hd, eps, x2=ws.qkv[:, D : 2 * D], w2=p.nk1)
                ops.attention_vt(ws.qkv[:, :D], ws.qkv[:, D : 2 * D], ws.vt, H, out=ws.att, batch=B)
                att = ws.att
            elif sp is None:
                self._ln_linear(ws, x, mod[li, 0, 1], mod[li, 0, 0], p, "qkv", ws.qkv, ab_rows=Nl, ab_stride=6 * D)
                ops.rmsnorm_rope_(ws.qkv[:, :D], p.nq1, cs, hd, eps, x2=ws.qkv[:, D : 2 * D], w2=p.nk1)
                ops.attention(ws.qkv[:, :D], ws.qkv[:, D : 2 * D], ws.qkv[:, 2 * D :], H, out=ws.att, batch=B)
                att = ws.att
            else:
                att = self._self_attention_ulysses(ws, sp, x, mod[li, 0, 1], mod[li, 0, 0], p, cs, N, Nl, B)
            self._linear(ws, att, p, "o1", x, quantised=q_o1, epilogue=ops.EPI_GATE_RES, gate=gate_msa[li] if B > 1 else mods[0][li, 2],
                         res=x, gate_rows=grow)
            if p.n2w is not None:
                self._ln_linear(ws, x, p.n2w, p.n2b, p, "q2", ws.q2)
            else:
                self._linear(ws, x, p, "q2", ws.q2)
            q_o2 = bool(ctx.vt and fuse_o2)
            if ctx.f8:
                seg_t, seg_i = ctx.kv[li]
                ops.rmsnorm_rope_mxfp8(ws.q2, p.nq2, None, hd, eps, out=ws.q8, scale=ws.sq, post_scale=ops.MXFP8_Q_SCALE)
                if seg_i is None and fuse_o2:
                    ops.attention_mxfp8(ws.q8, ws.sq, *seg_t, H, batch=B, out8=ws.a8[:, :D], scale8=ws.s8)
                else:
                    ops.attention_mxfp8(ws.q8, ws.sq, *seg_t, H, out=ws.att, batch=B)
                    if seg_i is not None and fuse_o2:
                        ops.attention_mxfp8(ws.q8, ws.sq, *seg_i, H, batch=B, out8=ws.a8[:, :D], scale8=ws.s8, add=ws.att)
                    elif seg_i is not None:
                        ops.attention_mxfp8(ws.q8, ws.sq, *seg_i, H, out=ws.att, batch=B, add=ws.att)
                q_o2 = fuse_o2
                self._linear(ws, ws.att, p, "o2", x, quantised=q_o2, epilogue=ops.EPI_GATE_RES, gate=None, res=x)
                k_t = None
            else:
                ops.rmsnorm_rope_(ws.q2, p.nq2, None, hd, eps)
                k_t, v_t, k_i, v_i = ctx.kv[li]
            if k_t is None:
                pass
            elif ctx.vt and fuse_o2:
                ops.attention_2seg_vt(ws.q2, k_t, v_t, Tt, k_i, v_i, Ti, H, batch=B, cols1=ctx.c1, cols2=ctx.c2, out8=ws.a8[:, :D], scale8=ws.s8)
            elif ctx.vt:
                ops.attention_2seg_vt(ws.q2, k_t, v_t, Tt, k_i, v_i, Ti, H, out=ws.att, batch=B, cols1=ctx.c1, cols2=ctx.c2)
            elif k_i is not None:
                ops.attention(ws.q2, k_t, v_t, H, out=ws.att, k2=k_i, v2=v_i, batch=B)
            else:
                ops.attention(ws.q2, k_t, v_t, H, out=ws.att, batch=B)
            if k_t is not None:
                self._linear(ws, ws.att, p, "o2", x, quantised=q_o2, epilogue=ops.EPI_GATE_RES, gate=None, res=x)
            if self.mx and self.fuse_quant and "f1" in self.fp8_set and "f2" in self.fp8_set:
                aq = ws.a8[:, :D]
                ops.ln_affine_mxfp8(x, mod[li, 0, 4], mod[li, 0, 3], eps, out=aq, scale=ws.s8, ab_rows=Nl, ab_stride=6 * D)
                ops.gemm_mxfp8_gelu_quant(aq, ws.s8, *p.q_f1, p.b_f1, out=ws.a8b, scale=ws.s8b)
                ops.gemm_mxfp8(ws.a8b, ws.s8b, *p.q_f2, p.b_f2, out=x, epilogue=ops.EPI_GATE_RES,
                               gate=gate_ffn[li] if B > 1 else mods[0][li, 5], res=x, gate_rows=grow)
            else:
                self._ln_linear(ws, x, mod[li, 0, 4], mod[li, 0, 3], p, "f1", ws.ffn, ab_rows=Nl, ab_stride=6 * D, epilogue=ops.EPI_BIAS_GELU)
                self._linear(ws, ws.ffn, p, "f2", x, epilogue=ops.EPI_GATE_RES, gate=gate_ffn[li] if B > 1 else mods[0][li, 5],
                             res=x, gate_rows=grow)

        ops.ln_affine(x, mod_out[0, 0, 1], mod_out[0, 0, 0], eps, out=ws.h, ab_rows=Nl, ab_stride=2 * D)
        ops.gemm(ws.h, self.w_out, self.b_out, out=ws.head)
        out = torch.empty((B, cfg.out_channels, T, Hh, Ww), dtype=torch.bfloat16, device=self.dev)
        if sp is None:
            for b in range(B):
                ops.unpatchify(ws.head[rows[b]], cfg.out_channels, T, Hh, Ww, out=out[b])
        else:
            full = sp.all_gather_rows(ws.head).view(sp.world, B, Nl, -1)
            for b in range(B):
                ops.unpatchify(full[:, b].reshape(sp.world * Nl, -1)[:N].contiguous(), cfg.out_channels, T, Hh, Ww, out=out[b])
        return out
```

### include/chronoedit_hip.h

```cpp
#ifndef CHRONOEDIT_HIP_H
#define CHRONOEDIT_HIP_H

#include <stddef.h>
#include <stdint.h>

#ifdef __cplusplus
extern "C" {
#endif

#ifndef __HIP_PLATFORM_AMD__
typedef struct ihipStream_t* hipStream_t;
#endif

#define CE_OK 0
#define CE_ERR_ARG (-1)
#define CE_ERR_SHAPE (-2)
#define CE_ERR_ALIGN (-3)

#define CE_EPI_BIAS 0
#define CE_EPI_BIAS_GELU 1
#define CE_EPI_GATE_RES 2
#define CE_EPI_BIAS_GELU_ERF 3
#define CE_EPI_BIAS_ROW 6
#define CE_EPI_BIAS_T 7
#define CE_EPI_F32 4

int ce_ln_affine_bf16(const void* x, void* y, const float* a, const float* b, int M, int D, int ldx, int ldy, float eps,
                      int ab_rows, int ab_stride, hipStream_t stream);

int ce_rmsnorm_rope_bf16(void* x, const float* w, void* x2, const float* w2, const float* cos_sin, int M, int D, int ld,
                         int head_dim, float eps, int rope_rows, hipStream_t stream);

int ce_gemm_bf16(const void* A, const void* W, void* C, const float* bias, int epilogue, const float* gate, const void* res,
                 int M, int N, int K, int lda, int ldw, int ldc, int ldres, int gate_rows, int a_seg_k, long long a_seg_stride,
                 int w_seg_k, long long w_seg_stride, void* ws, size_t ws_bytes, hipStream_t stream);



int ce_gemm_bf16_tile_rows(int M, int N, int K, int cus, long long ws_bytes);

int ce_attention_bf16(const void* Q, const void* K1, const void* V1, int len1, int ldk1, int ldv1, const void* K2,
                      const void* V2, int len2, int ldk2, int ldv2, void* O, int Nq, int H, int head_dim, int ldq, int ldo,
                      float softmax_scale, hipStream_t stream);

int ce_attention_batched_bf16(const void* Q, const void* K1, const void* V1, int len1, int ldk1, int ldv1, const void* K2,
                              const void* V2, int len2, int ldk2, int ldv2, void* O, int Nq, int H, int head_dim, int ldq,
                              int ldo, float softmax_scale, int batch, hipStream_t stream);

int ce_attention_vt_bf16(const void* Q, const void* K, const void* Vt, int len, int ldk, int ldvt, void* O, int Nq, int H, int head_dim,
                         int ldq, int ldo, float softmax_scale, int batch, hipStream_t stream);

int ce_attention_2seg_vt_bf16(const void* Q, const void* K1, const void* V1t, int len1, int ldk1, int ldv1t, int vt_cols1, const void* K2,
                              const void* V2t, int len2, int ldk2, int ldv2t, int vt_cols2, void* O, int Nq, int H, int head_dim, int ldq,
                              int ldo, float softmax_scale, int batch, hipStream_t stream);

int ce_attention_2seg_vt_quant_bf16(const void* Q, const void* K1, const void* V1t, int len1, int ldk1, int ldv1t, int vt_cols1, const void* K2,
                                    const void* V2t, int len2, int ldk2, int ldv2t, int vt_cols2, void* o8, void* scale8, int Nq, int H,
                                    int head_dim, int ldq, int ldo8, float softmax_scale, int batch, hipStream_t stream);

int ce_attention_vt_blocked_bf16(const void* Q, const void* K, const void* Vt, int len, int ldk, int ldvt, void* O, int Nq, int H, int head_dim,
                                 int ldq, int ldo, float softmax_scale, int batch, int blk_rows, int blk_stride, int vt_sample_cols,
                                 hipStream_t stream);

int ce_v_transpose_blocked_bf16(const void* v, int ldv, void* vt, int ldvt, int n_keys, int H, int batch, int blk_rows, int blk_stride,
                                int vt_sample_cols, hipStream_t stream);

int ce_v_transpose_bf16(const void* v, int ldv, void* vt, int ldvt, int n_keys, int H, hipStream_t stream);


int ce_timestep_sinusoid(const int64_t* t, float* out, int dim, hipStream_t stream);

int ce_timestep_sinusoid_f32(const float* t, float* out, int dim, hipStream_t stream);

int ce_gemv(const void* W, int w_is_bf16, const float* x, const float* bias, float* y, int N, int K, int flags,
            hipStream_t stream);

int ce_modulation(const float* table, const float* v, float* mod, int L, int J, int D, int v_rows, int one_mask,
                  hipStream_t stream);

int ce_patchify_bf16(const void* x, void* cols, int C, int T, int H, int W, int Kpad, hipStream_t stream);

int ce_patchify_rows_bf16(const void* x, void* cols, int C, int T, int H, int W, int Kpad, int row0, int nrows, hipStream_t stream);

int ce_rope_scatter_bf16(const void* x, int ldx, void* send, int M, int D, int W, int nt, int col0, const float* w0, int col1,
                         const float* w1, int col2, const float* w2, const float* cos_sin, int head_dim, float eps,
                         int rope_rows, hipStream_t stream);

int ce_unpatchify_bf16(const void* y, void* out, int Cout, int T, int H, int W, int ldy, hipStream_t stream);

int ce_cfg_unipc_step(const void* v_cond, const void* v_uncond, float* x, float* x_last, float* m0, float* m1,
                      float* x0_out, const float* coef, const void* reserved, long long n, int flags, hipStream_t stream);


int ce_conv_igemm_bf16(const void* const* in_frames, int n_in_frames, const void* weight, const float* bias,
                       void* const* out_frames, int n_out_frames, const void* const* res_frames, int Cin, int Cout, int KT,
                       int KH, int KW, int st, int ss, int H_out, int W_out, int in_Wp, int in_off_h, int in_off_w, int out_Wp,
                       int out_border, int out_cstride, int out_coff, hipStream_t stream);

int ce_conv3d_head_bf16(const void* const* in_frames, int n_in_frames, const void* weight, const float* bias, void* const* out_frames,
                        int n_out_frames, int Cin, int Cout, int KT, int H_out, int W_out, int in_Wp, int out_Wp, int out_border,
                        int out_cstride, int out_coff, hipStream_t stream);

int ce_conv3d_gemm_bf16(const void* in_stack, const void* weight, int ldw, const float* bias, void* out_stack, const void* res_stack,
                        int T_out, int H, int W, int Cin, int Cout, int KT, int out_cstride, int n_tile, hipStream_t stream);

int ce_conv3d_gemm_rms_silu_bf16(const void* in_stack, const void* weight, int ldw, const float* bias, void* out_stack, const void* res_stack,
                                 void* normed_stack, int T_out, int H, int W, int Cin, int Cout, int KT, int out_cstride, const float* gamma,
                                 int apply_silu, hipStream_t stream);

int ce_rms_silu_bf16(const void* x, void* y, const float* gamma, long long npix, int C, int H, int W, int in_border,
                     int out_border, int apply_silu, hipStream_t stream);

int ce_zero_border_bf16(void* frames, int T, int H, int W, int C, int ld, hipStream_t stream);

int ce_upsample2x_bf16(const void* x, void* y, int T, int C, int H, int W, hipStream_t stream);

int ce_attention_1head_bf16(const void* Q, const void* K, const void* Vt, void* O, int Nq, int Nk, int C, int ldq, int ldk, int ldvt,
                            int ldo, float softmax_scale, void* ws, long long ws_bytes, hipStream_t stream);

int ce_softmax_rows_f32_bf16(const float* scores, void* probs, int M, int n, int npad, int ld, int ldp, float scale,
                             hipStream_t stream);


int ce_quant_rows_fp8(const void* x, void* q, float* scale, int M, int K, int ldx, int ldq, hipStream_t stream);

int ce_ln_affine_fp8(const void* x, void* q, float* scale, const float* a, const float* b, int M, int D, int ldx, int ldq, float eps,
                     int ab_rows, int ab_stride, hipStream_t stream);

int ce_gemm_fp8(const void* Aq, const void* Wq, void* C, const float* sa, const float* sw, const float* bias, int epilogue,
                const float* gate, const void* res, int M, int N, int K, int lda, int ldw, int ldc, int ldres, int gate_rows,
                void* ws, size_t ws_bytes, hipStream_t stream);


int ce_quant_rows_mxfp8(const void* x, void* q, void* scale8, int M, int K, int ldx, int ldq, hipStream_t stream);

int ce_quant_rows_mxfp8_w(const void* x, void* q, void* scale8, int M, int K, int ldx, int ldq, hipStream_t stream);

int ce_ln_affine_mxfp8(const void* x, void* q, void* scale8, const float* a, const float* b, int M, int D, int ldx, int ldq, float eps,
                       int ab_rows, int ab_stride, hipStream_t stream);

int ce_gemm_mxfp8(const void* Aq, const void* Wq, void* C, const void* sa8, const void* sw8, const float* bias, int epilogue, const float* gate,
                  const void* res, int M, int N, int K, int lda, int ldw, int ldc, int ldres, int gate_rows, void* ws, size_t ws_bytes,
                  hipStream_t stream);

int ce_gemm_mxfp8_gelu_quant(const void* Aq, const void* Wq, const void* sa8, const void* sw8, const float* bias, void* q_out, void* qs_out,
                             int M, int N, int K, int lda, int ldw, int ldq, void* ws, size_t ws_bytes, hipStream_t stream);



int ce_rmsnorm_rope_mxfp8(const void* x, const float* w, const float* cos_sin, void* q8, void* scale8, int M, int D, int ldx, int ldq8,
                          int head_dim, float eps, int rope_rows, float post_scale, hipStream_t stream);

int ce_v_mxfp8_transpose(const void* v, int ldv, void* v8t, void* sv, int n_tokens, int batch, int H, int npad, hipStream_t stream);

int ce_attention_mxfp8(const void* q8, const void* sq, const void* k8, const void* sk, const void* v8t, const void* sv, void* O, int Nq,
                       int Nkv, int npad, int H, int head_dim, int ldq8, int ldk8, int ldo, int batch, hipStream_t stream);

int ce_attention_mxfp8_quant(const void* q8, const void* sq, const void* k8, const void* sk, const void* v8t, const void* sv, void* o8,
                             void* scale8, int Nq, int Nkv, int npad, int H, int head_dim, int ldq8, int ldk8, int ldo8, int batch,
                             hipStream_t stream);

int ce_attention_mxfp8_add(const void* q8, const void* sq, const void* k8, const void* sk, const void* v8t, const void* sv, const void* o_add,
                           int ldadd, void* O, int ldo, void* o8, void* scale8, int ldo8, int Nq, int Nkv, int npad, int H, int head_dim,
                           int ldq8, int ldk8, int batch, hipStream_t stream);




int ce_gemm_batched_bf16(const void* A, const void* W, void* C, const float* bias, int epilogue, int M, int N, int K, int lda,
                         int ldw, int ldc, int batch0, int batch1, long long sA0, long long sA1, long long sW0, long long sW1,
                         long long sC0, long long sC1, hipStream_t stream);

int ce_im2col_patch2d_bf16(const void* img, void* cols, int B, int C, int H, int W, int P, int Kpad, hipStream_t stream);

int ce_gather_rows_bf16(const void* table, const long long* ids, void* out, int n, int D, int ldt, int ldo, int vocab,
                        hipStream_t stream);

int ce_rmsnorm_bf16(const void* x, void* y, const void* w, int M, int D, int ldx, int ldy, float eps, hipStream_t stream);

int ce_softmax_t5_bf16(const float* scores, void* probs, int batch, int heads, int Lq, int Lk, int ld, int ldp,
                       const int* bucket_lut, const float* table, const int* valid_len, hipStream_t stream);

int ce_lora_merge_bf16(const void* W0, int ldw0, void* W, int ldw, int N, int K, int n_adapters, const void* const* B,
                       const void* const* A, const int* ranks, const float* scales, hipStream_t stream);

int ce_comm_load(const char* librccl_path);
int ce_comm_unique_id(void* id128);
int ce_comm_init(void** comm_out, const void* id128, int rank, int world);
int ce_comm_destroy(void* comm);
int ce_comm_all_to_all(void* comm, const void* send, void* recv, size_t bytes_per_peer, hipStream_t stream);
int ce_comm_all_gather(void* comm, const void* send, void* recv, size_t bytes_per_rank, hipStream_t stream);

int ce_build_info(void);

#ifdef __cplusplus
}
#endif
#endif
```

Baseline: 3.061.

## Fold Q RMSNorm and RoPE application into attention kernel prologue

The RMSNorm kernel now only computes per-row rstd for Q (it still fully normalises K), and the attention kernels apply the norm weight and optional RoPE to Q fragments in registers before scaling. This removes a full read-modify-write pass over Q in both self-attention and cross-attention paths. In exchange, every attention work item reloads norm weights and cos/sin values and does extra shuffles and register work, which could raise register pressure in a kernel launched with 512 threads and a minimum of 2 blocks.

After: 3.058 (median of 2 runs). Within noise of the previous version (-0.1%).

```diff
diff --git a/chronoedit_amd/csrc/ce_attn.hip b/chronoedit_amd/csrc/ce_attn.hip
--- a/chronoedit_amd/csrc/ce_attn.hip
+++ b/chronoedit_amd/csrc/ce_attn.hip
@@ -38,6 +38,13 @@
   int ld8;
 };
 
+struct QNorm {
+  const float* rstd;
+  const float* w;
+  const float* cs;
+  int rope_rows;
+};
+
 template <bool TWO_SEG, int NWAVE>
 __global__ __launch_bounds__(NWAVE * 64, NWAVE == 8 ? 2 : 2) void attn_fwd_kernel(const bf16* __restrict__ Q, bf16* __restrict__ O, KVSeg seg0,
                                                        KVSeg seg1, int Nq, int H, int ldq, int ldo, int nqb,
@@ -279,10 +286,10 @@
 constexpr int SP_TILE_BYTES = 2 * PK_TILE + 3 * PV_TILE;
 constexpr int sp_smem_bytes(bool two_seg) { return two_seg ? SP_TILE_BYTES + 8 * QW * OST_ROW : SP_TILE_BYTES; }
 
-template <bool TWO_SEG, bool VT = false, bool QOUT = false>
+template <bool TWO_SEG, bool VT = false, bool QOUT = false, int NORMQ = 0>
 __global__ __launch_bounds__(512, 2) void attn_fwd_sp_kernel(const bf16* __restrict__ Q_, bf16* __restrict__ O_, KVSeg seg0_,
                                                               KVSeg seg1_, int Nq, int H, int ldq, int ldo, int nqb,
-                                                              float scale_log2e, int batch, BlkRows blk) {
+                                                              float scale_log2e, int batch, BlkRows blk, QNorm qn) {
   extern __shared__ __attribute__((aligned(16))) unsigned char smem[];
   constexpr int NWAVE = 8, QB = QW * NWAVE;
   const int tid = threadIdx.x, lane = tid & 63;
@@ -327,7 +334,7 @@
       Q += (size_t)bz * Nq * ldq;
       O += (size_t)bz * Nq * ldo;
       seg0.k += (size_t)bz * seg0.len * seg0.ldk;
-      seg0.v += VT ? (size_t)bz * (TWO_SEG ? blk.vt_cols : seg0.len) : (size_t)bz * seg0.len * seg0.ldv;
+      seg0.v += VT ? (size_t)bz * ((TWO_SEG || NORMQ) ? blk.vt_cols : seg0.len) : (size_t)bz * seg0.len * seg0.ldv;
     }
     if (TWO_SEG) {
       seg1.k += (size_t)bz * seg1.len * seg1.ldk;
@@ -345,7 +352,47 @@
 #pragma unroll
     for (int ks = 0; ks < 8; ++ks) qf[ks] = *reinterpret_cast<const bf16x8*>(qrow + 16 * ks);
   }
+  constexpr bool ROPE = NORMQ == 2;
+  float q_rstd = 0.f;
+  f32x4 q_cs[ROPE ? 16 : 1];
+  f32x2 q_w2 = {0.f, 0.f};
+  int q_ln = lane;
+  if (NORMQ) {
+    asm volatile("" : "+v"(q_ln));
+    const int grow = bz * Nq + (q0 + l31 < Nq ? q0 + l31 : 0);
+    q_rstd = qn.rstd[grow];
+    q_w2 = *reinterpret_cast<const f32x2*>(qn.w + hoff + 2 * q_ln);
+    if (ROPE) {
+      const int cr = qn.rope_rows > 0 ? grow % qn.rope_rows : grow;
+      const float* cp = qn.cs + (size_t)cr * HD + 8 * (q_ln >> 5);
+#pragma unroll
+      for (int c = 0; c < 16; ++c) q_cs[c] = *reinterpret_cast<const f32x4*>(cp + 16 * (c >> 1) + 4 * (c & 1));
+    }
+  }
   auto scale_q = [&]() __attribute__((always_inline)) {
+  if (NORMQ) {
+#pragma unroll
+    for (int ks = 0; ks < 8; ++ks) {
+      const u32x4 w = __builtin_bit_cast(u32x4, qf[ks]);
+      u32x4 o;
+#pragma unroll
+      for (int i = 0; i < 4; ++i) {
+        const int src = 4 * (q_ln >> 5) + 8 * ks + i;
+        const float ww0 = __shfl(q_w2[0], src, 64), ww1 = __shfl(q_w2[1], src, 64);
+        float v0 = round_bf16(round_bf16(bf16lo(w[i]) * q_rstd) * ww0);
+        float v1 = round_bf16(round_bf16(bf16hi(w[i]) * q_rstd) * ww1);
+        if (ROPE) {
+          const f32x4 cv = q_cs[ROPE ? 2 * ks + (i >> 1) : 0];
+          const float co = cv[2 * (i & 1)], si = cv[2 * (i & 1) + 1];
+          const float r0 = __builtin_fmaf(co, v0, -(si * v1)), r1 = __builtin_fmaf(co, v1, si * v0);
+          v0 = r0;
+          v1 = r1;
+        }
+        o[i] = pack_bf16(v0, v1);
+      }
+      qf[ks] = __builtin_bit_cast(bf16x8, o);
+    }
+  }
 #pragma unroll
   for (int ks = 0; ks < 8; ++ks) {
     const u32x4 w = __builtin_bit_cast(u32x4, qf[ks]);
@@ -1274,7 +1321,7 @@
       done = true;                                                                                                   \
     }                                                                                                                \
     hipLaunchKernelGGL((attn_fwd_sp_kernel<TWO>), dim3(nqb * H * batch), block, sp_smem_bytes(TWO), stream, (const bf16*)Q, \
-                       (bf16*)O, s0, s1, Nq, H, ldq, ldo, nqb, sl2, batch, BlkRows{0, 0, 0u, 0});                    \
+                       (bf16*)O, s0, s1, Nq, H, ldq, ldo, nqb, sl2, batch, BlkRows{0, 0, 0u, 0}, QNorm{});                    \
   } while (0)
     if (two) CE_ATTN_SP(true); else CE_ATTN_SP(false);
 #undef CE_ATTN_SP
@@ -1335,13 +1382,14 @@
 
 static int attention_vt_launch(const void* Q, const void* K, const void* Vt, int len, int ldk, int ldvt, void* O, int Nq, int H, int head_dim,
                                int ldq, int ldo, float softmax_scale, int batch, int blk_rows, int blk_stride, int vt_sample_cols,
-                               hipStream_t stream) {
+                               const QNorm* qn, hipStream_t stream) {
   if (!Q || !K || !Vt || !O) return CE_ERR_ARG;
+  if (qn && (!qn->rstd || !qn->w || blk_rows != 0 || qn->rope_rows < 0)) return CE_ERR_ARG;
   if (head_dim != HD || Nq <= 0 || H <= 0 || len <= 0 || batch <= 0 || batch > 65535) return CE_ERR_SHAPE;
   const int ntiles_cols = (len + KVB - 1) / KVB * KVB;
   if (blk_rows == 0) {
-    vt_sample_cols = len;
-    if (ldvt < (batch - 1) * len + ntiles_cols) return CE_ERR_SHAPE;
+    if (!qn || vt_sample_cols <= 0) vt_sample_cols = len;
+    if (vt_sample_cols < len || ldvt < (batch - 1) * vt_sample_cols + ntiles_cols) return CE_ERR_SHAPE;
   } else {
     if ((blk_rows & 63) || blk_stride < batch * blk_rows || (Nq % blk_rows) || vt_sample_cols < ntiles_cols ||
         ldvt < (batch - 1) * vt_sample_cols + ntiles_cols)
@@ -1365,6 +1413,25 @@
   }
   const int cus = ce_device_cus();
   const int items = nqb * H * batch;
+  if (qn) {
+    static bool doneq_[CE_MAX_DEVICES] = {};
+    bool& doneq = doneq_[ce_device_slot()];
+    if (!doneq) {
+      (void)hipFuncSetAttribute((const void*)attn_fwd_sp_kernel<false, true, false, 1>, hipFuncAttributeMaxDynamicSharedMemorySize,
+                                sp_smem_bytes(false));
+      (void)hipFuncSetAttribute((const void*)attn_fwd_sp_kernel<false, true, false, 2>, hipFuncAttributeMaxDynamicSharedMemorySize,
+                                sp_smem_bytes(false));
+      doneq = true;
+    }
+    const int gridq = items <= 2 * cus ? items : ((2 * cus) & ~7);
+    if (qn->cs)
+      hipLaunchKernelGGL((attn_fwd_sp_kernel<false, true, false, 2>), dim3(gridq), dim3(512), sp_smem_bytes(false), stream, (const bf16*)Q,
+                         (bf16*)O, s0, s1, Nq, H, ldq, ldo, nqb, sl2, batch, blk, *qn);
+    else
+      hipLaunchKernelGGL((attn_fwd_sp_kernel<false, true, false, 1>), dim3(gridq), dim3(512), sp_smem_bytes(false), stream, (const bf16*)Q,
+                         (bf16*)O, s0, s1, Nq, H, ldq, ldo, nqb, sl2, batch, blk, *qn);
+    return (int)hipGetLastError();
+  }
 #ifdef CE_DIAGNOSTICS
   if (g_attn_nwave == 16 && blk_rows == 0) {
     const int rc = ce_attn16_launch(Q, K, Vt, len, ldk, ldvt, O, Nq, H, ldq, ldo, sl2, batch, cus, stream);
@@ -1385,13 +1452,20 @@
   }
   const int grid_vt = items <= 2 * cus ? items : ((2 * cus) & ~7);
   hipLaunchKernelGGL((attn_fwd_sp_kernel<false, true>), dim3(grid_vt), dim3(512), sp_smem_bytes(false), stream, (const bf16*)Q, (bf16*)O,
-                     s0, s1, Nq, H, ldq, ldo, nqb, sl2, batch, blk);
+                     s0, s1, Nq, H, ldq, ldo, nqb, sl2, batch, blk, QNorm{});
   return (int)hipGetLastError();
 }
 
 CE_API int ce_attention_vt_bf16(const void* Q, const void* K, const void* Vt, int len, int ldk, int ldvt, void* O, int Nq, int H,
                                     int head_dim, int ldq, int ldo, float softmax_scale, int batch, hipStream_t stream) {
-  return attention_vt_launch(Q, K, Vt, len, ldk, ldvt, O, Nq, H, head_dim, ldq, ldo, softmax_scale, batch, 0, 0, 0, stream);
+  return attention_vt_launch(Q, K, Vt, len, ldk, ldvt, O, Nq, H, head_dim, ldq, ldo, softmax_scale, batch, 0, 0, 0, nullptr, stream);
+}
+
+CE_API int ce_attention_vt_normq_bf16(const void* Q, const void* K, const void* Vt, int len, int ldk, int ldvt, void* O, int Nq, int H,
+                                          int head_dim, int ldq, int ldo, float softmax_scale, int batch, const float* rstd_q, const float* nq,
+                                          const float* cos_sin, int rope_rows, hipStream_t stream) {
+  const QNorm qn{rstd_q, nq, cos_sin, rope_rows};
+  return attention_vt_launch(Q, K, Vt, len, ldk, ldvt, O, Nq, H, head_dim, ldq, ldo, softmax_scale, batch, 0, 0, 0, &qn, stream);
 }
 
 CE_API int ce_attention_vt_blocked_bf16(const void* Q, const void* K, const void* Vt, int len, int ldk, int ldvt, void* O, int Nq, int H,
@@ -1399,15 +1473,16 @@
                                             int vt_sample_cols, hipStream_t stream) {
   if (blk_rows <= 0) return CE_ERR_SHAPE;
   return attention_vt_launch(Q, K, Vt, len, ldk, ldvt, O, Nq, H, head_dim, ldq, ldo, softmax_scale, batch, blk_rows, blk_stride, vt_sample_cols,
-                             stream);
+                             nullptr, stream);
 }
 
 
 static int attention_2seg_vt_launch(const void* Q, const void* K1, const void* V1t, int len1, int ldk1, int ldv1t, int vt_cols1,
                                     const void* K2, const void* V2t, int len2, int ldk2, int ldv2t, int vt_cols2, void* O, int Nq,
                                     int H, int head_dim, int ldq, int ldo, float softmax_scale, int batch, void* O8, void* S8, int ldo8,
-                                    hipStream_t stream) {
+                                    const QNorm* qn, hipStream_t stream) {
   if (!Q || !K1 || !V1t || !K2 || !V2t || (!O && !O8)) return CE_ERR_ARG;
+  if (qn && (!qn->rstd || !qn->w || O8)) return CE_ERR_ARG;
   if (head_dim != HD || Nq <= 0 || H <= 0 || len1 <= 0 || len2 <= 0 || batch <= 0 || batch > 65535) return CE_ERR_SHAPE;
   const int c1 = (len1 + KVB - 1) / KVB * KVB, c2 = (len2 + KVB - 1) / KVB * KVB;
   if (vt_cols1 < len1 || vt_cols2 < len2 || ldv1t < (batch - 1) * vt_cols1 + c1 || ldv2t < (batch - 1) * vt_cols2 + c2) return CE_ERR_SHAPE;
@@ -1421,18 +1496,22 @@
   if (!done) {
     (void)hipFuncSetAttribute((const void*)attn_fwd_sp_kernel<true, true>, hipFuncAttributeMaxDynamicSharedMemorySize, sp_smem_bytes(true));
     (void)hipFuncSetAttribute((const void*)attn_fwd_sp_kernel<true, true, true>, hipFuncAttributeMaxDynamicSharedMemorySize, sp_smem_bytes(true));
+    (void)hipFuncSetAttribute((const void*)attn_fwd_sp_kernel<true, true, false, 1>, hipFuncAttributeMaxDynamicSharedMemorySize, sp_smem_bytes(true));
     done = true;
   }
   const BlkRows blk{0, vt_cols2, 0u, vt_cols1, (unsigned char*)O8, (unsigned char*)S8, ldo8};
   const int cus = ce_device_cus();
   const int items = nqb * H * batch;
   const int grid = items <= 2 * cus ? items : ((2 * cus) & ~7);
-  if (O8)
+  if (qn)
+    hipLaunchKernelGGL((attn_fwd_sp_kernel<true, true, false, 1>), dim3(grid), dim3(512), sp_smem_bytes(true), stream, (const bf16*)Q,
+                       (bf16*)O, s0, s1, Nq, H, ldq, ldo, nqb, sl2, batch, blk, *qn);
+  else if (O8)
     hipLaunchKernelGGL((attn_fwd_sp_kernel<true, true, true>), dim3(grid), dim3(512), sp_smem_bytes(true), stream, (const bf16*)Q,
-                       (bf16*)O, s0, s1, Nq, H, ldq, ldo, nqb, sl2, batch, blk);
+                       (bf16*)O, s0, s1, Nq, H, ldq, ldo, nqb, sl2, batch, blk, QNorm{});
   else
     hipLaunchKernelGGL((attn_fwd_sp_kernel<true, true>), dim3(grid), dim3(512), sp_smem_bytes(true), stream, (const bf16*)Q, (bf16*)O,
-                       s0, s1, Nq, H, ldq, ldo, nqb, sl2, batch, blk);
+                       s0, s1, Nq, H, ldq, ldo, nqb, sl2, batch, blk, QNorm{});
   return (int)hipGetLastError();
 }
 
@@ -1441,7 +1520,21 @@
                                          int H, int head_dim, int ldq, int ldo, float softmax_scale, int batch, hipStream_t stream) {
   if (!O) return CE_ERR_ARG;
   return attention_2seg_vt_launch(Q, K1, V1t, len1, ldk1, ldv1t, vt_cols1, K2, V2t, len2, ldk2, ldv2t, vt_cols2, O, Nq, H, head_dim, ldq, ldo,
-                                  softmax_scale, batch, nullptr, nullptr, 0, stream);
+                                  softmax_scale, batch, nullptr, nullptr, 0, nullptr, stream);
+}
+
+CE_API int ce_attention_2seg_vt_normq_bf16(const void* Q, const void* K1, const void* V1t, int len1, int ldk1, int ldv1t, int vt_cols1,
+                                               const void* K2, const void* V2t, int len2, int ldk2, int ldv2t, int vt_cols2, void* O, int Nq,
+                                               int H, int head_dim, int ldq, int ldo, float softmax_scale, int batch, const float* rstd_q,
+                                               const float* nq, hipStream_t stream) {
+  if (!O || !rstd_q || !nq) return CE_ERR_ARG;
+  const QNorm qn{rstd_q, nq, nullptr, 0};
+  if (len2 == 0) {
+    if (vt_cols1 < len1 || (vt_cols1 & 1)) return vt_cols1 < len1 ? CE_ERR_SHAPE : CE_ERR_ALIGN;
+    return attention_vt_launch(Q, K1, V1t, len1, ldk1, ldv1t, O, Nq, H, head_dim, ldq, ldo, softmax_scale, batch, 0, 0, vt_cols1, &qn, stream);
+  }
+  return attention_2seg_vt_launch(Q, K1, V1t, len1, ldk1, ldv1t, vt_cols1, K2, V2t, len2, ldk2, ldv2t, vt_cols2, O, Nq, H, head_dim, ldq, ldo,
+                                  softmax_scale, batch, nullptr, nullptr, 0, &qn, stream);
 }
 
 CE_API int ce_attention_2seg_vt_quant_bf16(const void* Q, const void* K1, const void* V1t, int len1, int ldk1, int ldv1t, int vt_cols1,
@@ -1450,5 +1543,5 @@
                                                hipStream_t stream) {
   if (!o8 || !scale8 || (ldo8 & 15) || ((H * head_dim) & 127)) return CE_ERR_ARG;
   return attention_2seg_vt_launch(Q, K1, V1t, len1, ldk1, ldv1t, vt_cols1, K2, V2t, len2, ldk2, ldv2t, vt_cols2, nullptr, Nq, H, head_dim, ldq,
-                                  8, softmax_scale, batch, o8, scale8, ldo8, stream);
-}
+                                  8, softmax_scale, batch, o8, scale8, ldo8, nullptr, stream);
+}
diff --git a/chronoedit_amd/csrc/ce_rowops.hip b/chronoedit_amd/csrc/ce_rowops.hip
--- a/chronoedit_amd/csrc/ce_rowops.hip
+++ b/chronoedit_amd/csrc/ce_rowops.hip
@@ -134,11 +134,11 @@
   }
 }
 
-template <bool FULL>
-__global__ __launch_bounds__(256) void rmsnorm_rope_kernel(bf16* __restrict__ x0, const float* __restrict__ w0,
-                                                           bf16* __restrict__ x1, const float* __restrict__ w1,
-                                                           const float* __restrict__ cs, int M, int D, int ld,
-                                                           int head_dim, float eps, int rope_rows) {
+template <bool FULL, bool QSTAT>
+__device__ __forceinline__ void rmsnorm_rope_body(bf16* __restrict__ x0, const float* __restrict__ w0,
+                                                  bf16* __restrict__ x1, const float* __restrict__ w1,
+                                                  const float* __restrict__ cs, int M, int D, int ld,
+                                                  int head_dim, float eps, int rope_rows, float* __restrict__ rstd0) {
   const int lane = threadIdx.x & 63;
   const int row = blockIdx.x * 4 + (threadIdx.x >> 6);
   if (row >= M) return;
@@ -162,6 +162,10 @@
     }
   }
   const float rstd = 1.0f / sqrtf(wave_sum(s) / (float)D + eps);
+  if (QSTAT && blockIdx.y == 0) {
+    if (lane == 0) rstd0[row] = rstd;
+    return;
+  }
   const int half = head_dim >> 1;
   const bool cs_once = cs != nullptr && (512 % head_dim) == 0;
   f32x4 csa = {0.f, 0.f, 0.f, 0.f}, csb = {0.f, 0.f, 0.f, 0.f};
@@ -199,6 +203,21 @@
       *reinterpret_cast<u32x4*>(xr + c * 8) = o;
     }
   }
+}
+
+template <bool FULL>
+__global__ __launch_bounds__(256) void rmsnorm_rope_kernel(bf16* __restrict__ x0, const float* __restrict__ w0,
+                                                           bf16* __restrict__ x1, const float* __restrict__ w1,
+                                                           const float* __restrict__ cs, int M, int D, int ld,
+                                                           int head_dim, float eps, int rope_rows) {
+  rmsnorm_rope_body<FULL, false>(x0, w0, x1, w1, cs, M, D, ld, head_dim, eps, rope_rows, nullptr);
+}
+template <bool FULL>
+__global__ __launch_bounds__(256) void rmsnorm_qstat_kernel(const bf16* __restrict__ x0, float* __restrict__ rstd0,
+                                                            bf16* __restrict__ x1, const float* __restrict__ w1,
+                                                            const float* __restrict__ cs, int M, int D, int ld,
+                                                            int head_dim, float eps, int rope_rows) {
+  rmsnorm_rope_body<FULL, true>(const_cast<bf16*>(x0), nullptr, x1, w1, cs, M, D, ld, head_dim, eps, rope_rows, rstd0);
 }
 
 template <bool FULL>
@@ -424,6 +443,19 @@
   return (int)hipGetLastError();
 }
 
+CE_API int ce_rmsnorm_rope_qstat_bf16(const void* xq, float* rstd_q, void* x2, const float* w2, const float* cos_sin, int M, int D,
+                                          int ld, int head_dim, float eps, int rope_rows, hipStream_t stream) {
+  if (!xq || !rstd_q || (x2 && !w2)) return CE_ERR_ARG;
+  if (M <= 0 || D <= 0 || (D & 7) || D > 64 * 8 * ROW_MAXC || (ld & 7) || (head_dim & 7) || D % head_dim) return CE_ERR_SHAPE;
+  if (D == 64 * 8 * ROW_MAXC)
+    hipLaunchKernelGGL(rmsnorm_qstat_kernel<true>, dim3((M + 3) / 4, x2 ? 2 : 1), dim3(256), 0, stream, (const bf16*)xq, rstd_q, (bf16*)x2,
+                       w2, cos_sin, M, D, ld, head_dim, eps, rope_rows);
+  else
+    hipLaunchKernelGGL(rmsnorm_qstat_kernel<false>, dim3((M + 3) / 4, x2 ? 2 : 1), dim3(256), 0, stream, (const bf16*)xq, rstd_q, (bf16*)x2,
+                       w2, cos_sin, M, D, ld, head_dim, eps, rope_rows);
+  return (int)hipGetLastError();
+}
+
 CE_API int ce_timestep_sinusoid(const int64_t* t, float* out, int dim, hipStream_t stream) {
   if (!t || !out || dim <= 0 || (dim & 1)) return CE_ERR_ARG;
   hipLaunchKernelGGL(timestep_sinusoid_kernel<int64_t>, dim3((dim + 255) / 256), dim3(256), 0, stream, t, out, dim);
diff --git a/chronoedit_amd/hiplib.py b/chronoedit_amd/hiplib.py
--- a/chronoedit_amd/hiplib.py
+++ b/chronoedit_amd/hiplib.py
@@ -26,6 +26,7 @@
 SIGNATURES: Dict[str, List] = {
     "ce_ln_affine_bf16": [_P, _P, _P, _P, _I, _I, _I, _I, _F, _I, _I, _P],
     "ce_rmsnorm_rope_bf16": [_P, _P, _P, _P, _P, _I, _I, _I, _I, _F, _I, _P],
+    "ce_rmsnorm_rope_qstat_bf16": [_P, _P, _P, _P, _P, _I, _I, _I, _I, _F, _I, _P],
     "ce_gemm_bf16": [_P, _P, _P, _P, _I, _P, _P, _I, _I, _I, _I, _I, _I, _I, _I, _I, _c.c_longlong, _I, _c.c_longlong, _P, _c.c_size_t, _P],
     "ce_rmsnorm_rope_mxfp8": [_P, _P, _P, _P, _P, _I, _I, _I, _I, _I, _F, _I, _F, _P],
     "ce_v_mxfp8_transpose": [_P, _I, _P, _P, _I, _I, _I, _I, _P],
@@ -56,6 +57,8 @@
     "ce_attention_bf16": [_P, _P, _P, _I, _I, _I, _P, _P, _I, _I, _I, _P, _I, _I, _I, _I, _I, _F, _P],
     "ce_attention_batched_bf16": [_P, _P, _P, _I, _I, _I, _P, _P, _I, _I, _I, _P, _I, _I, _I, _I, _I, _F, _I, _P],
     "ce_attention_vt_bf16": [_P, _P, _P, _I, _I, _I, _P, _I, _I, _I, _I, _I, _F, _I, _P],
+    "ce_attention_vt_normq_bf16": [_P, _P, _P, _I, _I, _I, _P, _I, _I, _I, _I, _I, _F, _I, _P, _P, _P, _I, _P],
+    "ce_attention_2seg_vt_normq_bf16": [_P, _P, _P, _I, _I, _I, _I, _P, _P, _I, _I, _I, _I, _P, _I, _I, _I, _I, _I, _F, _I, _P, _P, _P],
     "ce_attention_2seg_vt_bf16": [_P, _P, _P, _I, _I, _I, _I, _P, _P, _I, _I, _I, _I, _P, _I, _I, _I, _I, _I, _F, _I, _P],
     "ce_attention_2seg_vt_quant_bf16": [_P, _P, _P, _I, _I, _I, _I, _P, _P, _I, _I, _I, _I, _P, _P, _I, _I, _I, _I, _I, _F, _I, _P],
     "ce_v_transpose_bf16": [_P, _I, _P, _I, _I, _I, _P],
diff --git a/chronoedit_amd/ops.py b/chronoedit_amd/ops.py
--- a/chronoedit_amd/ops.py
+++ b/chronoedit_amd/ops.py
@@ -166,6 +166,39 @@
                                       _stream()), "ce_rmsnorm_rope_bf16")
     _prof_end(st, f"rmsnorm_rope_{M}x{D}" + ("x2" if x2 is not None else ""), (8.0 if x2 is not None else 4.0) * M * D)
     return x
+
+
+def rmsnorm_rope_qstat(q: torch.Tensor, rstd: torch.Tensor, cos_sin: Optional[torch.Tensor], head_dim: int, eps: float,
+                       x2: Optional[torch.Tensor] = None, w2: Optional[torch.Tensor] = None):
+    _dev(q, torch.bfloat16, "q"), _dev(rstd, torch.float32, "rstd")
+    M, D, ld = _rows(q, "q")
+    assert rstd.is_contiguous() and rstd.numel() >= M
+    rope_rows = 0
+    if cos_sin is not None:
+        _dev(cos_sin, torch.float32, "cos_sin")
+        assert cos_sin.is_contiguous() and cos_sin.shape[1:] == (head_dim // 2, 2) and M % cos_sin.shape[0] == 0, (cos_sin.shape, M)
+        rope_rows = cos_sin.shape[0]
+    if x2 is not None:
+        _dev(x2, torch.bfloat16, "x2"), _dev(w2, torch.float32, "w2")
+        assert _rows(x2, "x2") == (M, D, ld)
+    st = _prof_begin()
+    _check(lib().ce_rmsnorm_rope_qstat_bf16(_ptr(q), _ptr(rstd), _ptr(x2), _ptr(w2), _ptr(cos_sin), M, D, ld, head_dim, float(eps), rope_rows,
+                                            _stream()), "ce_rmsnorm_rope_qstat_bf16")
+    _prof_end(st, f"rmsnorm_rope_qstat_{M}x{D}" + ("x2" if x2 is not None else ""), (6.0 if x2 is not None else 2.0) * M * D)
+    return rstd
+
+
+def _normq_args(normq, Nq: int, Dq: int, rope: bool):
+    rstd, w = normq[0], normq[1]
+    cs = normq[2] if rope and len(normq) > 2 else None
+    _dev(rstd, torch.float32, "rstd"), _dev(w, torch.float32, "nq")
+    assert rstd.is_contiguous() and rstd.numel() >= Nq and w.is_contiguous() and w.numel() == Dq
+    rope_rows = 0
+    if cs is not None:
+        _dev(cs, torch.float32, "cos_sin")
+        assert cs.is_contiguous() and cs.shape[1:] == (64, 2) and Nq % cs.shape[0] == 0, (cs.shape, Nq)
+        rope_rows = cs.shape[0]
+    return rstd, w, cs, rope_rows
 
 
 def gemm(a: torch.Tensor, w: torch.Tensor, bias: Optional[torch.Tensor], out: Optional[torch.Tensor] = None,
@@ -337,7 +370,7 @@
 
 
 def attention_vt(q: torch.Tensor, k: torch.Tensor, vt: torch.Tensor, heads: int, out: Optional[torch.Tensor] = None,
-                 scale: Optional[float] = None, batch: int = 1):
+                 scale: Optional[float] = None, batch: int = 1, normq=None):
     for n, t in (("q", q), ("k", k), ("vt", vt)):
         _dev(t, torch.bfloat16, n)
     Nq, Dq, ldq = _rows(q, "q")
@@ -350,8 +383,16 @@
     _, _, ldo = _rows(out, "out")
     if scale is None:
         scale = 128 ** -0.5
-    st = _prof_begin()
     nq, l1 = Nq // batch, L1 // batch
+    if normq is not None:
+        rstd, w, cs, rope_rows = _normq_args(normq, Nq, Dq, True)
+        st = _prof_begin()
+        _check(lib().ce_attention_vt_normq_bf16(_ptr(q), _ptr(k), _ptr(vt), l1, ldk, vt.stride(0), _ptr(out), nq, heads, 128, ldq, ldo,
+                                                float(scale), batch, _ptr(rstd), _ptr(w), _ptr(cs), rope_rows, _stream()),
+               "ce_attention_vt_normq_bf16")
+        _prof_end(st, f"attention_{nq}x{l1}+0_h{heads}" + (f"_b{batch}" if batch > 1 else ""), 4.0 * nq * l1 * 128 * heads * batch)
+        return out
+    st = _prof_begin()
     _check(lib().ce_attention_vt_bf16(_ptr(q), _ptr(k), _ptr(vt), l1, ldk, vt.stride(0), _ptr(out), nq, heads, 128, ldq, ldo, float(scale),
                                       batch, _stream()), "ce_attention_vt_bf16")
     _prof_end(st, f"attention_{nq}x{l1}+0_h{heads}" + (f"_b{batch}" if batch > 1 else ""), 4.0 * nq * l1 * 128 * heads * batch)
@@ -361,7 +402,27 @@
 def attention_2seg_vt(q: torch.Tensor, k1: torch.Tensor, v1t: torch.Tensor, len1: int, k2: torch.Tensor, v2t: torch.Tensor, len2: int,
                       heads: int, out: Optional[torch.Tensor] = None, scale: Optional[float] = None, batch: int = 1,
                       cols1: Optional[int] = None, cols2: Optional[int] = None, out8: Optional[torch.Tensor] = None,
-                      scale8: Optional[torch.Tensor] = None):
+                      scale8: Optional[torch.Tensor] = None, normq=None):
+    if normq is not None and len2 == 0:
+        for n, t in (("q", q), ("k1", k1), ("v1t", v1t)):
+            _dev(t, torch.bfloat16, n)
+        Nq, Dq, ldq = _rows(q, "q")
+        _, _, ldk1 = _rows(k1, "k1")
+        assert Dq == heads * 128 and v1t.shape[0] == Dq and v1t.stride(1) == 1 and Nq % batch == 0 and k1.shape[0] == batch * len1 and out8 is None
+        if cols1 is None:
+            assert v1t.shape[1] % batch == 0
+            cols1 = v1t.shape[1] // batch
+        rstd, w, _, _ = _normq_args(normq, Nq, Dq, False)
+        if out is None:
+            out = torch.empty((Nq, Dq), dtype=torch.bfloat16, device=q.device)
+        _, _, ldo = _rows(out, "out")
+        nq = Nq // batch
+        st = _prof_begin()
+        _check(lib().ce_attention_2seg_vt_normq_bf16(_ptr(q), _ptr(k1), _ptr(v1t), len1, ldk1, v1t.stride(0), int(cols1), None, None, 0, 0, 0, 0,
+                                                     _ptr(out), nq, heads, 128, ldq, ldo, float(128 ** -0.5 if scale is None else scale), batch,
+                                                     _ptr(rstd), _ptr(w), _stream()), "ce_attention_2seg_vt_normq_bf16")
+        _prof_end(st, f"attention_{nq}x{len1}+0_h{heads}" + (f"_b{batch}" if batch > 1 else ""), 4.0 * nq * len1 * 128 * heads * batch)
+        return out
     for n, t in (("q", q), ("k1", k1), ("v1t", v1t), ("k2", k2), ("v2t", v2t)):
         _dev(t, torch.bfloat16, n)
     Nq, Dq, ldq = _rows(q, "q")
@@ -392,6 +453,15 @@
     if out is None:
         out = torch.empty((Nq, Dq), dtype=torch.bfloat16, device=q.device)
     _, _, ldo = _rows(out, "out")
+    if normq is not None:
+        rstd, w, _, _ = _normq_args(normq, Nq, Dq, False)
+        st = _prof_begin()
+        _check(lib().ce_attention_2seg_vt_normq_bf16(_ptr(q), _ptr(k1), _ptr(v1t), len1, ldk1, v1t.stride(0), int(cols1), _ptr(k2), _ptr(v2t),
+                                                     len2, ldk2, v2t.stride(0), int(cols2), _ptr(out), nq, heads, 128, ldq, ldo,
+                                                     float(scale), batch, _ptr(rstd), _ptr(w), _stream()), "ce_attention_2seg_vt_normq_bf16")
+        _prof_end(st, f"attention_{nq}x{len1}+{len2}_h{heads}" + (f"_b{batch}" if batch > 1 else ""),
+                  4.0 * nq * (len1 + len2) * 128 * heads * batch)
+        return out
     st = _prof_begin()
     _check(lib().ce_attention_2seg_vt_bf16(_ptr(q), _ptr(k1), _ptr(v1t), len1, ldk1, v1t.stride(0), int(cols1), _ptr(k2), _ptr(v2t),
                                            len2, ldk2, v2t.stride(0), int(cols2), _ptr(out), nq, heads, 128, ldq, ldo,
diff --git a/chronoedit_amd/transformer.py b/chronoedit_amd/transformer.py
--- a/chronoedit_amd/transformer.py
+++ b/chronoedit_amd/transformer.py
@@ -2,6 +2,7 @@
 
 import inspect
 import math
+import os
 import re
 from dataclasses import dataclass
 from types import SimpleNamespace
@@ -186,6 +187,7 @@
         self.fp8_fuse_quant = True
         self.fp8_fuse_attn_quant = True
         self.cross_vt = True
+        self.fused_q_norm = os.environ.get("CE_FUSED_Q_NORM", "1") != "0"
         self._sp = None
         self._cfgp = None
 
@@ -290,6 +292,12 @@
             self._engine.v_transposed = self.v_transposed
             self._engine._ws = {}
             self._engine.ws_generation += 1
+        return self
+
+    def enable_fused_q_norm(self, on: bool = True):
+        self.fused_q_norm = bool(on)
+        if self._engine is not None:
+            self._engine.fused_q_norm = self.fused_q_norm
         return self
 
     def enable_cross_vt(self, on: bool = True):
@@ -360,6 +368,7 @@
         eng = self._engine
         sp = self._sp
         return (self._gen, None if eng is None else eng.ws_generation, self.gemm_dtype, self.fp8_linears, self.attn_dtype, self.v_transposed, self.cross_vt,
+                self.fused_q_norm,
                 self.sp_batch_cfg, bool(getattr(self, "rope_plain_temporal", False)), self.cache_context,
                 None if sp is None else (sp.world, sp.rank), self._cfgp is not None)
 
@@ -498,6 +507,7 @@
         self.fuse_quant = bool(getattr(model, "fp8_fuse_quant", True)) and self.F % 128 == 0
         self.fuse_attn_quant = self.fuse_quant and bool(getattr(model, "fp8_fuse_attn_quant", True))
         self.v_transposed = bool(getattr(model, "v_transposed", True))
+        self.fused_q_norm = bool(getattr(model, "fused_q_norm", True))
         if self.fp8:
             if self.D % 256 or self.F % 256:
                 raise NotImplementedError("fp8 GEMMs need inner and ffn dims that are multiples of 256")
@@ -614,7 +624,8 @@
             D, F, dev = self.D, self.F, self.dev
             e = lambda *s: torch.empty(s, dtype=torch.bfloat16, device=dev)
             ws = SimpleNamespace(x=e(N, D), h=e(N, D), qkv=e(N, 3 * D), att=e(N, D), q2=e(N, D), ffn=e(N, F),
-                                 cols=e(N, self.kpatch), head=e(N, self.w_out.shape[0]))
+                                 cols=e(N, self.kpatch), head=e(N, self.w_out.shape[0]),
+                                 rstd=torch.empty((N,), dtype=torch.float32, device=dev))
             if self.fp8:
                 ws.a8 = torch.empty((N, max(D, F)), dtype=torch.uint8, device=dev)
                 ws.s8 = (torch.empty((ops.mx_scale_bytes(N, max(D, F)),), dtype=torch.uint8, device=dev) if self.mx else
@@ -839,8 +850,12 @@
                     ops.gemm(p.w_qkv[2 * D :], ws.h, p.b_qkv[2 * D :], out=ws.vt[:, : B * Nl], epilogue=ops.EPI_BIAS_ROW)
                 else:
                     ops.gemm(ws.h, p.w_qkv[2 * D :], p.b_qkv[2 * D :], out=ws.vt[:, : B * Nl], epilogue=ops.EPI_BIAS_T)
-                ops.rmsnorm_rope_(ws.qkv[:, :D], p.nq1, cs, hd, eps, x2=ws.qkv[:, D : 2 * D], w2=p.nk1)
-                ops.attention_vt(ws.qkv[:, :D], ws.qkv[:, D : 2 * D], ws.vt, H, out=ws.att, batch=B)
+                if self.fused_q_norm and hd == 128:
+                    ops.rmsnorm_rope_qstat(ws.qkv[:, :D], ws.rstd, cs, hd, eps, x2=ws.qkv[:, D : 2 * D], w2=p.nk1)
+                    ops.attention_vt(ws.qkv[:, :D], ws.qkv[:, D : 2 * D], ws.vt, H, out=ws.att, batch=B, normq=(ws.rstd, p.nq1, cs))
+                else:
+                    ops.rmsnorm_rope_(ws.qkv[:, :D], p.nq1, cs, hd, eps, x2=ws.qkv[:, D : 2 * D], w2=p.nk1)
+                    ops.attention_vt(ws.qkv[:, :D], ws.qkv[:, D : 2 * D], ws.vt, H, out=ws.att, batch=B)
                 att = ws.att
             elif sp is None:
                 self._ln_linear(ws, x, mod[li, 0, 1], mod[li, 0, 0], p, "qkv", ws.qkv, ab_rows=Nl, ab_stride=6 * D)
@@ -871,14 +886,19 @@
                 self._linear(ws, ws.att, p, "o2", x, quantised=q_o2, epilogue=ops.EPI_GATE_RES, gate=None, res=x)
                 k_t = None
             else:
-                ops.rmsnorm_rope_(ws.q2, p.nq2, None, hd, eps)
+                fold_q2 = self.fused_q_norm and ctx.vt and not fuse_o2 and hd == 128
+                if fold_q2:
+                    ops.rmsnorm_rope_qstat(ws.q2, ws.rstd, None, hd, eps)
+                else:
+                    ops.rmsnorm_rope_(ws.q2, p.nq2, None, hd, eps)
                 k_t, v_t, k_i, v_i = ctx.kv[li]
             if k_t is None:
                 pass
             elif ctx.vt and fuse_o2:
                 ops.attention_2seg_vt(ws.q2, k_t, v_t, Tt, k_i, v_i, Ti, H, batch=B, cols1=ctx.c1, cols2=ctx.c2, out8=ws.a8[:, :D], scale8=ws.s8)
             elif ctx.vt:
-                ops.attention_2seg_vt(ws.q2, k_t, v_t, Tt, k_i, v_i, Ti, H, out=ws.att, batch=B, cols1=ctx.c1, cols2=ctx.c2)
+                ops.attention_2seg_vt(ws.q2, k_t, v_t, Tt, k_i, v_i, Ti, H, out=ws.att, batch=B, cols1=ctx.c1, cols2=ctx.c2,
+                                      normq=(ws.rstd, p.nq2) if fold_q2 else None)
             elif k_i is not None:
                 ops.attention(ws.q2, k_t, v_t, H, out=ws.att, k2=k_i, v2=v_i, batch=B)
             else:
diff --git a/include/chronoedit_hip.h b/include/chronoedit_hip.h
--- a/include/chronoedit_hip.h
+++ b/include/chronoedit_hip.h
@@ -31,6 +31,9 @@
 int ce_rmsnorm_rope_bf16(void* x, const float* w, void* x2, const float* w2, const float* cos_sin, int M, int D, int ld,
                          int head_dim, float eps, int rope_rows, hipStream_t stream);
 
+int ce_rmsnorm_rope_qstat_bf16(const void* xq, float* rstd_q, void* x2, const float* w2, const float* cos_sin, int M, int D, int ld,
+                               int head_dim, float eps, int rope_rows, hipStream_t stream);
+
 int ce_gemm_bf16(const void* A, const void* W, void* C, const float* bias, int epilogue, const float* gate, const void* res,
                  int M, int N, int K, int lda, int ldw, int ldc, int ldres, int gate_rows, int a_seg_k, long long a_seg_stride,
                  int w_seg_k, long long w_seg_stride, void* ws, size_t ws_bytes, hipStream_t stream);
@@ -50,9 +53,18 @@
 int ce_attention_vt_bf16(const void* Q, const void* K, const void* Vt, int len, int ldk, int ldvt, void* O, int Nq, int H, int head_dim,
                          int ldq, int ldo, float softmax_scale, int batch, hipStream_t stream);
 
+int ce_attention_vt_normq_bf16(const void* Q, const void* K, const void* Vt, int len, int ldk, int ldvt, void* O, int Nq, int H,
+                               int head_dim, int ldq, int ldo, float softmax_scale, int batch, const float* rstd_q, const float* nq,
+                               const float* cos_sin, int rope_rows, hipStream_t stream);
+
 int ce_attention_2seg_vt_bf16(const void* Q, const void* K1, const void* V1t, int len1, int ldk1, int ldv1t, int vt_cols1, const void* K2,
                               const void* V2t, int len2, int ldk2, int ldv2t, int vt_cols2, void* O, int Nq, int H, int head_dim, int ldq,
                               int ldo, float softmax_scale, int batch, hipStream_t stream);
+
+int ce_attention_2seg_vt_normq_bf16(const void* Q, const void* K1, const void* V1t, int len1, int ldk1, int ldv1t, int vt_cols1,
+                                    const void* K2, const void* V2t, int len2, int ldk2, int ldv2t, int vt_cols2, void* O, int Nq, int H,
+                                    int head_dim, int ldq, int ldo, float softmax_scale, int batch, const float* rstd_q, const float* nq,
+                                    hipStream_t stream);
 
 int ce_attention_2seg_vt_quant_bf16(const void* Q, const void* K1, const void* V1t, int len1, int ldk1, int ldv1t, int vt_cols1, const void* K2,
                                     const void* V2t, int len2, int ldk2, int ldv2t, int vt_cols2, void* o8, void* scale8, int Nq, int H,
```
